# zhizdev/mvdfusion

Hardware: AMD Instinct MI355X
Metric: denoising-steps/sec (higher is better)
Workload: dtype f16x3 (f16 MFMA operands split hi+lo, 3 partial products, fp32 accumulate); 1 GPU; BASELINE.json configs[1]: V=4 views x 256^2 images (32x32 latents), D=1, 50-step DDIM (eta 1), cfg 2.5, SD1.x UNet 320ch + 10 view-aligned transformers + GridAttn, random-init (deterministic fill) weights; views=4, latent=32, depth_samples=1, parallelism=single GPU, CFG pair batched as 2V, hipgraph=True, gemm_tuning=mvdfusion_amd/tuned/gemm_f16.json: 410 problems; 0 problems tuned in this run

## Files before the change

### include/mvd_hip.h

```cpp
#ifndef MVD_HIP_H
#define MVD_HIP_H
#include <stddef.h>
#include <stdint.h>
#ifdef __cplusplus
extern "C" {
#endif

typedef void* mvd_stream_t;

#define MVD_VERSION 100
#define MVD_PREC_X1 1
#define MVD_PREC_X3 3
#define MVD_PREC_X4 4

int mvd_version(void);
const char* mvd_last_error(void);
int mvd_operand_format(void);

size_t mvd_packed_weight_bytes(int N, int K);
int mvd_pack_linear_weight(const float* w, int N, int K, int ldw, int geglu, float scale, void* packed,
                           mvd_stream_t stream);
int mvd_pack_linear_weight_t(const float* wt, int N, int K, int ldw, float scale, void* packed, mvd_stream_t stream);
int mvd_pack_conv3x3_weight(const float* w, int Cout, int Cin, int cin_pad, float scale, void* packed,
                            mvd_stream_t stream);

#define MVD_A_DENSE 0
#define MVD_A_CONV3X3 1

#define MVD_EPI_STORE 0
#define MVD_EPI_GEGLU 1
#define MVD_EPI_QKV 2

#define MVD_ACT_NONE 0
#define MVD_ACT_GELU 1
#define MVD_ACT_SILU 2
#define MVD_ACT_QUICKGELU 3

#define MVD_GEMM_TILES 5
#define MVD_GEMM_LOOPS 8
#define MVD_GEMM_CFG_STRIDE 32
#define MVD_B_PACKED 0
#define MVD_B_PLANES 1

typedef struct mvd_prefetch_item_s {
  const void* ptr;
  unsigned long long bytes;
  int start_after;
  int consumer;
} mvd_prefetch_item;

typedef struct mvd_gemm_desc {
  int M, N, K;
  const void* A;
  int lda;
  int a_mode;
  int B, Hin, Win, Cin, Hout, Wout, stride, upsample;
  int no_pad_tl;
  const void* Wp;
  int b_mode;
  int ldb;
  float acc_scale;
  int prec;
  int epi;
  int act;
  float* out;
  int ldo;
  void* out_sp;
  int ldp;
  int n_store;
  const float* bias;
  const float* bias_b;
  int rows_per_batch;
  int ldbb;
  const float* colscale;
  const float* res;
  int ldr;
  void *q_hi, *q_lo, *k_hi, *k_lo, *vt_hi, *vt_lo;
  int heads, dhead, L, Lpad;
  float qscale;
  int splitk;
  float* workspace;
  size_t workspace_elems;
  int cfg;
  long long* gn_stats;
  int gn_hw, gn_groups;
  float* rs_out;
  int* rs_count;
  int rs_ld;
  const float* ln_stats;
  const int* ln_count;
  const float* ln_colsum;
  int ln_ld, ln_dim;
  float ln_eps;
  void* gna_out_sp;
  const float* gna_gamma;
  const float* gna_beta;
  float gna_eps;
  int gna_flags;
  const float* cat_b;
  int cat_cb;
  void* cat_raw_sp;
  const float* acc_scale_dev;
  const struct mvd_prefetch_item_s* pf_items;
  int pf_n;
  int tap_mode;
  const void* A2;
  int lda2, Cin2;
} mvd_gemm_desc;
#define MVD_TAPS_FULL 0
#define MVD_TAPS_CENTRE_TAIL 2
#define MVD_GNA_SILU 1
#define MVD_GNA_ROUND_F16 2
#define MVD_GNA_OUT_UNUSED 4

int mvd_gemm(const mvd_gemm_desc* d, mvd_stream_t stream);
int mvd_gemm_cfg_supported(const mvd_gemm_desc* d, int cfg);

int mvd_split_planes(const float* x, void* sp, size_t rows, int cols, int ldx, int ldp, mvd_stream_t stream);
int mvd_split_planes_scaled(const float* x, void* sp, size_t rows, int cols, int ldx, int ldp, const float* scale_dev, mvd_stream_t stream);

int mvd_gemv(const float* W, const float* bias, const float* x, float* y, int M, int N, int K, int ldx, int ldy,
             int act_in, int act_out, mvd_stream_t stream);

int mvd_groupnorm_chunks(int HW);
int mvd_groupnorm_nhwc(const float* x, void* y_sp, const float* gamma, const float* beta, int B, int HW, int C,
                       int groups, float eps, int silu, double* ws, size_t ws_elems, mvd_stream_t stream);
int mvd_groupnorm_from_stats(const float* x, void* y_sp, const float* gamma, const float* beta, const long long* stats, int B, int HW,
                             int C, int groups, float eps, int silu, mvd_stream_t stream);
int mvd_softmax_rows(const float* x, void* y_sp, int rows, int cols, int ldx, float scale, float out_scale,
                     mvd_stream_t stream);

int mvd_layernorm(const float* x, void* y_sp, float* y_f32, const float* w, const float* b, int rows, int C, float eps,
                  int w_plus_one, mvd_stream_t stream);
int mvd_layernorm_groups(const float* x, void* y_sp, float* y_f32, const float* w, const float* b, int ldw, int rows, int rows_per_group,
                         int C, float eps, int w_plus_one, mvd_stream_t stream);

size_t mvd_attn_qk_plane_elems(int B, int heads, int L, int dhead);
size_t mvd_attn_vt_plane_elems(int B, int heads, int L, int dhead);
int mvd_attn_lpad(int L);
int mvd_attention(const void* q_hi, const void* q_lo, const void* k_hi, const void* k_lo, const void* vt_hi,
                  const void* vt_lo, void* out_sp, int ldo, int B, int heads, int L, int Lkeys, int dhead, int prec,
                  mvd_stream_t stream);

int mvd_pixel_cross_attn(const float* q, const float* k, const float* v, void* out_sp, int P, int D, int heads,
                         int dhead, mvd_stream_t stream);

int mvd_unet_input(const float* x, const float* input_latents, void* out_sp, int V, int S, int cpad, int cfg,
                   mvd_stream_t stream);
int mvd_unet_input_scenes(const float* x, const float* input_latents, void* out_sp, int nscene, int V, int S, int cpad, int cfg,
                          mvd_stream_t stream);
int mvd_concat_channels(const float* a, int Ca, const float* b, int Cb, float* out, void* out_sp, int rows, long long* gn_stats,
                        int gn_hw, int gn_groups, mvd_stream_t stream);
int mvd_concat_groupnorm_fits(int Ca, int Cb, int hw, int groups);
int mvd_concat_groupnorm(const float* a, int Ca, const float* b, int Cb, float* out, void* raw_sp, void* y_sp, const float* gamma,
                         const float* beta, long long* gn_stats, int B, int hw, int groups, float eps, int silu, mvd_stream_t stream);
int mvd_area_pool(const float* vol, void* out_sp, int B, int S, int D, int C, int factor, int ldp, mvd_stream_t stream);
int mvd_fill_zero(float* p, size_t n, mvd_stream_t stream);

#define MVD_STEP_STRIDE 8
int mvd_timestep_embedding(const float* steps, const int* iter, const float* freqs, float* out, int dim,
                           mvd_stream_t stream);
int mvd_timestep_embedding_scenes(const float* steps, const int* iter, const float* freqs, float* out, int dim, int nscene,
                                  int steps_scene_stride, mvd_stream_t stream);
int mvd_advance_iter(int* iter, mvd_stream_t stream);

#define MVD_CAM_RECORD 20
#define MVD_TOKEN_DIM 723
#define MVD_TOKEN_LD 736
int mvd_zembed(const float* lat, const float* w, const float* b, float* feat, int N, int S, mvd_stream_t stream);
int mvd_gridattn_tokens(const float* x, const float* depth_noise, const float* steps, const int* iter,
                        const float* grid_lin ,
                        const float* feat, const float* in_feat, const float* cams, const float* in_cam,
                        void* tokens_sp, int V, int q0, int Vq, int S, int D, float depth_scale, float depth_shift,
                        mvd_stream_t stream);
int mvd_gridattn_tokens_scenes(const float* x, const float* depth_noise, const float* steps, const int* iter, const float* grid_lin,
                               const float* feat, const float* in_feat, const float* cams, const float* in_cam, void* tokens_sp,
                               int nscene, int V, int q0, int Vq, int S, int D, float depth_scale, float depth_shift,
                               mvd_stream_t stream);
int mvd_gridattn_tokens_scenes_t(const float* x, const float* depth_noise, const float* steps, const int* iter, const float* grid_lin,
                                 const float* feat, const float* in_feat, const float* cams, const float* in_cam, void* tokens_sp,
                                 int nscene, int V, int q0, int Vq, int S, int D, float depth_scale, float depth_shift,
                                 int steps_scene_stride, mvd_stream_t stream);
int mvd_gridattn_fused_slots(void);
size_t mvd_gridattn_fused_stream_bytes(void);
size_t mvd_gridattn_fused_vec_floats(void);
int mvd_gridattn_fused(const float* x, const float* depth_noise, const float* steps, const int* iter, const float* grid_lin,
                       const float* feat, const float* in_feat, const float* cams, const float* in_cam, const void* wstream,
                       const float* vecs, void* pooled_sp, int V, int q0, int Vq, int S, int D, float depth_scale,
                       float depth_shift, int prec ,
                       mvd_stream_t stream);
int mvd_gridattn_fused_scenes(const float* x, const float* depth_noise, const float* steps, const int* iter, const float* grid_lin,
                              const float* feat, const float* in_feat, const float* cams, const float* in_cam, const void* wstream,
                              const float* vecs, void* pooled_sp, int nscene, int V, int q0, int Vq, int S, int D, float depth_scale,
                              float depth_shift, int prec, mvd_stream_t stream);
int mvd_gridattn_fused_scenes_t(const float* x, const float* depth_noise, const float* steps, const int* iter, const float* grid_lin,
                                const float* feat, const float* in_feat, const float* cams, const float* in_cam, const void* wstream,
                                const float* vecs, void* pooled_sp, int nscene, int V, int q0, int Vq, int S, int D, float depth_scale,
                                float depth_shift, int prec, int steps_scene_stride, int vecs_scene_stride, mvd_stream_t stream);
int mvd_gridattn_tokens_window(const float* x, const float* depth_noise, const float* steps, const int* iter, const float* grid_lin,
                               const float* feat, const float* in_feat, const float* cams, const float* in_cam, void* tokens_sp,
                               int nscene, int V, int q0, int Vq, int S, int D, float depth_scale, float depth_shift,
                               int steps_scene_stride, int window, mvd_stream_t stream);
int mvd_gridattn_fused_window(const float* x, const float* depth_noise, const float* steps, const int* iter, const float* grid_lin,
                              const float* feat, const float* in_feat, const float* cams, const float* in_cam, const void* wstream,
                              const float* vecs, void* pooled_sp, int nscene, int V, int q0, int Vq, int S, int D, float depth_scale,
                              float depth_shift, int prec, int steps_scene_stride, int vecs_scene_stride, int window,
                              mvd_stream_t stream);
int mvd_view_mha(const float* qkv, void* out_sp, int Nseq, int V, int heads, int dhead,
                 mvd_stream_t stream);
int mvd_view_pool(const float* x, const float* w, const float* b, void* out_sp, int Nseq, int V, int C,
                  mvd_stream_t stream);

int mvd_cfg_ddim_update(const float* eps_nhwc, int ldc, float* x, float* x0, float* eps_out,
                        const float* ddim_noise, size_t noise_stride ,
                        const float* steps, const int* iter, int V, int S, int cfg, float cfg_scale, int do_update,
                        mvd_stream_t stream);

int mvd_graph_begin(mvd_stream_t stream);
int mvd_graph_end(mvd_stream_t stream, void** graph_exec);
int mvd_graph_launch(void* graph_exec, mvd_stream_t stream);
int mvd_graph_destroy(void* graph_exec);
int mvd_event_create(void** ev);
int mvd_event_record(void* ev, mvd_stream_t stream);
int mvd_event_elapsed_ms(void* start, void* stop, float* ms);
int mvd_event_destroy(void* ev);

int mvd_transpose_planes(const void* x, int src_planes, int rows, int cols, int ldx, void* out_sp, int ldo, mvd_stream_t stream);
int mvd_transpose_planes_scaled(const float* x, int rows, int cols, int ldx, void* out_sp, int ldo, const float* scale_dev,
                                mvd_stream_t stream);
int mvd_im2col3x3_t_planes(const void* x_sp, int B, int H, int W, int Cin, void* out_sp, int ldo, mvd_stream_t stream);
int mvd_pow2_scale(const float* x, size_t n, float* out2, unsigned* scratch2, mvd_stream_t stream);
int mvd_adamw_multi(const void* tensors, int n_tensors, int n_chunks, float lr, float beta1, float beta2, float eps, float weight_decay,
                    float bias_c1, float bias_c2_sqrt, float grad_scale, mvd_stream_t stream);
size_t mvd_col_sum_workspace_doubles(int rows, int cols);
int mvd_col_sum(const float* x, int rows, int cols, int ldx, float* out, double* ws, size_t ws_doubles, mvd_stream_t stream);
int mvd_col_sum_pow2(const float* x, int rows, int cols, int ldx, float* out, double* ws, size_t ws_doubles, float* out2, unsigned* scratch1,
                     mvd_stream_t stream);
int mvd_groupnorm_backward(const float* x, const float* dy, const float* gamma, const float* beta, int B, int HW, int C, int groups,
                           float eps, int silu, float* dx, float* dgamma, float* dbeta, float* ws, size_t ws_floats,
                           mvd_stream_t stream);

int mvd_layernorm_backward(const float* x, const float* dy, const float* w, int rows, int C, float eps, float* dx, float* dyxhat,
                           mvd_stream_t stream);
size_t mvd_col_sum_groups_workspace_doubles(int ngroups, int rows_per_group, int cols);
int mvd_col_sum_groups(const float* x, int ngroups, int rows_per_group, int cols, int ldx, float* out, double* ws, size_t ws_doubles,
                       mvd_stream_t stream);
int mvd_layernorm_backward_groups(const float* x, const float* dy, const float* w, int ldw, int rows, int rows_per_group, int C, float eps,
                                  float* dx, float* dyxhat, float* dw, float* db, double* ws, size_t ws_doubles, mvd_stream_t stream);
int mvd_act_planes(const float* x, void* sp, float* y, size_t rows, int cols, int ldx, int ldp, int ldy, int act, mvd_stream_t stream);
int mvd_act_backward(const float* dy, const float* x, float* dx, size_t n, int act, mvd_stream_t stream);
int mvd_geglu_backward(const float* h, const float* dy, int rows, int half, float* dh, mvd_stream_t stream);
int mvd_attention_backward(const float* q, const float* k, const float* v, const float* dout, int B, int heads, int L, int dhead,
                           float* dq, float* dk, float* dv, float* stats, size_t stats_floats, mvd_stream_t stream);
int mvd_pixel_cross_attn_backward(const float* q, const float* k, const float* v, const float* dout, int P, int D, int heads, int dhead,
                                  float* dq, float* dk, float* dv, mvd_stream_t stream);

int mvd_gridattn_tokens_backward(const float* x, const float* depth_noise, const float* steps, const int* iter, const float* grid_lin,
                                 const float* cams, const float* in_cam, const float* dtok, int ldt, long long* dfeat_acc,
                                 long long* din_feat_acc, float scale, int V, int q0, int Vq, int S, int D, float depth_scale,
                                 float depth_shift, mvd_stream_t stream);
int mvd_gridattn_tokens_backward_scenes(const float* x, const float* depth_noise, const float* steps, const int* iter, const float* grid_lin,
                                        const float* cams, const float* in_cam, const float* dtok, int ldt, long long* dfeat_acc,
                                        long long* din_feat_acc, float scale, int nscene, int V, int q0, int Vq, int S, int D,
                                        float depth_scale, float depth_shift, int steps_scene_stride, mvd_stream_t stream);
int mvd_gridattn_tokens_backward_window(const float* x, const float* depth_noise, const float* steps, const int* iter, const float* grid_lin,
                                        const float* cams, const float* in_cam, const float* dtok, int ldt, long long* dfeat_acc,
                                        long long* din_feat_acc, float scale, int nscene, int V, int q0, int Vq, int S, int D,
                                        float depth_scale, float depth_shift, int steps_scene_stride, int window, mvd_stream_t stream);

#ifdef __cplusplus
}
#endif
#endif
```

### mvdfusion_amd/csrc/gemm.hip

```cpp
#include "gemm_device.hpp"

namespace {

__global__ __launch_bounds__(256) void splitk_reduce_kernel(GemmParams p) {
  const mvd_gemm_desc& d = p.d;
  const size_t MN = (size_t)d.M * d.N;
  if (d.epi == MVD_EPI_GEGLU) {
    const size_t total = (size_t)d.M * (d.N >> 1);
    for (size_t e = (size_t)blockIdx.x * 256 + threadIdx.x; e < total; e += (size_t)gridDim.x * 256) {
      const int m = (int)(e / (d.N >> 1));
      const int col = (int)(e - (size_t)m * (d.N >> 1));
      const int pv = (col >> 4) * 32 + (col & 15);
      float v = 0.f, g = 0.f;
      for (int z = 0; z < p.splits; ++z) {
        v += d.workspace[z * MN + (size_t)m * d.N + pv];
        g += d.workspace[z * MN + (size_t)m * d.N + pv + 16];
      }
      epi_geglu_elem(d, m, pv, v, g);
    }
    return;
  }
  if (d.epi == MVD_EPI_STORE) {
    const size_t MN4 = MN >> 2;
    const float inv = 1.0f / gemm_acc_scale(d);
    (void)inv;
    for (size_t e = (size_t)blockIdx.x * 256 + threadIdx.x; e < MN4; e += (size_t)gridDim.x * 256) {
      float4 v = make_float4(0.f, 0.f, 0.f, 0.f);
      for (int z = 0; z < p.splits; ++z) {
        const float4 t = *(const float4*)(d.workspace + z * MN + e * 4);
        v.x += t.x; v.y += t.y; v.z += t.z; v.w += t.w;
      }
      const int m = (int)((e * 4) / d.N);
      const int n = (int)(e * 4 - (size_t)m * d.N);
      if (n + 3 < d.n_store) {
        epi_store4(d, m, n, v);
      } else {
        epi_store_elem(d, m, n, v.x);
        epi_store_elem(d, m, n + 1, v.y);
        epi_store_elem(d, m, n + 2, v.z);
        epi_store_elem(d, m, n + 3, v.w);
      }
    }
    return;
  }
  for (size_t e = (size_t)blockIdx.x * 256 + threadIdx.x; e < MN; e += (size_t)gridDim.x * 256) {
    float v = 0.f;
    for (int z = 0; z < p.splits; ++z) v += d.workspace[z * MN + e];
    const int m = (int)(e / d.N);
    const int n = (int)(e - (size_t)m * d.N);
    epi_store_elem(d, m, n, v);
  }
}

__global__ __launch_bounds__(256) void splitk_reduce_rows_kernel(GemmParams p) {
  const mvd_gemm_desc& d = p.d;
  const size_t MN = (size_t)d.M * d.N;
  const int lane = threadIdx.x & 63;
  const int m = blockIdx.x * 4 + (threadIdx.x >> 6);
  const int n = blockIdx.y * 256 + lane * 4;
  if (m >= d.M) return;
  float s1 = 0.f, q1 = 0.f;
  if (n < d.N) {
    float4 v = make_float4(0.f, 0.f, 0.f, 0.f);
    const float* w = d.workspace + (size_t)m * d.N + n;
    for (int z = 0; z < p.splits; ++z) {
      const float4 t = *(const float4*)(w + z * MN);
      v.x += t.x; v.y += t.y; v.z += t.z; v.w += t.w;
    }
    const float4 f = epi_store4(d, m, n, v);
    s1 = (f.x + f.y) + (f.z + f.w);
    q1 = (f.x * f.x + f.y * f.y) + (f.z * f.z + f.w * f.w);
  }
  s1 = wave_sum(s1);
  q1 = wave_sum(q1);
  if (lane == 0) *((float2*)d.rs_out + (size_t)m * d.rs_ld + blockIdx.y) = make_float2(s1, q1);
  if (blockIdx.x == 0 && blockIdx.y == 0 && threadIdx.x == 0) d.rs_count[0] = gridDim.y;
}

template <int RPT>
__global__ __launch_bounds__(256) void splitk_reduce_stats_kernel(GemmParams p) {
  __shared__ float cs[2][4][256];
  const mvd_gemm_desc& d = p.d;
  const size_t MN = (size_t)d.M * d.N;
  const int m0 = blockIdx.x * (4 * RPT), n0 = blockIdx.y * 256;
  const int c4 = threadIdx.x & 63, rg = threadIdx.x >> 6;
  const int n = n0 + c4 * 4;
  float4 s = make_float4(0.f, 0.f, 0.f, 0.f), q = make_float4(0.f, 0.f, 0.f, 0.f);
  if (n < d.N) {
    float4 v[RPT];
#pragma unroll
    for (int r = 0; r < RPT; ++r) v[r] = make_float4(0.f, 0.f, 0.f, 0.f);
    const float* w = d.workspace + (size_t)(m0 + rg * RPT) * d.N + n;
#pragma unroll 2
    for (int z = 0; z < p.splits; ++z) {
#pragma unroll
      for (int r = 0; r < RPT; ++r) {
        const float4 t = *(const float4*)(w + z * MN + (size_t)r * d.N);
        v[r].x += t.x; v[r].y += t.y; v[r].z += t.z; v[r].w += t.w;
      }
    }
#pragma unroll
    for (int r = 0; r < RPT; ++r) v[r] = epi_value4(d, m0 + rg * RPT + r, n, v[r]);
#pragma unroll
    for (int r = 0; r < RPT; ++r) {
      const float4 f = v[r];
      epi_put4(d, m0 + rg * RPT + r, n, f);
      s.x += f.x; s.y += f.y; s.z += f.z; s.w += f.w;
      q.x += f.x * f.x; q.y += f.y * f.y; q.z += f.z * f.z; q.w += f.w * f.w;
    }
  }
  *(float4*)&cs[0][rg][c4 * 4] = s;
  *(float4*)&cs[1][rg][c4 * 4] = q;
  __syncthreads();
  const int c = threadIdx.x, nn = n0 + c;
  const float cs_ = cs[0][0][c] + cs[0][1][c] + cs[0][2][c] + cs[0][3][c];
  const float cq_ = cs[1][0][c] + cs[1][1][c] + cs[1][2][c] + cs[1][3][c];
  __syncthreads();
  cs[0][0][c] = cs_;
  cs[1][0][c] = cq_;
  __syncthreads();
  if (nn >= d.N) return;
  const int cg = d.N / d.gn_groups;
  const int g = nn / cg, pos = nn - g * cg;
  if (c != 0 && pos != 0) return;
  int len = cg - pos;
  if (len > 256 - c) len = 256 - c;
  float ss = 0.f, qq = 0.f;
  for (int j = 0; j < len; ++j) {
    ss += cs[0][0][c + j];
    qq += cs[1][0][c + j];
  }
  gn_stats_add(d.gn_stats, m0 / d.gn_hw, g, d.gn_groups, ss, qq);
}

#define MVD_GNK_THREADS 1024
__global__ __launch_bounds__(MVD_GNK_THREADS) void splitk_gn_kernel(GemmParams p) {
  constexpr int NT = MVD_GNK_THREADS, NWV = NT / 64, U = 3, ZC = 4;
  extern __shared__ float s_val[];
  __shared__ double s_red[2][NWV];
  __shared__ float s_coef[2][128];
  const mvd_gemm_desc& d = p.d;
  const int G = d.gn_groups, HW = d.gn_hw;
  const int CT = d.N + (d.cat_b ? d.cat_cb : 0);
  const int cg = CT / G, cg2 = cg >> 1;
  int g, b;
  {
    const int bid = blockIdx.x;
    if ((G & 7) == 0) {
      const int gpx = G >> 3, x = bid & 7, r = bid >> 3;
      g = x * gpx + r % gpx;
      b = r / gpx;
    } else {
      g = bid % G;
      b = bid / G;
    }
  }
  const int tid = threadIdx.x, lane = tid & 63, wave = tid >> 6;
  const int c0 = g * cg, m0 = b * HW;
  const size_t MN = (size_t)d.M * d.N;
  const int total = HW * cg2;
  const bool put_out = d.out != nullptr && !(d.gna_flags & MVD_GNA_OUT_UNUSED);
  const int dq = NT / cg2, dj = NT - dq * cg2;
  const int rs = tid / cg2, js = tid - rs * cg2;
  const int r0 = tid < total ? rs : 0, j0 = tid < total ? js : 0;
  const float* const zero2 = (const float*)g_zero_page;
  const bool has_bias = d.bias != nullptr, has_bb = d.bias_b != nullptr, has_res = d.res != nullptr;
  const float ascale = gemm_acc_scale(d);
  float s = 0.f, q = 0.f;
  {
    int r = rs, j = js;
    for (int e0 = tid; e0 < total; e0 += NT * U) {
      int rr[U], jj[U];
      bool ok[U];
#pragma unroll
      for (int u = 0; u < U; ++u) {
        ok[u] = e0 + u * NT < total;
        rr[u] = ok[u] ? r : r0;
        jj[u] = ok[u] ? j : j0;
        r += dq;
        j += dj;
        if (j >= cg2) {
          j -= cg2;
          ++r;
        }
      }
      float2 acc[U], tb[U], tbb[U], tr[U];
      float2 t[ZC][U];
      const int nz0 = p.splits < ZC ? p.splits : ZC;
      bool own[U];
      float2 tc[U];
#pragma unroll
      for (int u = 0; u < U; ++u) {
        const int m = m0 + rr[u], nn = c0 + 2 * jj[u];
        own[u] = nn < d.N;
        const int n = own[u] ? nn : 0;
        tb[u] = *(const float2*)(has_bias ? d.bias + n : zero2);
        tbb[u] = *(const float2*)(has_bb ? d.bias_b + (size_t)(m / d.rows_per_batch) * d.ldbb + n : zero2);
        tr[u] = *(const float2*)(has_res ? d.res + (size_t)m * d.ldr + n : zero2);
        tc[u] = *(const float2*)(own[u] ? zero2 : d.cat_b + (size_t)m * d.cat_cb + (nn - d.N));
#pragma unroll
        for (int z = 0; z < ZC; ++z) {
          const float* w = d.workspace + (size_t)(z < nz0 ? z : 0) * MN + (size_t)m * d.N + n;
          t[z][u] = *(const float2*)w;
        }
      }
#pragma unroll
      for (int u = 0; u < U; ++u) {
        acc[u] = make_float2(0.f, 0.f);
#pragma unroll
        for (int z = 0; z < ZC; ++z)
          if (z < nz0) {
            acc[u].x += t[z][u].x;
            acc[u].y += t[z][u].y;
          }
      }
      for (int zb = ZC; zb < p.splits; zb += ZC) {
        const int nz = p.splits - zb < ZC ? p.splits - zb : ZC;
#pragma unroll
        for (int u = 0; u < U; ++u) {
          const int m = m0 + rr[u], n = own[u] ? c0 + 2 * jj[u] : 0;
#pragma unroll
          for (int z = 0; z < ZC; ++z) t[z][u] = *(const float2*)(d.workspace + (size_t)(zb + (z < nz ? z : 0)) * MN + (size_t)m * d.N + n);
        }
#pragma unroll
        for (int u = 0; u < U; ++u)
#pragma unroll
          for (int z = 0; z < ZC; ++z)
            if (z < nz) {
              acc[u].x += t[z][u].x;
              acc[u].y += t[z][u].y;
            }
      }
#pragma unroll
      for (int u = 0; u < U; ++u) {
        float2 v = acc[u];
        v.x = v.x * ascale + tb[u].x + tbb[u].x + tr[u].x;
        v.y = v.y * ascale + tb[u].y + tbb[u].y + tr[u].y;
        if (!own[u]) v = tc[u];
        if (ok[u]) {
          const int m = m0 + rr[u], n = c0 + 2 * jj[u];
          if (put_out && own[u]) *(float2*)(d.out + (size_t)m * d.ldo + n) = v;
          if (d.cat_raw_sp) {
            uint32_t hh, ll;
            split_op16x2(v.x, v.y, hh, ll);
            u16* pp = (u16*)d.cat_raw_sp + sp_index((size_t)m, CT, n);
            *(uint32_t*)pp = hh;
            *(uint32_t*)(pp + 32) = ll;
          }
          *(float2*)(s_val + 2 * (e0 + u * NT)) = v;
          s += v.x + v.y;
          q += v.x * v.x + v.y * v.y;
        }
      }
    }
  }
  unsigned pf_sink = 0;
  if (d.pf_items != nullptr) {
    const __attribute__((address_space(4))) mvd_prefetch_item* tab = (const __attribute__((address_space(4))) mvd_prefetch_item*)d.pf_items;
    const int gw = blockIdx.x * NWV + wave, GW = gridDim.x * NWV;
    for (int it = 0; it < d.pf_n; ++it) {
      const unsigned char* base = (const unsigned char*)tab[it].ptr;
      const long lines = (long)((tab[it].bytes + 127) >> 7);
      for (long l = (long)gw * 64 + lane; l < lines; l += (long)GW * 64) {
        const unsigned char* a = base + (l << 7);
        asm volatile("global_load_dword %0, %1, off" : "+v"(pf_sink) : "v"(a) : "memory");
      }
    }
  }
  {
    const double sd = wave_sum_d((double)s), qd = wave_sum_d((double)q);
    if (lane == 0) {
      s_red[0][wave] = sd;
      s_red[1][wave] = qd;
    }
  }
  __syncthreads();
  double S1 = 0.0, S2 = 0.0;
#pragma unroll
  for (int w = 0; w < NWV; ++w) {
    S1 += s_red[0][w];
    S2 += s_red[1][w];
  }
  const double cnt = (double)HW * cg;
  const double mean = S1 / cnt;
  double var = S2 / cnt - mean * mean;
  if (var < 0.0) var = 0.0;
  const float rstd = (float)(1.0 / sqrt(var + (double)d.gna_eps));
  if (tid < cg) {
    const float a = rstd * d.gna_gamma[c0 + tid];
    s_coef[0][tid] = a;
    s_coef[1][tid] = d.gna_beta[c0 + tid] - (float)mean * a;
  }
  if (tid == 0 && d.gn_stats) gn_stats_add(d.gn_stats, b, g, G, (float)S1, (float)S2);
  __syncthreads();
  u16* const ysp = (u16*)d.gna_out_sp;
  const int fl = d.gna_flags;
  {
    int r = rs, j = js;
    for (int e = tid; e < total; e += NT) {
      float2 v = *(const float2*)(s_val + 2 * e);
      v.x = v.x * s_coef[0][2 * j] + s_coef[1][2 * j];
      v.y = v.y * s_coef[0][2 * j + 1] + s_coef[1][2 * j + 1];
      if (fl & MVD_GNA_ROUND_F16) {
        v.x = (float)(_Float16)v.x;
        v.y = (float)(_Float16)v.y;
      }
      if (fl & MVD_GNA_SILU) {
        v.x = silu_f(v.x);
        v.y = silu_f(v.y);
      }
      uint32_t hh, ll;
      split_op16x2(v.x, v.y, hh, ll);
      u16* pp = ysp + sp_index((size_t)(m0 + r), CT, c0 + 2 * j);
      *(uint32_t*)pp = hh;
      *(uint32_t*)(pp + 32) = ll;
      r += dq;
      j += dj;
      if (j >= cg2) {
        j -= cg2;
        ++r;
      }
    }
  }
  asm volatile("" ::"v"(pf_sink));
}

struct TileInfo {
  int bm, bn, waves;
  int cores_plain, cores_pipe;
};
static const TileInfo kTiles[MVD_GEMM_TILES] = {{64, 64, 4, 5, 3}, {128, 128, 8, 2, 1}, {128, 80, 4, 2, 2}, {64, 80, 4, 4, 3},
                                                {128, 160, 8, 1, 1}};

static int choose_splits(long tiles, int nk, const TileInfo& ti, int loop, size_t mn) {
  const double area = (double)ti.bm * ti.bn / (128.0 * 128.0);
  const double t_mfma = 0.75 * area;
  const double t_lat = loop == 0 ? 1.0 : (loop == 1 ? 0.4 : (loop == 2 ? 0.2 : (loop == 5 ? 0.05 : 0.1)));
  const double t_epi = 0.27 + 1.73 * area;
  const int coresident = loop == 0 ? ti.cores_plain : (loop == 1 ? ti.cores_pipe : (loop == 4 && ti.waves == 4 ? 2 : 1));
  const double red_fixed = 6.0, red_per_split = (double)mn * 8.0 / 3.0e12 / 0.7e-6;
  int best = 1;
  double best_t = 1e30;
  const int smax = nk / 8 < 1 ? 1 : (nk / 8 > 32 ? 32 : nk / 8);
  for (int sp = 1; sp <= smax; ++sp) {
    const int iters = (nk + sp - 1) / sp;
    if ((long)iters * (sp - 1) >= nk) continue;
    const long per_cu = (tiles * sp + 255) / 256;
    const long rounds = (per_cu + coresident - 1) / coresident;
    const double busy = (double)per_cu * (iters * t_mfma + t_epi);
    const double lat = (double)rounds * (iters * t_lat + t_epi);
    double t = busy > lat ? busy : lat;
    if (sp > 1) t += red_fixed + sp * red_per_split;
    if (t < best_t * 0.97) {
      best_t = t;
      best = sp;
    }
  }
  return best;
}

static int patch_shares(const mvd_gemm_desc& d, const TileInfo& ti) {
  if (d.a_mode != MVD_A_CONV3X3 || d.b_mode != MVD_B_PACKED || d.stride != 1 || d.upsample || d.no_pad_tl) return 0;
  if (d.tap_mode != MVD_TAPS_FULL) return 0;
  if (d.Hin != d.Hout || d.Win != d.Wout || ti.bm != 128) return 0;
  const int W = d.Wout, HW = d.Hout * d.Wout;
  if (ti.bm % W != 0 || (HW >= ti.bm ? HW % ti.bm != 0 : ti.bm % HW != 0)) return 0;
  const int nseg = HW >= ti.bm ? 1 : ti.bm / HW, Rb = HW >= ti.bm ? ti.bm / W : d.Hout;
  const int P = nseg * (Rb + 2) * (W + 2);
  if (P > MVD_PATCH_SLOTS_MAX) return 0;
  const int PG = (P + 7) / 8, cap = (11 - conv_patch_ring(ti.bn, ti.waves)) * ti.waves;
  return PG <= cap ? 1 : (PG <= 2 * cap ? 2 : 0);
}

static bool cfg_supported(const mvd_gemm_desc& d, int cfg) {
  if (cfg == 0) return true;
  if (cfg < 0 || cfg > MVD_GEMM_CFG_STRIDE * MVD_GEMM_TILES) return false;
  const int tile = (cfg - 1) / MVD_GEMM_CFG_STRIDE, loop = ((cfg - 1) % MVD_GEMM_CFG_STRIDE) >> 1;
  if (loop >= MVD_GEMM_LOOPS) return false;
  if (tile >= 2 && d.epi != MVD_EPI_STORE) return false;
  const int waves = kTiles[tile].waves;
  if ((loop == 2 || loop == 3) && waves != 8) return false;
  if (loop == 3 || loop >= 8) return false;
  if (loop == 5 && waves != 4) return false;
  if (loop == 6) return (tile == 1 || tile == 2 || tile == 4) && patch_shares(d, kTiles[tile]) > 0;
  if (loop == 7) return tile == 1 || ((tile == 2 || tile == 4) && d.epi == MVD_EPI_STORE);
  return true;
}

}

extern "C" int mvd_gemm_cfg_supported(const mvd_gemm_desc* dp, int cfg) { return dp && cfg_supported(*dp, cfg) ? 1 : 0; }

extern "C" int mvd_gemm(const mvd_gemm_desc* dp, mvd_stream_t stream) {
  MVD_CHECK_ARG(dp != nullptr, "mvd_gemm: null descriptor");
  GemmParams p;
  p.d = *dp;
  mvd_gemm_desc& d = p.d;
  MVD_CHECK_ARG(d.M > 0 && d.N > 0 && d.K > 0, "mvd_gemm: bad sizes M=%d N=%d K=%d", d.M, d.N, d.K);
  MVD_CHECK_ARG(d.K % 32 == 0, "mvd_gemm: K=%d must be a multiple of 32 (pad the packed weight)", d.K);
  MVD_CHECK_ARG(d.N % 16 == 0, "mvd_gemm: N=%d must be a multiple of 16 (pad the packed weight)", d.N);
  MVD_CHECK_ARG(d.prec == MVD_PREC_X1 || d.prec == MVD_PREC_X3 || d.prec == MVD_PREC_X4, "mvd_gemm: bad prec %d", d.prec);
  MVD_CHECK_ARG(d.A && d.Wp, "mvd_gemm: null operand");
  MVD_CHECK_ARG(((uintptr_t)d.A & 127) == 0 && ((uintptr_t)d.Wp & 127) == 0, "mvd_gemm: operands must be 128-byte aligned");
  if (d.a_mode == MVD_A_CONV3X3) {
    MVD_CHECK_ARG(d.tap_mode == MVD_TAPS_FULL || d.tap_mode == MVD_TAPS_CENTRE_TAIL, "mvd_gemm: tap_mode %d is not served", d.tap_mode);
    const bool tail = d.tap_mode == MVD_TAPS_CENTRE_TAIL;
    if (tail) {
      MVD_CHECK_ARG(d.A2 != nullptr && ((uintptr_t)d.A2 & 127) == 0 && d.Cin2 > 0 && d.Cin2 % 32 == 0 && d.lda2 >= d.Cin2 && d.lda2 % 32 == 0,
                    "mvd_gemm: the centre-tap tail needs A2 (128-byte aligned), Cin2 %% 32 == 0 and lda2 >= Cin2, a multiple of 32 (Cin2=%d lda2=%d)",
                    d.Cin2, d.lda2);
      MVD_CHECK_ARG(d.stride == 1 && !d.upsample && !d.no_pad_tl && d.Hin == d.Hout && d.Win == d.Wout && d.b_mode == MVD_B_PACKED,
                    "mvd_gemm: the centre-tap tail serves stride-1 padded convolutions with Hin == Hout, Win == Wout and a packed weight");
      MVD_CHECK_ARG((long long)d.M * 2 * d.lda2 < (1ll << 31), "mvd_gemm: A2 is addressed with 32-bit offsets (M=%d lda2=%d)", d.M, d.lda2);
    }
    MVD_CHECK_ARG(d.Cin % 32 == 0 && d.K == 9 * d.Cin + (tail ? d.Cin2 : 0),
                  "mvd_gemm: conv needs Cin %% 32 == 0 and K == 9*Cin (+ Cin2 with a centre-tap tail) (Cin=%d Cin2=%d K=%d)", d.Cin,
                  tail ? d.Cin2 : 0, d.K);
    MVD_CHECK_ARG(d.M == d.B * d.Hout * d.Wout, "mvd_gemm: conv M mismatch");
    MVD_CHECK_ARG(d.stride == 1 || d.stride == 2, "mvd_gemm: conv stride must be 1 or 2");
    if (d.upsample) MVD_CHECK_ARG(d.stride == 1 && d.Hout == 2 * d.Hin && d.Wout == 2 * d.Win, "mvd_gemm: upsample geometry");
  } else {
    MVD_CHECK_ARG(d.a_mode == MVD_A_DENSE, "mvd_gemm: bad a_mode");
    MVD_CHECK_ARG(d.tap_mode == MVD_TAPS_FULL, "mvd_gemm: tap_mode %d needs a_mode == MVD_A_CONV3X3", d.tap_mode);
    MVD_CHECK_ARG(d.lda >= d.K && d.lda % 32 == 0, "mvd_gemm: lda=%d must be >= K=%d and a multiple of 32", d.lda, d.K);
  }
  if (d.out_sp) MVD_CHECK_ARG(d.ldp > 0 && d.ldp % 32 == 0 && ((uintptr_t)d.out_sp & 127) == 0,
                              "mvd_gemm: split-plane output needs ldp %% 32 == 0 and 128-byte alignment");
  if (d.out) MVD_CHECK_ARG(d.ldo % 4 == 0 && ((uintptr_t)d.out & 15) == 0, "mvd_gemm: out must be 16-byte aligned with ldo %% 4 == 0");
  if (d.res) MVD_CHECK_ARG(d.ldr % 4 == 0 && ((uintptr_t)d.res & 15) == 0, "mvd_gemm: res must be 16-byte aligned with ldr %% 4 == 0");
  MVD_CHECK_ARG(((uintptr_t)d.bias & 15) == 0 && ((uintptr_t)d.bias_b & 15) == 0 && ((uintptr_t)d.colscale & 15) == 0,
                "mvd_gemm: bias / bias_b / colscale must be 16-byte aligned");
  if (d.epi == MVD_EPI_STORE) {
    MVD_CHECK_ARG(d.out != nullptr || d.out_sp != nullptr, "mvd_gemm: no output");
    if (d.n_store <= 0 || d.n_store > d.N) d.n_store = d.N;
    if (d.bias_b) {
      MVD_CHECK_ARG(d.rows_per_batch > 0, "mvd_gemm: bias_b needs rows_per_batch");
      if (d.ldbb == 0) d.ldbb = d.N;
      MVD_CHECK_ARG(d.ldbb % 4 == 0, "mvd_gemm: ldbb %% 4 != 0");
    }
  } else if (d.epi == MVD_EPI_GEGLU) {
    MVD_CHECK_ARG((d.out != nullptr || d.out_sp != nullptr) && d.N % 32 == 0, "mvd_gemm: GEGLU needs an output and N %% 32 == 0");
    d.bias_b = nullptr;
  } else if (d.epi == MVD_EPI_QKV) {
    MVD_CHECK_ARG(d.q_hi && d.q_lo && d.k_hi && d.k_lo && d.vt_hi && d.vt_lo, "mvd_gemm: QKV planes missing");
    MVD_CHECK_ARG(d.heads > 0 && d.dhead > 0 && d.N == 3 * d.heads * d.dhead, "mvd_gemm: QKV needs N == 3*heads*dhead");
    MVD_CHECK_ARG(d.L > 0 && d.M % d.L == 0 && d.Lpad >= d.L, "mvd_gemm: QKV needs M %% L == 0");
    MVD_CHECK_ARG(d.dhead % 4 == 0 && d.L % 4 == 0, "mvd_gemm: QKV needs dhead %% 4 == 0 and L %% 4 == 0");
  } else {
    MVD_CHECK_ARG(false, "mvd_gemm: bad epilogue %d", d.epi);
  }
  if (d.rs_out)
    MVD_CHECK_ARG(d.epi == MVD_EPI_STORE && d.n_store == d.N && !d.gn_stats && d.rs_count && d.rs_ld >= cdiv(d.N, 32) && ((uintptr_t)d.rs_out & 7) == 0,
                  "mvd_gemm: rs_out needs MVD_EPI_STORE, n_store == N, no gn_stats, rs_count and rs_ld >= N / 32 (N=%d rs_ld=%d)", d.N, d.rs_ld);
  if (d.ln_stats) {
    MVD_CHECK_ARG((d.epi == MVD_EPI_QKV || d.epi == MVD_EPI_GEGLU) && d.ln_count && d.ln_colsum && d.ln_dim > 0 && d.ln_ld > 0 &&
                      ((uintptr_t)d.ln_stats & 7) == 0 && ((uintptr_t)d.ln_colsum & 15) == 0,
                  "mvd_gemm: ln_stats (LayerNorm fold) serves the QKV / GEGLU epilogues and needs ln_count, ln_colsum, ln_dim, ln_ld");
    d.splitk = 1;
  }
  if (d.gn_stats)
    MVD_CHECK_ARG(d.epi == MVD_EPI_STORE && d.n_store == d.N && d.M % 16 == 0 && d.gn_hw > 0 && d.gn_hw % 16 == 0 && d.gn_groups > 0 &&
                      d.N % d.gn_groups == 0,
                  "mvd_gemm: gn_stats needs MVD_EPI_STORE, n_store == N, M %% 16 == 0, gn_hw %% 16 == 0, N %% gn_groups == 0 (N=%d M=%d hw=%d)",
                  d.N, d.M, d.gn_hw);
  if (d.gna_out_sp)
    MVD_CHECK_ARG(d.gn_stats && d.out && d.ldo == d.N && d.gna_gamma && d.gna_beta && d.N % 32 == 0 && d.M % d.gn_hw == 0 &&
                      ((uintptr_t)d.gna_out_sp & 127) == 0,
                  "mvd_gemm: gna_out_sp (GroupNorm apply behind the GEMM) needs gn_stats, out with ldo == N, gamma / beta, N %% 32 == 0, M %% gn_hw == 0");
  if (d.cat_b)
    MVD_CHECK_ARG(d.gna_out_sp && d.cat_cb > 0 && d.cat_cb % 2 == 0 && (d.N + d.cat_cb) % 32 == 0 && (d.N + d.cat_cb) % d.gn_groups == 0 &&
                      ((uintptr_t)d.cat_b & 7) == 0 && ((uintptr_t)d.cat_raw_sp & 127) == 0 &&
                      mvd_concat_groupnorm_fits(d.N, d.cat_cb, d.gn_hw, d.gn_groups),
                  "mvd_gemm: cat_b (GroupNorm over [out | cat_b]) needs gna_out_sp, an even cat_cb, (N + cat_cb) %% 32 == 0 and a shape "
                  "mvd_concat_groupnorm_fits() accepts (N=%d cat_cb=%d hw=%d)", d.N, d.cat_cb, d.gn_hw);
  long long* const gna_stats = d.gn_stats;
  if (d.cat_b) d.gn_stats = nullptr;
  if (d.b_mode == MVD_B_PLANES)
    MVD_CHECK_ARG(d.ldb >= d.K && d.ldb % 32 == 0, "mvd_gemm: B planes need ldb=%d >= K=%d, a multiple of 32", d.ldb, d.K);
  else
    MVD_CHECK_ARG(d.b_mode == MVD_B_PACKED, "mvd_gemm: bad b_mode %d", d.b_mode);
  if (d.acc_scale == 0.f) d.acc_scale = 1.f;
  p.nk = d.K / 32;
  p.nt16 = d.N / 16;
  int tile, loop = 0, order = -1;
  MVD_CHECK_ARG(d.cfg >= 0 && d.cfg <= MVD_GEMM_CFG_STRIDE * MVD_GEMM_TILES, "mvd_gemm: bad cfg %d", d.cfg);
  if (d.cfg >= 1) {
    tile = (d.cfg - 1) / MVD_GEMM_CFG_STRIDE;
    loop = ((d.cfg - 1) % MVD_GEMM_CFG_STRIDE) >> 1;
    order = (d.cfg - 1) & 1;
    MVD_CHECK_ARG(cfg_supported(d, d.cfg), "mvd_gemm: cfg %d (tile %d, loop %d) does not serve this problem (include/mvd_hip.h: cfg)", d.cfg, tile,
                  loop);
  } else {
    const long tiles128 = (long)cdiv(d.M, 128) * cdiv(d.N, 128);
    tile = (tiles128 >= 128 && (d.N >= 512 || d.K >= 2048)) ? 1 : 0;
  }
  const TileInfo& ti = kTiles[tile];
  p.tiles_n = cdiv(d.N, ti.bn);
  p.tiles_m = cdiv(d.M, ti.bm);
  if (order < 0) {
    const double W = (double)d.N * d.K * 4.0;
    const double A = (double)d.M * d.K * 4.0 / (d.a_mode == MVD_A_CONV3X3 ? 9.0 : 1.0);
    const double rep_m = p.tiles_m < 8 ? p.tiles_m : 8, rep_n = p.tiles_n < 8 ? p.tiles_n : 8;
    order = (W + A * rep_n) < (W * rep_m + A) ? 1 : 0;
  }
  p.m_fastest = order;
  int splits = d.splitk;
  const long tiles = (long)p.tiles_m * p.tiles_n;
  if (splits == 0) splits = choose_splits(tiles, p.nk, ti, loop, (size_t)d.M * d.N);
  if (splits < 1) splits = 1;
  if (splits > p.nk) splits = p.nk;
  if (splits > 1) {
    if (d.workspace == nullptr) splits = 1;
    else {
      const size_t cap = d.workspace_elems / ((size_t)d.M * d.N);
      if ((size_t)splits > cap) splits = cap < 1 ? 1 : (int)cap;
    }
  }
  p.kt_per_split = cdiv(p.nk, splits);
  if (loop == 6) p.kt_per_split = 9 * cdiv(p.nk / 9, splits);
  p.splits = cdiv(p.nk, p.kt_per_split);
  hipStream_t s = (hipStream_t)stream;
  bool launched;
  if (loop == 6) launched = mvd_gemm_launch_patch(tile, p, s, patch_shares(d, ti));
  else if (loop == 7) launched = mvd_gemm_launch_ws(tile, p, s);
  else if (tile == 0) launched = mvd_gemm_launch_plain_t0(loop, p, s);
  else if (tile == 1) launched = mvd_gemm_launch_plain_t1(loop, p, s);
  else if (tile == 2) launched = mvd_gemm_launch_plain_t2(loop, p, s);
  else if (tile == 3) launched = mvd_gemm_launch_plain_t3(loop, p, s);
  else launched = mvd_gemm_launch_plain_t4(loop, p, s);
  MVD_CHECK_ARG(launched, "mvd_gemm: no kernel for tile %d loop %d", tile, loop);
  MVD_CHECK_LAUNCH("mvd_gemm");
  const int gna_ct = d.N + (d.cat_b ? d.cat_cb : 0);
  const int gna_cg = d.gna_out_sp ? gna_ct / d.gn_groups : 0;
  const size_t gna_lds = (size_t)d.gn_hw * gna_cg * 4;
  const bool gna_fused = d.gna_out_sp && p.splits > 1 && !d.rs_out && !d.out_sp && !d.colscale && d.act == MVD_ACT_NONE && (gna_cg & 1) == 0 &&
                         gna_cg <= 128 && gna_lds <= 128 * 1024 && d.ldo % 2 == 0 && (!d.res || d.ldr % 2 == 0) && (!d.bias_b || d.ldbb % 2 == 0) &&
                         d.N % 2 == 0;
  if (gna_fused) {
    {
      static unsigned long long raised = 0;
      const hipError_t e = mvd_raise_dynamic_lds((const void*)splitk_gn_kernel, 128 * 1024, &raised);
      MVD_CHECK_ARG(e == hipSuccess, "mvd_gemm: hipFuncSetAttribute(MaxDynamicSharedMemorySize): %s", hipGetErrorString(e));
    }
    p.d.gn_stats = gna_stats;
    if (loop == 7) p.d.pf_items = nullptr;
    hipLaunchKernelGGL(splitk_gn_kernel, dim3((d.M / d.gn_hw) * d.gn_groups), dim3(MVD_GNK_THREADS), gna_lds, s, p);
    MVD_CHECK_LAUNCH("mvd_gemm/splitk_gn");
    return 0;
  }
  if (p.splits > 1) {
    if (d.rs_out) {
      hipLaunchKernelGGL(splitk_reduce_rows_kernel, dim3(cdiv(d.M, 4), cdiv(d.N, 256)), dim3(256), 0, s, p);
    } else if (d.gn_stats) {
      const int spans = (d.N + 255) / 256;
      if ((d.M / 16) * spans >= 1024)
        hipLaunchKernelGGL(splitk_reduce_stats_kernel<4>, dim3(d.M / 16, spans), dim3(256), 0, s, p);
      else
        hipLaunchKernelGGL(splitk_reduce_stats_kernel<2>, dim3(d.M / 8, spans), dim3(256), 0, s, p);
    } else {
      const size_t total = (size_t)d.M * d.N;
      int blocks = (int)((total + 255) / 256);
      if (blocks > 2048) blocks = 2048;
      hipLaunchKernelGGL(splitk_reduce_kernel, dim3(blocks), dim3(256), 0, s, p);
    }
    MVD_CHECK_LAUNCH("mvd_gemm/splitk_reduce");
  }
  if (d.gna_out_sp && d.cat_b)
    return mvd_concat_groupnorm(d.out, d.N, d.cat_b, d.cat_cb, nullptr, d.cat_raw_sp, d.gna_out_sp, d.gna_gamma, d.gna_beta, gna_stats,
                                d.M / d.gn_hw, d.gn_hw, d.gn_groups, d.gna_eps, d.gna_flags & (MVD_GNA_SILU | MVD_GNA_ROUND_F16), stream);
  if (d.gna_out_sp)
    return mvd_groupnorm_from_stats(d.out, d.gna_out_sp, d.gna_gamma, d.gna_beta, d.gn_stats, d.M / d.gn_hw, d.gn_hw, d.N, d.gn_groups,
                                    d.gna_eps, d.gna_flags & (MVD_GNA_SILU | MVD_GNA_ROUND_F16), stream);
  return 0;
}

namespace {
__global__ __launch_bounds__(256) void pack_kernel(const float* __restrict__ w, u16* __restrict__ out, int N, int K,
                                                   int Np, int Kp, int ldw, int geglu, int conv_cin, int trans,
                                                   float scale) {
  const int nt16 = Np >> 4;
  const size_t total = (size_t)(Kp >> 5) * nt16 * 64;
  for (size_t e = (size_t)blockIdx.x * 256 + threadIdx.x; e < total; e += (size_t)gridDim.x * 256) {
    const size_t mt = e >> 6;
    const int l = (int)(e & 63);
    const int kt = (int)(mt / nt16), nt = (int)(mt - (size_t)kt * nt16);
    const int n = nt * 16 + (l & 15);
    const int k = kt * 32 + (l >> 4) * 8;
    int src_n = n;
    if (geglu) {
      const int blk = n >> 5, within = n & 31;
      src_n = within < 16 ? blk * 16 + within : (N >> 1) + blk * 16 + (within - 16);
    }
    float v[8];
#pragma unroll
    for (int j = 0; j < 8; ++j) v[j] = 0.f;
    if (src_n < N) {
      if (conv_cin > 0) {
        const int cb = kt / 9, tap = kt - cb * 9;
        const int ci0 = cb * 32 + (k & 31);
#pragma unroll
        for (int j = 0; j < 8; ++j)
          if (ci0 + j < conv_cin) v[j] = w[((size_t)src_n * conv_cin + ci0 + j) * 9 + tap];
      } else if (trans) {
#pragma unroll
        for (int j = 0; j < 8; ++j)
          if (k + j < K) v[j] = w[(size_t)(k + j) * ldw + src_n];
      } else {
        const float* src = w + (size_t)src_n * ldw + k;
        if (k + 7 < K && (ldw & 3) == 0 && ((uintptr_t)w & 15) == 0) {
          const float4 a = *(const float4*)src, b = *(const float4*)(src + 4);
          v[0] = a.x; v[1] = a.y; v[2] = a.z; v[3] = a.w; v[4] = b.x; v[5] = b.y; v[6] = b.z; v[7] = b.w;
        } else {
#pragma unroll
          for (int j = 0; j < 8; ++j)
            if (k + j < K) v[j] = src[j];
        }
      }
    }
    union { uint4 q; u16 h[8]; } H, Lo;
#pragma unroll
    for (int j = 0; j < 8; ++j) split_op16(v[j] * scale, H.h[j], Lo.h[j]);
    u16* o = out + mt * 1024 + l * 8;
    *(uint4*)o = H.q;
    *(uint4*)(o + 512) = Lo.q;
  }
}

__global__ __launch_bounds__(256) void split_planes_kernel(const float* __restrict__ x, u16* __restrict__ sp, size_t rows, int cols,
                                                           int ldx, int ldp, const float* __restrict__ scale) {
  const float sc = scale != nullptr ? *scale : 1.f;
  const int c4 = ldp >> 2;
  const size_t total = rows * c4;
  for (size_t e = (size_t)blockIdx.x * 256 + threadIdx.x; e < total; e += (size_t)gridDim.x * 256) {
    const size_t r = e / c4;
    const int c = (int)(e - r * c4) * 4;
    float v[4];
#pragma unroll
    for (int j = 0; j < 4; ++j) v[j] = (c + j) < cols ? x[r * ldx + c + j] * sc : 0.f;
    store_sp4(sp, r, ldp, c, v[0], v[1], v[2], v[3]);
  }
}
}

extern "C" size_t mvd_packed_weight_bytes(int N, int K) {
  const size_t Np = (size_t)((N + 15) & ~15), Kp = (size_t)((K + 31) & ~31);
  return Np * Kp * 4;
}

extern "C" int mvd_operand_format(void) { return MVD_OPERAND_FORMAT; }

extern "C" int mvd_pack_linear_weight(const float* w, int N, int K, int ldw, int geglu, float scale, void* packed,
                                      mvd_stream_t stream) {
  MVD_CHECK_ARG(w && packed && N > 0 && K > 0 && ldw >= K, "mvd_pack_linear_weight: bad arguments");
  if (geglu) MVD_CHECK_ARG(N % 32 == 0, "mvd_pack_linear_weight: geglu needs N %% 32 == 0");
  const int Np = (N + 15) & ~15, Kp = (K + 31) & ~31;
  const size_t total = (size_t)Np * Kp / 8;
  int blocks = (int)((total + 255) / 256);
  if (blocks > 4096) blocks = 4096;
  hipLaunchKernelGGL(pack_kernel, dim3(blocks), dim3(256), 0, (hipStream_t)stream, w, (u16*)packed, N, K, Np, Kp, ldw,
                     geglu, 0, 0, scale);
  MVD_CHECK_LAUNCH("mvd_pack_linear_weight");
  return 0;
}

extern "C" int mvd_pack_linear_weight_t(const float* wt, int N, int K, int ldw, float scale, void* packed, mvd_stream_t stream) {
  MVD_CHECK_ARG(wt && packed && N > 0 && K > 0 && ldw >= N, "mvd_pack_linear_weight_t: bad arguments");
  const int Np = (N + 15) & ~15, Kp = (K + 31) & ~31;
  const size_t total = (size_t)Np * Kp / 8;
  int blocks = (int)((total + 255) / 256);
  if (blocks > 4096) blocks = 4096;
  hipLaunchKernelGGL(pack_kernel, dim3(blocks), dim3(256), 0, (hipStream_t)stream, wt, (u16*)packed, N, K, Np, Kp, ldw, 0, 0, 1, scale);
  MVD_CHECK_LAUNCH("mvd_pack_linear_weight_t");
  return 0;
}

extern "C" int mvd_pack_conv3x3_weight(const float* w, int Cout, int Cin, int cin_pad, float scale, void* packed,
                                       mvd_stream_t stream) {
  MVD_CHECK_ARG(w && packed && Cout > 0 && Cin > 0 && cin_pad >= Cin && cin_pad % 32 == 0,
                "mvd_pack_conv3x3_weight: bad arguments (cin_pad must be a multiple of 32)");
  const int Np = (Cout + 15) & ~15, Kp = 9 * cin_pad;
  const size_t total = (size_t)Np * Kp / 8;
  int blocks = (int)((total + 255) / 256);
  if (blocks > 4096) blocks = 4096;
  hipLaunchKernelGGL(pack_kernel, dim3(blocks), dim3(256), 0, (hipStream_t)stream, w, (u16*)packed, Cout, Kp, Np, Kp, 0,
                     0, Cin, 0, scale);
  MVD_CHECK_LAUNCH("mvd_pack_conv3x3_weight");
  return 0;
}

extern "C" int mvd_split_planes_scaled(const float* x, void* sp, size_t rows, int cols, int ldx, int ldp, const float* scale_dev,
                                       mvd_stream_t stream) {
  MVD_CHECK_ARG(x && sp && rows > 0 && cols > 0 && ldx >= cols && ldp >= cols && ldp % 32 == 0,
                "mvd_split_planes: bad arguments (ldp must be a multiple of 32)");
  const size_t total = rows * (size_t)(ldp / 4);
  int blocks = (int)((total + 255) / 256);
  if (blocks > 4096) blocks = 4096;
  hipLaunchKernelGGL(split_planes_kernel, dim3(blocks), dim3(256), 0, (hipStream_t)stream, x, (u16*)sp, rows, cols, ldx, ldp, scale_dev);
  MVD_CHECK_LAUNCH("mvd_split_planes");
  return 0;
}

extern "C" int mvd_split_planes(const float* x, void* sp, size_t rows, int cols, int ldx, int ldp, mvd_stream_t stream) {
  return mvd_split_planes_scaled(x, sp, rows, cols, ldx, ldp, nullptr, stream);
}
```

### mvdfusion_amd/csrc/gemm_common.hpp

```cpp
#pragma once
#include "common.hpp"
#include "../../include/mvd_hip.h"

struct GemmParams {
  mvd_gemm_desc d;
  int nk;
  int nt16;
  int kt_per_split;
  int splits;
  int tiles_m, tiles_n;
  int m_fastest;
};

__device__ __forceinline__ float gemm_acc_scale(const mvd_gemm_desc& d) {
  return d.acc_scale_dev != nullptr ? d.acc_scale * *d.acc_scale_dev : d.acc_scale;
}

bool mvd_gemm_launch_plain_t0(int loop, GemmParams& p, hipStream_t s);
bool mvd_gemm_launch_plain_t1(int loop, GemmParams& p, hipStream_t s);
bool mvd_gemm_launch_plain_t2(int loop, GemmParams& p, hipStream_t s);
bool mvd_gemm_launch_plain_t3(int loop, GemmParams& p, hipStream_t s);
bool mvd_gemm_launch_plain_t4(int loop, GemmParams& p, hipStream_t s);
bool mvd_gemm_launch_ws(int tile, GemmParams& p, hipStream_t s);
bool mvd_gemm_launch_patch(int tile, GemmParams& p, hipStream_t s, int patch_shares);
```

### mvdfusion_amd/csrc/gemm_device.hpp

```cpp
#pragma once
#include <stdlib.h>
#include <type_traits>

#include "gemm_common.hpp"

namespace {

__device__ __attribute__((aligned(16))) unsigned int g_zero_page[4];

__device__ __forceinline__ float apply_act(float v, int act) {
  if (act == MVD_ACT_GELU) return gelu_erf(v);
  if (act == MVD_ACT_SILU) return silu_f(v);
  if (act == MVD_ACT_QUICKGELU) return v / (1.0f + expf(-1.702f * v));
  return v;
}

__device__ __forceinline__ void store_out(const mvd_gemm_desc& d, int m, int n, float v) {
  if (d.out) d.out[(size_t)m * d.ldo + n] = v;
  if (d.out_sp) store_sp1((u16*)d.out_sp, (size_t)m, d.ldp, n, v);
}

__device__ __forceinline__ float epi_store_elem(const mvd_gemm_desc& d, int m, int n, float v) {
  if (d.epi == MVD_EPI_STORE && n >= d.n_store) return 0.f;
  v *= gemm_acc_scale(d);
  if (d.bias) v += d.bias[n];
  if (d.bias_b) v += d.bias_b[(size_t)(m / d.rows_per_batch) * d.ldbb + n];
  if (d.epi == MVD_EPI_QKV) {
    const int C = d.heads * d.dhead;
    const int which = n / C;
    const int cc = n - which * C;
    const int head = cc / d.dhead;
    const int dd = cc - head * d.dhead;
    const int b = m / d.L;
    const int tok = m - b * d.L;
    if (which == 0) v *= d.qscale;
    if (which < 2) {
      const int dq = mvd_attn_dpad(d.dhead);
      const size_t idx = ((size_t)(b * d.heads + head) * d.Lpad + tok) * dq + dd;
      store_planes1((u16*)(which == 0 ? d.q_hi : d.k_hi), (u16*)(which == 0 ? d.q_lo : d.k_lo), idx, v);
    } else {
      const int dv = (d.dhead + 15) & ~15;
      const size_t idx = ((size_t)(b * d.heads + head) * dv + dd) * d.Lpad + tok;
      store_planes1((u16*)d.vt_hi, (u16*)d.vt_lo, idx, v);
    }
    return v;
  }
  v = apply_act(v, d.act);
  if (d.colscale) v *= d.colscale[n];
  if (d.res) v += d.res[(size_t)m * d.ldr + n];
  store_out(d, m, n, v);
  return v;
}

__device__ __forceinline__ void epi_geglu_elem(const mvd_gemm_desc& d, int m, int p_value, float v, float g) {
  const int col = (p_value >> 5) * 16 + (p_value & 15);
  const int half = d.N >> 1;
  v *= gemm_acc_scale(d);
  g *= gemm_acc_scale(d);
  if (d.bias) {
    v += d.bias[col];
    g += d.bias[half + col];
  }
  store_out(d, m, col, v * gelu_erf(g));
}

__device__ __forceinline__ float4 epi_value4(const mvd_gemm_desc& d, int m, int n, float4 v) {
  v.x *= gemm_acc_scale(d); v.y *= gemm_acc_scale(d); v.z *= gemm_acc_scale(d); v.w *= gemm_acc_scale(d);
  if (d.bias) {
    const float4 b = *(const float4*)(d.bias + n);
    v.x += b.x; v.y += b.y; v.z += b.z; v.w += b.w;
  }
  if (d.bias_b) {
    const float4 b = *(const float4*)(d.bias_b + (size_t)(m / d.rows_per_batch) * d.ldbb + n);
    v.x += b.x; v.y += b.y; v.z += b.z; v.w += b.w;
  }
  if (d.act) {
    v.x = apply_act(v.x, d.act); v.y = apply_act(v.y, d.act); v.z = apply_act(v.z, d.act); v.w = apply_act(v.w, d.act);
  }
  if (d.colscale) {
    const float4 g = *(const float4*)(d.colscale + n);
    v.x *= g.x; v.y *= g.y; v.z *= g.z; v.w *= g.w;
  }
  if (d.res) {
    const float4 r = *(const float4*)(d.res + (size_t)m * d.ldr + n);
    v.x += r.x; v.y += r.y; v.z += r.z; v.w += r.w;
  }
  return v;
}
__device__ __forceinline__ void epi_put4(const mvd_gemm_desc& d, int m, int n, const float4& v) {
  if (d.out) *(float4*)(d.out + (size_t)m * d.ldo + n) = v;
  if (d.out_sp) store_sp4((u16*)d.out_sp, (size_t)m, d.ldp, n, v.x, v.y, v.z, v.w);
}
__device__ __forceinline__ float4 epi_store4(const mvd_gemm_desc& d, int m, int n, float4 v) {
  v = epi_value4(d, m, n, v);
  epi_put4(d, m, n, v);
  return v;
}

__device__ __forceinline__ int conv_tail_start(const mvd_gemm_desc& d) {
  return d.tap_mode == MVD_TAPS_CENTRE_TAIL ? 9 * (d.Cin >> 5) : 0x7fffffff;
}

#define MVD_PATCH_SLOTS_MAX 288
__host__ __device__ constexpr int conv_patch_ring(int bn, int waves) {
  const int bstage = ((bn / 8 + waves - 1) / waves) * waves;
  const int fit = (160 - 2 * (MVD_PATCH_SLOTS_MAX / 8 + 1) - 2) / bstage;
  return fit > 4 ? 4 : fit;
}

__device__ __forceinline__ float2 ln_row_stats(const mvd_gemm_desc& d, int m) {
  const int cnt = d.ln_count[0];
  const float2* p = (const float2*)d.ln_stats + (size_t)m * d.ln_ld;
  double s = 0.0, q = 0.0;
  for (int i = 0; i < cnt; i += 4) {
    float2 v[4];
#pragma unroll
    for (int j = 0; j < 4; ++j) v[j] = p[min(i + j, cnt - 1)];
#pragma unroll
    for (int j = 0; j < 4; ++j) {
      if (i + j < cnt) {
        s += (double)v[j].x;
        q += (double)v[j].y;
      }
    }
  }
  const double mean = s / (double)d.ln_dim;
  double var = q / (double)d.ln_dim - mean * mean;
  if (var < 0.0) var = 0.0;
  return make_float2((float)mean, (float)(1.0 / sqrt(var + (double)d.ln_eps)));
}

#ifdef MVD_STAMP
#define MVD_STAMP_AT(d, wave, slot)                                                                                       \
  do {                                                                                                                    \
    if ((blockIdx.x == 0 || blockIdx.x == 100) && (wave) < 4 && (threadIdx.x & 63) == 0)                                  \
      ((long long*)(d).workspace)[(blockIdx.x == 100 ? 64 : 0) + (wave) * 16 + (slot)] = (long long)__builtin_readcyclecounter(); \
  } while (0)
#else
#define MVD_STAMP_AT(d, wave, slot) do {} while (0)
#endif

template <int BM, int BN, int WM, int WN>
__device__ __forceinline__ void tile_epilogue(const GemmParams& p, f32x4 (&acc)[BM / WM / 16][BN / WN / 16], unsigned char* smem, int m0,
                                              int n0, int lane, int wave, const float* s_rows = nullptr) {
  constexpr int WTM = BM / WM, WTN = BN / WN;
  constexpr int TM = WTM / 16, TN = WTN / 16;
  constexpr int LDW = WTN + 4;
  constexpr int C4 = WTN / 4;
  const mvd_gemm_desc& d = p.d;
  const int wm = wave / WN, wn = wave % WN;
  float* sC = (float*)smem + wave * (WTM * LDW);
  MVD_STAMP_AT(d, wave, 4);
  {
    const int crow = (lane >> 4) * 4, ccol = lane & 15;
#pragma unroll
    for (int i = 0; i < TM; ++i)
#pragma unroll
      for (int j = 0; j < TN; ++j)
#pragma unroll
        for (int r = 0; r < 4; ++r) sC[(i * 16 + crow + r) * LDW + j * 16 + ccol] = acc[i][j][r];
  }
  const int wm0 = m0 + wm * WTM, wn0 = n0 + wn * WTN;
#ifdef MVD_STAMP
  asm volatile("s_waitcnt lgkmcnt(0)" ::: "memory");
#endif
  MVD_STAMP_AT(d, wave, 5);
  if (wn0 >= d.N) return;
  const bool lnf = s_rows != nullptr;
  const float* sR = s_rows + (wave / WN) * WTM * 2;
  if (p.splits > 1) {
    float* ws = d.workspace + (size_t)blockIdx.z * d.M * d.N;
#pragma unroll 2
    for (int ps = 0; ps < (WTM * C4 + 63) / 64; ++ps) {
      const int idx = ps * 64 + lane;
      const int row = idx / C4, col = (idx - row * C4) * 4;
      const int m = wm0 + row, n = wn0 + col;
      if (idx < WTM * C4 && m < d.M && n < d.N) *(float4*)(ws + (size_t)m * d.N + n) = *(const float4*)(sC + row * LDW + col);
    }
    return;
  }
  if constexpr (WTN % 32 == 0) {
  if (d.epi == MVD_EPI_GEGLU || d.epi == MVD_EPI_QKV) {
  const int wn0_tile = wn0;
  float* const sC_tile = sC;
#pragma unroll 1
  for (int jb = 0; jb < WTN / 32; ++jb) {
  const int wn0 = wn0_tile + jb * 32;
  float* const sC = sC_tile + jb * 32;
  if (wn0 >= d.N) break;
  if (d.epi == MVD_EPI_GEGLU) {
    const int ocol0 = (wn0 >> 5) * 16;
    const int half = d.N >> 1;
    const int q = (lane & 3) * 4, col = ocol0 + q;
    float4 sv = make_float4(0.f, 0.f, 0.f, 0.f), sg = sv, bv = sv, bg = sv;
    if (lnf) {
      sv = *(const float4*)(d.ln_colsum + col);
      sg = *(const float4*)(d.ln_colsum + half + col);
    }
    if (d.bias) {
      bv = *(const float4*)(d.bias + col);
      bg = *(const float4*)(d.bias + half + col);
    }
    constexpr int NCH = WTM / 16;
    float4 gv[NCH];
    const float scale = gemm_acc_scale(d);
    auto geglu_values = [&](auto lnf_c) {
      constexpr bool LNF = decltype(lnf_c)::value;
#pragma unroll
      for (int ps = 0; ps < NCH; ++ps) {
        const int row = ps * 16 + (lane >> 2);
        float4 v = *(const float4*)(sC + row * LDW + q);
        float4 g = *(const float4*)(sC + row * LDW + 16 + q);
        v.x *= scale; v.y *= scale; v.z *= scale; v.w *= scale;
        g.x *= scale; g.y *= scale; g.z *= scale; g.w *= scale;
        if (LNF) {
          const float mean = sR[row * 2], rstd = sR[row * 2 + 1];
          v.x = (v.x - mean * sv.x) * rstd; v.y = (v.y - mean * sv.y) * rstd; v.z = (v.z - mean * sv.z) * rstd; v.w = (v.w - mean * sv.w) * rstd;
          g.x = (g.x - mean * sg.x) * rstd; g.y = (g.y - mean * sg.y) * rstd; g.z = (g.z - mean * sg.z) * rstd; g.w = (g.w - mean * sg.w) * rstd;
        }
        v.x += bv.x; v.y += bv.y; v.z += bv.z; v.w += bv.w;
        g.x += bg.x; g.y += bg.y; g.z += bg.z; g.w += bg.w;
        gelu_erf4(g.x, g.y, g.z, g.w);
        v.x *= g.x; v.y *= g.y; v.z *= g.z; v.w *= g.w;
        gv[ps] = v;
      }
    };
    if (lnf) geglu_values(std::integral_constant<bool, true>{});
    else geglu_values(std::integral_constant<bool, false>{});
#pragma unroll
    for (int ps = 0; ps < NCH; ++ps) {
      const int m = wm0 + ps * 16 + (lane >> 2);
      if (m < d.M) {
        if (d.out) *(float4*)(d.out + (size_t)m * d.ldo + col) = gv[ps];
        if (d.out_sp) store_sp4((u16*)d.out_sp, (size_t)m, d.ldp, col, gv[ps].x, gv[ps].y, gv[ps].z, gv[ps].w);
      }
    }
    continue;
  }
  {
    const int C = d.heads * d.dhead;
    const int which = wn0 / C;
    if (which < 2) {
      const int dq = mvd_attn_dpad(d.dhead);
      u16* ph = (u16*)(which == 0 ? d.q_hi : d.k_hi);
      u16* pl = (u16*)(which == 0 ? d.q_lo : d.k_lo);
      const int col = (lane & 7) * 4, n = wn0 + col;
      const int cc = n - which * C;
      const int head = cc / d.dhead, dd = cc - head * d.dhead;
      const float qs = which == 0 ? d.qscale : 1.0f;
      float4 bb = make_float4(0.f, 0.f, 0.f, 0.f), cs = bb;
      if (d.bias) bb = *(const float4*)(d.bias + n);
      if (lnf) cs = *(const float4*)(d.ln_colsum + n);
      constexpr int NCQ = WTM / 8;
      float4 qv[NCQ];
      const float scale = gemm_acc_scale(d);
      auto qk_values = [&](auto lnf_c) {
        constexpr bool LNF = decltype(lnf_c)::value;
#pragma unroll
        for (int ps = 0; ps < NCQ; ++ps) {
          const int row = ps * 8 + (lane >> 3);
          float4 v = *(const float4*)(sC + row * LDW + col);
          v.x *= scale; v.y *= scale; v.z *= scale; v.w *= scale;
          if (LNF) {
            const float mean = sR[row * 2], rstd = sR[row * 2 + 1];
            v.x = (v.x - mean * cs.x) * rstd; v.y = (v.y - mean * cs.y) * rstd; v.z = (v.z - mean * cs.z) * rstd; v.w = (v.w - mean * cs.w) * rstd;
          }
          qv[ps] = make_float4((v.x + bb.x) * qs, (v.y + bb.y) * qs, (v.z + bb.z) * qs, (v.w + bb.w) * qs);
        }
      };
      if (lnf) qk_values(std::integral_constant<bool, true>{});
      else qk_values(std::integral_constant<bool, false>{});
#pragma unroll
      for (int ps = 0; ps < NCQ; ++ps) {
        const int m = wm0 + ps * 8 + (lane >> 3);
        if (m < d.M) {
          const int b = m / d.L, tok = m - b * d.L;
          const size_t idx = ((size_t)(b * d.heads + head) * d.Lpad + tok) * dq + dd;
          store_planes4(ph, pl, idx, qv[ps].x, qv[ps].y, qv[ps].z, qv[ps].w);
        }
      }
    } else {
      const int dv = (d.dhead + 15) & ~15;
      const int col = lane & 31, rsel = lane >> 5;
      const int cc = wn0 + col - 2 * C;
      const int head = cc / d.dhead, dd = cc - head * d.dhead;
      const float bv = d.bias ? d.bias[wn0 + col] : 0.f;
      const float csv = lnf ? d.ln_colsum[wn0 + col] : 0.f;
      constexpr int NCV = WTM / 8;
      float4 vv[NCV];
      const float scale = gemm_acc_scale(d);
      auto vt_values = [&](auto lnf_c) {
        constexpr bool LNF = decltype(lnf_c)::value;
#pragma unroll
        for (int ps = 0; ps < NCV; ++ps) {
          const int row = (ps * 2 + rsel) * 4;
          float t4[4];
#pragma unroll
          for (int i = 0; i < 4; ++i) {
            t4[i] = sC[(row + i) * LDW + col] * scale;
            if (LNF) t4[i] = (t4[i] - sR[(row + i) * 2] * csv) * sR[(row + i) * 2 + 1];
            t4[i] += bv;
          }
          vv[ps] = make_float4(t4[0], t4[1], t4[2], t4[3]);
        }
      };
      if (lnf) vt_values(std::integral_constant<bool, true>{});
      else vt_values(std::integral_constant<bool, false>{});
#pragma unroll
      for (int ps = 0; ps < NCV; ++ps) {
        const int m = wm0 + (ps * 2 + rsel) * 4;
        if (m < d.M) {
          const int b = m / d.L, tok = m - b * d.L;
          const size_t idx = ((size_t)(b * d.heads + head) * dv + dd) * d.Lpad + tok;
          store_planes4((u16*)d.vt_hi, (u16*)d.vt_lo, idx, vv[ps].x, vv[ps].y, vv[ps].z, vv[ps].w);
        }
      }
    }
  }
  }
  MVD_STAMP_AT(d, wave, 9);
  MVD_STAMP_AT(d, wave, 6);
  MVD_STAMP_AT(d, wave, 7);
  return;
  }
  }
  constexpr int RPC = 64 / C4;
  constexpr int NPS = (WTM + RPC - 1) / RPC;
  const int lrow = lane / C4, lcol = (lane - lrow * C4) * 4;
  const int n = wn0 + lcol;
  const int mrow0 = wm0 + lrow;
  const bool lane_ok = lane < RPC * C4 && n + 3 < d.n_store;
  float* const sL = sC + lrow * LDW + lcol;
  const int rows_ok = min(WTM - lrow, d.M - mrow0);
  auto pass1 = [&](auto act_c, auto res_c, auto bb_c) {
    constexpr int ACT = decltype(act_c)::value;
    constexpr bool HAS_RES = decltype(res_c)::value, HAS_BB = decltype(bb_c)::value;
    constexpr int GRP = NPS <= 11 ? NPS : (NPS + 1) / 2, NGRP = (NPS + GRP - 1) / GRP;
    const float scale = gemm_acc_scale(d);
    const bool has_bias = d.bias != nullptr, has_cs = d.colscale != nullptr;
    float4 b = make_float4(0.f, 0.f, 0.f, 0.f), cs = make_float4(1.f, 1.f, 1.f, 1.f);
    if (has_bias && lane_ok) b = *(const float4*)(d.bias + n);
    if (has_cs && lane_ok) cs = *(const float4*)(d.colscale + n);
    const float* const zero = (const float*)g_zero_page;
    const bool use_res = HAS_RES && d.res != nullptr, use_bb = HAS_BB && d.bias_b != nullptr;
    const bool lane_any = lane_ok && rows_ok > 0;
    const float* const rbase = use_res && lane_any ? d.res + (size_t)mrow0 * d.ldr + n : zero;
    const size_t rstep = use_res && lane_any ? (size_t)RPC * d.ldr : 0;
    const float* const bbase = use_bb && lane_any ? d.bias_b + n : zero;
    const int rpb = use_bb ? d.rows_per_batch : 1, ldbb = use_bb && lane_any ? d.ldbb : 0;
#pragma unroll 1
    for (int g = 0; g < NGRP; ++g) {
      float4 qr[GRP], qb[GRP], qv[GRP];
#pragma unroll
      for (int j = 0; j < GRP; ++j) {
        const int ps = g * GRP + j;
        const bool ok = lane_ok && ps * RPC < rows_ok;
        const int pc = ok ? ps : 0;
        if (HAS_RES) qr[j] = *(const float4*)(rbase + (size_t)pc * rstep);
        if (HAS_BB) qb[j] = *(const float4*)(bbase + (size_t)((mrow0 + pc * RPC) / rpb) * ldbb);
        qv[j] = *(const float4*)(sL + pc * (RPC * LDW));
      }
#pragma unroll
      for (int j = 0; j < GRP; ++j) {
        const int ps = g * GRP + j;
        float4 v = qv[j];
        v.x *= scale; v.y *= scale; v.z *= scale; v.w *= scale;
        if (has_bias) {
          v.x += b.x; v.y += b.y; v.z += b.z; v.w += b.w;
        }
        if (HAS_BB) {
          v.x += qb[j].x; v.y += qb[j].y; v.z += qb[j].z; v.w += qb[j].w;
        }
        if (ACT == MVD_ACT_GELU) {
          gelu_erf4(v.x, v.y, v.z, v.w);
        } else if (ACT != MVD_ACT_NONE) {
          v.x = apply_act(v.x, ACT); v.y = apply_act(v.y, ACT); v.z = apply_act(v.z, ACT); v.w = apply_act(v.w, ACT);
        }
        if (has_cs) {
          v.x *= cs.x; v.y *= cs.y; v.z *= cs.z; v.w *= cs.w;
        }
        if (HAS_RES) {
          v.x += qr[j].x; v.y += qr[j].y; v.z += qr[j].z; v.w += qr[j].w;
        }
        if (lane_ok && ps * RPC < rows_ok) *(float4*)(sL + ps * (RPC * LDW)) = v;
      }
    }
  };
  {
    using std::integral_constant;
    const integral_constant<bool, true> yes{};
    const integral_constant<bool, false> no{};
    if (d.act == MVD_ACT_NONE) {
      if (d.res) {
        if (d.bias_b) pass1(integral_constant<int, MVD_ACT_NONE>{}, yes, yes);
        else pass1(integral_constant<int, MVD_ACT_NONE>{}, yes, no);
      } else {
        if (d.bias_b) pass1(integral_constant<int, MVD_ACT_NONE>{}, no, yes);
        else pass1(integral_constant<int, MVD_ACT_NONE>{}, no, no);
      }
    } else if (d.act == MVD_ACT_SILU) pass1(integral_constant<int, MVD_ACT_SILU>{}, yes, yes);
    else if (d.act == MVD_ACT_GELU) pass1(integral_constant<int, MVD_ACT_GELU>{}, yes, yes);
    else pass1(integral_constant<int, MVD_ACT_QUICKGELU>{}, yes, yes);
  }
  if (d.n_store & 3 || d.n_store < d.N) {
    if (lane < RPC * C4 && n < d.N && n + 3 >= d.n_store) {
#pragma unroll 1
      for (int ps = 0; ps * RPC < rows_ok; ++ps)
#pragma unroll 1
        for (int e = 0; e < 4; ++e) epi_store_elem(d, mrow0 + ps * RPC, n + e, sL[ps * (RPC * LDW) + e]);
    }
  }
  MVD_STAMP_AT(d, wave, 9);
  if (lane_ok) {
    float* po = d.out ? d.out + (size_t)mrow0 * d.ldo + n : nullptr;
    u16* psp = d.out_sp ? (u16*)d.out_sp + sp_index((size_t)mrow0, d.ldp, n) : nullptr;
    const size_t ostep = (size_t)RPC * d.ldo, sstep = (size_t)RPC * 2 * d.ldp;
#pragma unroll 1
    for (int p0 = 0; p0 * RPC < rows_ok; p0 += 4) {
      float4 f[4];
#pragma unroll
      for (int j = 0; j < 4; ++j) f[j] = *(const float4*)(sL + ((p0 + j) * RPC < rows_ok ? p0 + j : 0) * (RPC * LDW));
#pragma unroll
      for (int j = 0; j < 4; ++j) {
        if ((p0 + j) * RPC >= rows_ok) break;
        if (po) {
          *(float4*)po = f[j];
          po += ostep;
        }
        if (psp) {
          uint32_t h0, l0, h1, l1;
          split_op16x2(f[j].x, f[j].y, h0, l0);
          split_op16x2(f[j].z, f[j].w, h1, l1);
          *(uint2*)psp = make_uint2(h0, h1);
          *(uint2*)(psp + 32) = make_uint2(l0, l1);
          psp += sstep;
        }
      }
    }
  }
  MVD_STAMP_AT(d, wave, 6);
#ifdef MVD_STAMP
  asm volatile("s_waitcnt vmcnt(0)" ::: "memory");
#endif
  MVD_STAMP_AT(d, wave, 7);
  if (d.rs_out) {
    __builtin_amdgcn_fence(__ATOMIC_RELEASE, "wavefront");
    __builtin_amdgcn_wave_barrier();
    const int ncol = min(WTN, d.n_store - wn0);
    for (int r = lane; r < WTM && wm0 + r < d.M; r += 64) {
      float s1 = 0.f, q1 = 0.f;
      for (int c = 0; c + 3 < ncol; c += 4) {
        const float4 v = *(const float4*)(sC + r * LDW + c);
        s1 += (v.x + v.y) + (v.z + v.w);
        q1 += (v.x * v.x + v.y * v.y) + (v.z * v.z + v.w * v.w);
      }
      *((float2*)d.rs_out + (size_t)(wm0 + r) * d.rs_ld + wn0 / WTN) = make_float2(s1, q1);
    }
    if (m0 == 0 && n0 == 0 && wave == 0 && lane == 0) d.rs_count[0] = (d.n_store + WTN - 1) / WTN;
  }
  if (d.gn_stats) {
    const int cg = d.n_store / d.gn_groups;
    const int jmax = cg < 64 ? cg : 64;
    __builtin_amdgcn_fence(__ATOMIC_RELEASE, "wavefront");
    __builtin_amdgcn_wave_barrier();
#pragma unroll 1
    for (int c0 = 0; c0 < WTN; c0 += 64) {
      const int col = c0 + lane, n = wn0 + col;
      const bool okc = col < WTN && n < d.n_store;
      const int gidx = okc ? n / cg : 0, pos = okc ? n - gidx * cg : 0;
      const bool leader = okc && (pos == 0 || lane == 0);
      int len = 0;
      if (leader) {
        len = cg - pos;
        if (len > 64 - lane) len = 64 - lane;
        if (len > WTN - col) len = WTN - col;
        if (len > d.n_store - n) len = d.n_store - n;
      }
      const bool whole = d.gn_hw % WTM == 0;
      float s1 = 0.f, q1 = 0.f;
#pragma unroll 1
      for (int sl = 0; sl < WTM / 16; ++sl) {
        const int ms = wm0 + sl * 16;
        if (ms >= d.M) break;
        if (!whole) s1 = q1 = 0.f;
        if (okc) {
#pragma unroll
          for (int r = 0; r < 16; ++r) {
            const float v = sC[(sl * 16 + r) * LDW + col];
            s1 += v;
            q1 += v * v;
          }
        }
        if (whole && sl + 1 < WTM / 16 && ms + 16 < d.M) continue;
        float ss = s1, qq = q1;
        for (int j = 1; j < jmax; ++j) {
          const float ts = __shfl_down(s1, j, 64), tq = __shfl_down(q1, j, 64);
          if (j < len) {
            ss += ts;
            qq += tq;
          }
        }
        if (leader) gn_stats_add(d.gn_stats, ms / d.gn_hw, gidx, d.gn_groups, ss, qq);
      }
    }
  }
}

__device__ __forceinline__ void wait_lgkm_and_barrier() { asm volatile("s_waitcnt lgkmcnt(0)\n\ts_barrier" ::: "memory"); }

template <int N>
__device__ __forceinline__ void wait_vm_and_barrier() {
  asm volatile("s_waitcnt vmcnt(%0) lgkmcnt(0)\n\ts_barrier" ::"i"(N) : "memory");
}

template <int G, int SLOTS, int NM, int LPS>
__device__ __forceinline__ void sched_pattern() {
  if constexpr (G < SLOTS) {
    constexpr int mf = NM * (G + 1) / SLOTS - NM * G / SLOTS;
    if constexpr (mf > 0) __builtin_amdgcn_sched_group_barrier(0x008, mf, 0);
    if constexpr (G < LPS)
      __builtin_amdgcn_sched_group_barrier(0x020, 1, 0);
    else
      __builtin_amdgcn_sched_group_barrier(0x100, 1, 0);
    sched_pattern<G + 1, SLOTS, NM, LPS>();
  }
}

template <int J, int N, class F>
__device__ __forceinline__ void unroll_steps(F&& f) {
  if constexpr (J < N) {
    f(std::integral_constant<int, J>{});
    unroll_steps<J + 1, N>(f);
  }
}

template <int G, int NR, int NM>
__device__ __forceinline__ void sched_reads_early() {
  if constexpr (G < NR) {
    __builtin_amdgcn_sched_group_barrier(0x008, 1, 0);
    __builtin_amdgcn_sched_group_barrier(0x100, 1, 0);
    sched_reads_early<G + 1, NR, NM>();
  } else if constexpr (NM > NR) {
    __builtin_amdgcn_sched_group_barrier(0x008, NM - NR, 0);
  }
}

}
```

### mvdfusion_amd/csrc/gemm_plain.hpp

```cpp
#pragma once
#include "gemm_device.hpp"

namespace {

template <int BM, int BN, int WM, int WN, int NS, int AMODE, int STAGES>
__global__ __launch_bounds__(WM * WN * 64, (BM == 128 && BN == 128 && STAGES == 2 && AMODE == MVD_A_DENSE) ? 4 : ((BM == 64 && BN == 80 && STAGES == 3) ? 3 : 1))
void gemm_kernel(GemmParams p) {
  constexpr int NW = WM * WN;
  constexpr int WTM = BM / WM, WTN = BN / WN;
  constexpr int TM = WTM / 16, TN = WTN / 16;
  constexpr int A_GRAN = BM / 8, B_GRAN = BN / 8;
  constexpr int AI = A_GRAN / NW, BI = (B_GRAN + NW - 1) / NW;
  constexpr int B_GRAN_P = BI * NW;
  constexpr int STAGE = (A_GRAN + B_GRAN_P) * 1024;
  constexpr int LPS = AI + BI;
  constexpr int LDW = WTN + 4;
  constexpr int EPI_BYTES = NW * WTM * LDW * 4;
  constexpr bool RING = STAGES == 6 || STAGES == 7;
  constexpr bool PIPE = STAGES == 3 || RING;
  constexpr bool STAG = STAGES == 4;
  constexpr int TAB_BYTES = AMODE != MVD_A_DENSE ? BM * 9 * 4 : 0;
  constexpr int LNR_BYTES = AMODE == MVD_A_DENSE ? BM * 8 : 0;
  constexpr int RING_FIT = (160 * 1024 - TAB_BYTES - LNR_BYTES) / STAGE;
  constexpr int RING_WANT = STAGES == 6 ? 4 : 8;
  constexpr int NBUF = STAG ? STAGES - 1 : (RING ? (RING_WANT < RING_FIT ? RING_WANT : RING_FIT) : 2);
  constexpr int LEAD = NBUF - 1;
  constexpr int SMEM = NBUF * STAGE > EPI_BYTES ? NBUF * STAGE : EPI_BYTES;
  static_assert(NBUF >= 2 && SMEM + TAB_BYTES + LNR_BYTES <= 160 * 1024, "LDS budget");
  static_assert(!STAG || NW == 8, "the staggered loop pairs the two wavefronts of each SIMD: 8-wave tiles only");
  static_assert(A_GRAN % NW == 0, "A granules must divide evenly over the waves");
  static_assert(WTM % 16 == 0 && WTN % 16 == 0 && B_GRAN % 2 == 0, "wave tiles are made of 16x16 MFMA tiles");

  __shared__ __attribute__((aligned(1024))) unsigned char smem[SMEM + TAB_BYTES + LNR_BYTES];

  const mvd_gemm_desc& d = p.d;
  const int tid = threadIdx.x;
  const int lane = tid & 63;
  const int wave = __builtin_amdgcn_readfirstlane(tid >> 6);
  const int wm = wave / WN, wn = wave % WN;
  MVD_STAMP_AT(d, wave, 0);
  int tile;
  {
    const int nb = p.tiles_n * p.tiles_m, bid = blockIdx.x;
    const int q = nb >> 3, r = nb & 7, xcd = bid & 7, idx = bid >> 3;
    tile = (xcd < r ? xcd * (q + 1) : r * (q + 1) + (xcd - r) * q) + idx;
  }
  const int m0 = (p.m_fastest ? tile % p.tiles_m : tile / p.tiles_n) * BM;
  const int n0 = (p.m_fastest ? tile / p.tiles_m : tile % p.tiles_n) * BN;
  const int kt0 = blockIdx.z * p.kt_per_split;
  const int kt1 = min(p.nk, kt0 + p.kt_per_split);
  const int nkt = kt1 - kt0;
  float* s_rows = (float*)(smem + SMEM + TAB_BYTES);
  auto ln_gather_rows = [&]() {
    if (AMODE == MVD_A_DENSE && d.ln_stats != nullptr && tid < BM) {
      const float2 st = m0 + tid < d.M ? ln_row_stats(d, m0 + tid) : make_float2(0.f, 0.f);
      s_rows[tid * 2] = st.x;
      s_rows[tid * 2 + 1] = st.y;
    }
  };

  const int gr = lane >> 3;
  const u16* zero = (const u16*)g_zero_page;

  const u16* a_src[AI];
  bool a_ok[AI];
  int a_tab[AI], a_chunk[AI];
  int a_tail[AI];
#pragma unroll
  for (int i = 0; i < AI; ++i) {
    const int gi = wave + i * NW;
    const int R = (gi & 1) * 8 + gr;
    const int gc = (lane & 7) ^ ((R >> 1) & 7);
    const int m = m0 + gi * 8 + gr;
    a_ok[i] = m < d.M;
    a_src[i] = (const u16*)d.A + (size_t)(a_ok[i] ? m : 0) * 2 * d.lda + gc * 8;
    a_tab[i] = (gi * 8 + gr) * 9;
    a_chunk[i] = gc * 8;
    a_tail[i] = a_ok[i] ? m * 2 * d.lda2 : -1;
  }
  int* s_tab = (int*)(smem + SMEM);
  if (AMODE != MVD_A_DENSE) {
    const int hw = d.Hout * d.Wout;
    for (int e = tid; e < BM * 9; e += NW * 64) {
      const int row = e / 9, tap = e - row * 9;
      const int m = m0 + row;
      int off = -1;
      if (m < d.M) {
        const int b = m / hw;
        const int rem = m - b * hw;
        const int oy = rem / d.Wout, ox = rem - oy * d.Wout;
        const int ky = tap / 3, kx = tap - ky * 3;
        int iy, ix;
        bool ok;
        if (d.upsample) {
          const int uy = oy + ky - 1, ux = ox + kx - 1;
          ok = uy >= 0 && uy < d.Hout && ux >= 0 && ux < d.Wout;
          iy = uy >> 1;
          ix = ux >> 1;
        } else {
          iy = oy * d.stride + ky - (d.no_pad_tl ? 0 : 1);
          ix = ox * d.stride + kx - (d.no_pad_tl ? 0 : 1);
          ok = iy >= 0 && iy < d.Hin && ix >= 0 && ix < d.Win;
        }
        if (ok) off = ((b * d.Hin + iy) * d.Win + ix) * 2 * d.Cin;
      }
      s_tab[e] = off;
    }
    __syncthreads();
  }
  const u16* b_src[BI];
#pragma unroll
  for (int i = 0; i < BI; ++i) {
    const int gi = wave + i * NW;
    const int nt = (n0 >> 4) + (gi >> 1);
    if (d.b_mode == MVD_B_PLANES) {
      const int R = (gi & 1) * 8 + gr;
      const int gc = (lane & 7) ^ ((R >> 1) & 7);
      const int n = n0 + gi * 8 + gr;
      b_src[i] = (gi < B_GRAN && n < d.N) ? (const u16*)d.Wp + (size_t)n * 2 * d.ldb + gc * 8 : nullptr;
    } else {
      b_src[i] = (gi < B_GRAN && nt < p.nt16) ? (const u16*)d.Wp + (size_t)nt * 1024 + (gi & 1) * 512 + lane * 8 : nullptr;
    }
  }
  const size_t b_kstride = d.b_mode == MVD_B_PLANES ? (size_t)64 : (size_t)p.nt16 * 1024;

  const u16* a_cur[AI];
  int a_step[AI];
  int a_off[AI];
  int c_tap = 0, c_cb = 0;
  int c_kt = kt0;
  const int c_main = conv_tail_start(d);
  if (AMODE == MVD_A_DENSE) {
#pragma unroll
    for (int i = 0; i < AI; ++i) {
      a_cur[i] = a_ok[i] ? a_src[i] + (size_t)kt0 * 64 : zero;
      a_step[i] = a_ok[i] ? 64 : 0;
    }
  } else {
    c_cb = kt0 / 9;
    c_tap = kt0 - c_cb * 9;
#pragma unroll
    for (int i = 0; i < AI; ++i) a_off[i] = s_tab[a_tab[i] + c_tap];
  }
  const u16* b_cur[BI];
  size_t b_step[BI];
#pragma unroll
  for (int i = 0; i < BI; ++i) {
    b_cur[i] = b_src[i] ? b_src[i] + (size_t)kt0 * b_kstride : zero;
    b_step[i] = b_src[i] ? b_kstride : 0;
  }

  auto stage = [&](int buf) {
    unsigned char* sbase = smem + buf * STAGE;
#pragma unroll
    for (int i = 0; i < AI; ++i) {
      const u16* src;
      if (AMODE == MVD_A_DENSE) {
        src = a_cur[i];
        a_cur[i] += a_step[i];
      } else {
        const bool tail = c_kt >= c_main;
        const u16* const base = (const u16*)(tail ? d.A2 : d.A);
        const int off = tail ? a_tail[i] : a_off[i];
        src = off >= 0 ? base + (unsigned)(off + (tail ? c_kt - c_main : c_cb) * 64 + a_chunk[i]) : zero;
      }
      __builtin_amdgcn_global_load_lds((const __attribute__((address_space(1))) void*)src,
                                       (__attribute__((address_space(3))) void*)(sbase + (wave + i * NW) * 1024), 16, 0, 0);
    }
#pragma unroll
    for (int i = 0; i < BI; ++i) {
      __builtin_amdgcn_global_load_lds(
          (const __attribute__((address_space(1))) void*)b_cur[i],
          (__attribute__((address_space(3))) void*)(sbase + (A_GRAN + wave + i * NW) * 1024), 16, 0, 0);
      b_cur[i] += b_step[i];
    }
  };
  auto advance_tap = [&]() {
    if (AMODE != MVD_A_DENSE) {
      ++c_kt;
      if (++c_tap == 9) {
        c_tap = 0;
        ++c_cb;
      }
#pragma unroll
      for (int i = 0; i < AI; ++i) a_off[i] = s_tab[a_tab[i] + c_tap];
    }
  };

  f32x4 acc[TM][TN];
#pragma unroll
  for (int i = 0; i < TM; ++i)
#pragma unroll
    for (int j = 0; j < TN; ++j) acc[i][j] = (f32x4){0.f, 0.f, 0.f, 0.f};

  const int frow = lane & 15;
  const int fsw = (frow >> 1) & 7;
  const int fbase = (frow >> 3) * 1024 + (frow & 7) * 128;
  const int foff_hi = fbase + (((lane >> 4)) ^ fsw) * 16;
  const int foff_lo = fbase + ((4 + (lane >> 4)) ^ fsw) * 16;

  auto mfma_tile = [&](const op16x8 (&ah)[TM], const op16x8 (&al)[TM], const op16x8 (&bh)[TN], const op16x8 (&bl)[TN]) {
    if (NS == 4) {
#pragma unroll
      for (int i = 0; i < TM; ++i)
#pragma unroll
        for (int j = 0; j < TN; ++j) acc[i][j] = MVD_MFMA_16x16x32(al[i], bl[j], acc[i][j], 0, 0, 0);
    }
    if (NS >= 3) {
#pragma unroll
      for (int i = 0; i < TM; ++i)
#pragma unroll
        for (int j = 0; j < TN; ++j) acc[i][j] = MVD_MFMA_16x16x32(al[i], bh[j], acc[i][j], 0, 0, 0);
#pragma unroll
      for (int i = 0; i < TM; ++i)
#pragma unroll
        for (int j = 0; j < TN; ++j) acc[i][j] = MVD_MFMA_16x16x32(ah[i], bl[j], acc[i][j], 0, 0, 0);
    }
#pragma unroll
    for (int i = 0; i < TM; ++i)
#pragma unroll
      for (int j = 0; j < TN; ++j) acc[i][j] = MVD_MFMA_16x16x32(ah[i], bh[j], acc[i][j], 0, 0, 0);
  };
  const int boff_hi = d.b_mode == MVD_B_PLANES ? foff_hi : lane * 16;
  const int boff_lo = d.b_mode == MVD_B_PLANES ? foff_lo : 1024 + lane * 16;
  auto read_frags = [&](int buf, op16x8 (&ah)[TM], op16x8 (&al)[TM], op16x8 (&bh)[TN], op16x8 (&bl)[TN]) {
    const unsigned char* sA = smem + buf * STAGE;
    const unsigned char* sB = sA + A_GRAN * 1024;
#pragma unroll
    for (int i = 0; i < TM; ++i) {
      ah[i] = *(const op16x8*)(sA + (wm * TM + i) * 2048 + foff_hi);
      if (NS >= 3) al[i] = *(const op16x8*)(sA + (wm * TM + i) * 2048 + foff_lo);
    }
#pragma unroll
    for (int j = 0; j < TN; ++j) {
      bh[j] = *(const op16x8*)(sB + (wn * TN + j) * 2048 + boff_hi);
      if (NS >= 3) bl[j] = *(const op16x8*)(sB + (wn * TN + j) * 2048 + boff_lo);
    }
  };

  if (STAG) {
    const int grp = wave >> 2;
    op16x8 ah[TM], al[TM], bh[TN], bl[TN];
#pragma unroll
    for (int q = 0; q < LEAD; ++q) {
      if (q < nkt) {
        stage(q);
        advance_tap();
      }
    }
    ln_gather_rows();
    MVD_STAMP_AT(d, wave, 1);
    if (nkt >= LEAD) wait_vm_and_barrier<(LEAD - 1) * LPS>();
    else wait_vm_and_barrier<0>();
    MVD_STAMP_AT(d, wave, 2);
    for (int ph = 0; ph <= 2 * nkt; ++ph) {
      const int u = ph - grp;
      if (u >= 0 && u < 2 * nkt) {
        const int t = u >> 1;
        if ((u & 1) == 0) {
          const bool more = t + LEAD < nkt;
          if (more) {
            stage((t + LEAD) % NBUF);
            advance_tap();
          }
          read_frags(t % NBUF, ah, al, bh, bl);
          if (more) wait_vm_and_barrier<(LEAD - 1) * LPS>();
          else wait_vm_and_barrier<0>();
          continue;
        }
        mfma_tile(ah, al, bh, bl);
      }
      asm volatile("s_barrier" ::: "memory");
    }
    __syncthreads();
  } else if (PIPE) {
    op16x8 fah[2][TM], fal[2][TM], fbh[2][TN], fbl[2][TN];
#pragma unroll
    for (int q = 0; q < NBUF; ++q) {
      if (q < nkt) {
        stage(q);
        advance_tap();
      }
    }
    ln_gather_rows();
    MVD_STAMP_AT(d, wave, 1);
    if (nkt >= NBUF) wait_vm_and_barrier<(NBUF - 1) * LPS>();
    else wait_vm_and_barrier<0>();
    MVD_STAMP_AT(d, wave, 2);
    read_frags(0, fah[0], fal[0], fbh[0], fbl[0]);
    int bs = 0, br = NBUF > 1 ? 1 : 0;
    auto step = [&](auto parity, auto steady, int it) {
      constexpr int P = decltype(parity)::value;
      constexpr bool FULL = decltype(steady)::value;
      if (FULL) wait_vm_and_barrier<(NBUF - 2) * LPS>();
      else wait_vm_and_barrier<0>();
      if (FULL || it + NBUF < nkt) stage(bs);
      if (FULL || it + 1 < nkt) read_frags(br, fah[P ^ 1], fal[P ^ 1], fbh[P ^ 1], fbl[P ^ 1]);
      mfma_tile(fah[P], fal[P], fbh[P], fbl[P]);
      if (FULL) {
        constexpr int NM = TM * TN * NS, NR = (TM + TN) * (NS >= 3 ? 2 : 1);
        sched_pattern<0, LPS + NR, NM, LPS>();
      }
      if (FULL || it + NBUF < nkt) advance_tap();
      bs = bs + 1 == NBUF ? 0 : bs + 1;
      br = br + 1 == NBUF ? 0 : br + 1;
    };
    using std::integral_constant;
    int it = 0;
    for (; it + NBUF + 1 < nkt; it += 2) {
      step(integral_constant<int, 0>{}, integral_constant<bool, true>{}, it);
      step(integral_constant<int, 1>{}, integral_constant<bool, true>{}, it + 1);
    }
    unroll_steps<0, NBUF + 1>([&](auto j) {
      constexpr int J = decltype(j)::value;
      if (it + J < nkt) step(integral_constant<int, J & 1>{}, integral_constant<bool, false>{}, it + J);
    });
    __syncthreads();
  } else {
    stage(0);
    advance_tap();
    ln_gather_rows();
    MVD_STAMP_AT(d, wave, 1);
    wait_vm_and_barrier<0>();
    MVD_STAMP_AT(d, wave, 2);
    int buf = 0;
    for (int it = 0; it < nkt; ++it) {
      if (it + 1 < nkt) {
        stage(buf ^ 1);
        advance_tap();
      }
      op16x8 ah[TM], al[TM], bh[TN], bl[TN];
      read_frags(buf, ah, al, bh, bl);
      mfma_tile(ah, al, bh, bl);
      wait_vm_and_barrier<0>();
      buf ^= 1;
    }
  }

  MVD_STAMP_AT(d, wave, 3);
  tile_epilogue<BM, BN, WM, WN>(p, acc, smem, m0, n0, lane, wave, AMODE == MVD_A_DENSE && d.ln_stats != nullptr ? s_rows : nullptr);
  MVD_STAMP_AT(d, wave, 8);
}

template <int BM, int BN, int WM, int WN, int STAGES>
void launch_cfg(GemmParams& p, hipStream_t s) {
  dim3 grid(p.tiles_n * p.tiles_m, 1, p.splits), block(WM * WN * 64);
  const bool conv = p.d.a_mode == MVD_A_CONV3X3;
  const int ns = p.d.prec;
  if (!conv && ns == 4) hipLaunchKernelGGL((gemm_kernel<BM, BN, WM, WN, 4, MVD_A_DENSE, STAGES>), grid, block, 0, s, p);
  if (!conv && ns == 3) hipLaunchKernelGGL((gemm_kernel<BM, BN, WM, WN, 3, MVD_A_DENSE, STAGES>), grid, block, 0, s, p);
  if (!conv && ns == 1) hipLaunchKernelGGL((gemm_kernel<BM, BN, WM, WN, 1, MVD_A_DENSE, STAGES>), grid, block, 0, s, p);
  if (conv && ns == 4) hipLaunchKernelGGL((gemm_kernel<BM, BN, WM, WN, 4, MVD_A_CONV3X3, STAGES>), grid, block, 0, s, p);
  if (conv && ns == 3) hipLaunchKernelGGL((gemm_kernel<BM, BN, WM, WN, 3, MVD_A_CONV3X3, STAGES>), grid, block, 0, s, p);
  if (conv && ns == 1) hipLaunchKernelGGL((gemm_kernel<BM, BN, WM, WN, 1, MVD_A_CONV3X3, STAGES>), grid, block, 0, s, p);
}

}
```

### mvdfusion_amd/csrc/gemm_ws.hip

```cpp
#include "gemm_device.hpp"

namespace {

template <int BM, int BN, int CM, int CN, int NS, int AMODE>
__global__ __launch_bounds__(512) void gemm_ws_kernel(GemmParams p) {
  constexpr int NC = CM * CN, NL = 4;
  static_assert(NC == 4, "four consumer wavefronts (one per SIMD) + four loader wavefronts");
  constexpr int WTM = BM / CM, WTN = BN / CN;
  constexpr int TM = WTM / 16, TN = WTN / 16;
  constexpr int A_GRAN = BM / 8, B_GRAN = BN / 8;
  constexpr int AI = A_GRAN / NL, BI = (B_GRAN + NL - 1) / NL;
  constexpr int B_GRAN_P = BI * NL;
  constexpr int STAGE = (A_GRAN + B_GRAN_P) * 1024;
  constexpr int LPS = AI + BI;
  constexpr int LDW = WTN + 4;
  constexpr int EPI_BYTES = NC * WTM * LDW * 4;
  constexpr int TAB_BYTES = AMODE != MVD_A_DENSE ? BM * 9 * 4 : 0;
  constexpr int LNR_BYTES = AMODE == MVD_A_DENSE ? BM * 8 : 0;
  constexpr int FIT = (160 * 1024 - TAB_BYTES - LNR_BYTES) / STAGE;
  constexpr int NBUF = FIT < 8 ? FIT : 8;
  constexpr int SMEM = NBUF * STAGE > EPI_BYTES ? NBUF * STAGE : EPI_BYTES;
  static_assert(NBUF >= 3 && SMEM + TAB_BYTES + LNR_BYTES <= 160 * 1024, "LDS budget");
  static_assert(A_GRAN % NL == 0 && WTM % 16 == 0 && WTN % 16 == 0 && B_GRAN % 2 == 0, "tile geometry");
  __shared__ __attribute__((aligned(1024))) unsigned char smem[SMEM + TAB_BYTES + LNR_BYTES];

  const mvd_gemm_desc& d = p.d;
  const int tid = threadIdx.x;
  const int lane = tid & 63;
  const int wave = __builtin_amdgcn_readfirstlane(tid >> 6);
  MVD_STAMP_AT(d, wave, 0);
  int tile;
  {
    const int nb = p.tiles_n * p.tiles_m, bid = blockIdx.x;
    const int q = nb >> 3, r = nb & 7, xcd = bid & 7, idx = bid >> 3;
    tile = (xcd < r ? xcd * (q + 1) : r * (q + 1) + (xcd - r) * q) + idx;
  }
  const int m0 = (p.m_fastest ? tile % p.tiles_m : tile / p.tiles_n) * BM;
  const int n0 = (p.m_fastest ? tile / p.tiles_m : tile % p.tiles_n) * BN;
  const int kt0 = blockIdx.z * p.kt_per_split;
  const int nkt = min(p.nk, kt0 + p.kt_per_split) - kt0;
  float* s_rows = (float*)(smem + SMEM + TAB_BYTES);
  int* s_tab = (int*)(smem + SMEM);
  if (AMODE != MVD_A_DENSE) {
    const int hw = d.Hout * d.Wout;
    for (int e = tid; e < BM * 9; e += 512) {
      const int row = e / 9, tap = e - row * 9;
      const int m = m0 + row;
      int off = -1;
      if (m < d.M) {
        const int b = m / hw;
        const int rem = m - b * hw;
        const int oy = rem / d.Wout, ox = rem - oy * d.Wout;
        const int ky = tap / 3, kx = tap - ky * 3;
        int iy, ix;
        bool ok;
        if (d.upsample) {
          const int uy = oy + ky - 1, ux = ox + kx - 1;
          ok = uy >= 0 && uy < d.Hout && ux >= 0 && ux < d.Wout;
          iy = uy >> 1;
          ix = ux >> 1;
        } else {
          iy = oy * d.stride + ky - (d.no_pad_tl ? 0 : 1);
          ix = ox * d.stride + kx - (d.no_pad_tl ? 0 : 1);
          ok = iy >= 0 && iy < d.Hin && ix >= 0 && ix < d.Win;
        }
        if (ok) off = ((b * d.Hin + iy) * d.Win + ix) * 2 * d.Cin;
      }
      s_tab[e] = off;
    }
    __syncthreads();
  }

  if (wave >= NC) {
    const int lw = wave - NC;
    const int gr = lane >> 3;
    const u16* zero = (const u16*)g_zero_page;
    const u16* a_cur[AI];
    int a_step[AI], a_tab[AI], a_chunk[AI], a_off[AI], a_tail[AI];
    int c_tap = 0, c_cb = 0, c_kt = kt0;
    const int c_main = conv_tail_start(d);
#pragma unroll
    for (int i = 0; i < AI; ++i) {
      const int gi = lw + i * NL;
      const int R = (gi & 1) * 8 + gr;
      const int gc = (lane & 7) ^ ((R >> 1) & 7);
      const int m = m0 + gi * 8 + gr;
      const bool ok = m < d.M;
      a_cur[i] = ok ? (const u16*)d.A + (size_t)m * 2 * d.lda + gc * 8 + (size_t)kt0 * 64 : zero;
      a_step[i] = ok ? 64 : 0;
      a_tab[i] = (gi * 8 + gr) * 9;
      a_chunk[i] = gc * 8;
      a_tail[i] = ok ? m * 2 * d.lda2 : -1;
    }
    if (AMODE != MVD_A_DENSE) {
      c_cb = kt0 / 9;
      c_tap = kt0 - c_cb * 9;
#pragma unroll
      for (int i = 0; i < AI; ++i) a_off[i] = s_tab[a_tab[i] + c_tap];
    }
    const u16* b_cur[BI];
    size_t b_step[BI];
    {
      const size_t b_kstride = d.b_mode == MVD_B_PLANES ? (size_t)64 : (size_t)p.nt16 * 1024;
#pragma unroll
      for (int i = 0; i < BI; ++i) {
        const int gi = lw + i * NL;
        const int nt = (n0 >> 4) + (gi >> 1);
        const u16* src;
        if (d.b_mode == MVD_B_PLANES) {
          const int R = (gi & 1) * 8 + gr;
          const int gc = (lane & 7) ^ ((R >> 1) & 7);
          const int n = n0 + gi * 8 + gr;
          src = (gi < B_GRAN && n < d.N) ? (const u16*)d.Wp + (size_t)n * 2 * d.ldb + gc * 8 : nullptr;
        } else {
          src = (gi < B_GRAN && nt < p.nt16) ? (const u16*)d.Wp + (size_t)nt * 1024 + (gi & 1) * 512 + lane * 8 : nullptr;
        }
        b_cur[i] = src ? src + (size_t)kt0 * b_kstride : zero;
        b_step[i] = src ? b_kstride : 0;
      }
    }
    auto stage = [&](int buf) {
      unsigned char* sbase = smem + buf * STAGE;
#pragma unroll
      for (int i = 0; i < AI; ++i) {
        const u16* src;
        if (AMODE == MVD_A_DENSE) {
          src = a_cur[i];
          a_cur[i] += a_step[i];
        } else {
          const bool tail = c_kt >= c_main;
          const u16* const base = (const u16*)(tail ? d.A2 : d.A);
          const int off = tail ? a_tail[i] : a_off[i];
          src = off >= 0 ? base + (unsigned)(off + (tail ? c_kt - c_main : c_cb) * 64 + a_chunk[i]) : zero;
        }
        __builtin_amdgcn_global_load_lds((const __attribute__((address_space(1))) void*)src,
                                         (__attribute__((address_space(3))) void*)(sbase + (lw + i * NL) * 1024), 16, 0, 0);
      }
#pragma unroll
      for (int i = 0; i < BI; ++i) {
        __builtin_amdgcn_global_load_lds((const __attribute__((address_space(1))) void*)b_cur[i],
                                         (__attribute__((address_space(3))) void*)(sbase + (A_GRAN + lw + i * NL) * 1024), 16, 0, 0);
        b_cur[i] += b_step[i];
      }
      if (AMODE != MVD_A_DENSE) {
        ++c_kt;
        if (++c_tap == 9) {
          c_tap = 0;
          ++c_cb;
        }
#pragma unroll
        for (int i = 0; i < AI; ++i) a_off[i] = s_tab[a_tab[i] + c_tap];
      }
    };
#pragma unroll
    for (int q = 0; q < NBUF; ++q)
      if (q < nkt) stage(q);
    if (nkt >= NBUF) wait_vm_and_barrier<(NBUF - 2) * LPS>();
    else wait_vm_and_barrier<0>();
    int bs = 0;
    for (int it = 0; it < nkt; ++it) {
      asm volatile("s_barrier" ::: "memory");
      if (it + NBUF < nkt) {
        stage(bs);
        asm volatile("s_waitcnt vmcnt(%0)" ::"i"((NBUF - 2) * LPS) : "memory");
      } else {
        asm volatile("s_waitcnt vmcnt(0)" ::: "memory");
      }
      bs = bs + 1 == NBUF ? 0 : bs + 1;
    }
    __syncthreads();
    return;
  }

#if defined(MVD_WS_VARIANT) && (MVD_WS_VARIANT & 2)
  __builtin_amdgcn_s_setprio(3);
#endif
  const int cm = wave / CN, cn = wave % CN;
  if (AMODE == MVD_A_DENSE && d.ln_stats != nullptr && tid < BM) {
    const float2 st = m0 + tid < d.M ? ln_row_stats(d, m0 + tid) : make_float2(0.f, 0.f);
    s_rows[tid * 2] = st.x;
    s_rows[tid * 2 + 1] = st.y;
  }
  f32x4 acc[TM][TN];
#pragma unroll
  for (int i = 0; i < TM; ++i)
#pragma unroll
    for (int j = 0; j < TN; ++j) acc[i][j] = (f32x4){0.f, 0.f, 0.f, 0.f};
  const int frow = lane & 15;
  const int fsw = (frow >> 1) & 7;
  const int fbase = (frow >> 3) * 1024 + (frow & 7) * 128;
  const int foff_hi = fbase + (((lane >> 4)) ^ fsw) * 16;
  const int foff_lo = fbase + ((4 + (lane >> 4)) ^ fsw) * 16;
  const int boff_hi = d.b_mode == MVD_B_PLANES ? foff_hi : lane * 16;
  const int boff_lo = d.b_mode == MVD_B_PLANES ? foff_lo : 1024 + lane * 16;
  auto read_frags = [&](int buf, op16x8 (&ah)[TM], op16x8 (&al)[TM], op16x8 (&bh)[TN], op16x8 (&bl)[TN]) {
    const unsigned char* sA = smem + buf * STAGE;
    const unsigned char* sB = sA + A_GRAN * 1024;
#pragma unroll
    for (int i = 0; i < TM; ++i) {
      ah[i] = *(const op16x8*)(sA + (cm * TM + i) * 2048 + foff_hi);
      if (NS >= 3) al[i] = *(const op16x8*)(sA + (cm * TM + i) * 2048 + foff_lo);
    }
#pragma unroll
    for (int j = 0; j < TN; ++j) {
      bh[j] = *(const op16x8*)(sB + (cn * TN + j) * 2048 + boff_hi);
      if (NS >= 3) bl[j] = *(const op16x8*)(sB + (cn * TN + j) * 2048 + boff_lo);
    }
  };
  auto mfma_tile = [&](const op16x8 (&ah)[TM], const op16x8 (&al)[TM], const op16x8 (&bh)[TN], const op16x8 (&bl)[TN]) {
    if (NS == 4) {
#pragma unroll
      for (int i = 0; i < TM; ++i)
#pragma unroll
        for (int j = 0; j < TN; ++j) acc[i][j] = MVD_MFMA_16x16x32(al[i], bl[j], acc[i][j], 0, 0, 0);
    }
    if (NS >= 3) {
#pragma unroll
      for (int i = 0; i < TM; ++i)
#pragma unroll
        for (int j = 0; j < TN; ++j) acc[i][j] = MVD_MFMA_16x16x32(al[i], bh[j], acc[i][j], 0, 0, 0);
#pragma unroll
      for (int i = 0; i < TM; ++i)
#pragma unroll
        for (int j = 0; j < TN; ++j) acc[i][j] = MVD_MFMA_16x16x32(ah[i], bl[j], acc[i][j], 0, 0, 0);
    }
#pragma unroll
    for (int i = 0; i < TM; ++i)
#pragma unroll
      for (int j = 0; j < TN; ++j) acc[i][j] = MVD_MFMA_16x16x32(ah[i], bh[j], acc[i][j], 0, 0, 0);
  };
  op16x8 fah[2][TM], fal[2][TM], fbh[2][TN], fbl[2][TN];
  unsigned pf_sink = 0;
  if (d.pf_items != nullptr) {
    const int gw = (blockIdx.z * gridDim.x + blockIdx.x) * NC + wave, GW = gridDim.x * gridDim.z * NC;
    const __attribute__((address_space(4))) mvd_prefetch_item* tab = (const __attribute__((address_space(4))) mvd_prefetch_item*)d.pf_items;
    for (int it = 0; it < d.pf_n; ++it) {
      const unsigned char* base = (const unsigned char*)tab[it].ptr;
      const long lines = (long)((tab[it].bytes + 127) >> 7);
      for (long l = (long)gw * 64 + lane; l < lines; l += (long)GW * 64) {
        const unsigned char* a = base + (l << 7);
        asm volatile("global_load_dword %0, %1, off" : "+v"(pf_sink) : "v"(a) : "memory");
      }
    }
  }
  MVD_STAMP_AT(d, wave, 1);
  wait_lgkm_and_barrier();
  MVD_STAMP_AT(d, wave, 2);
  read_frags(0, fah[0], fal[0], fbh[0], fbl[0]);
  int br = 1 % NBUF;
  auto step = [&](auto parity, int it) {
    constexpr int Pq = decltype(parity)::value;
    wait_lgkm_and_barrier();
    if (it + 1 < nkt) read_frags(br, fah[Pq ^ 1], fal[Pq ^ 1], fbh[Pq ^ 1], fbl[Pq ^ 1]);
    mfma_tile(fah[Pq], fal[Pq], fbh[Pq], fbl[Pq]);
    {
      constexpr int NM = TM * TN * NS, NR = (TM + TN) * (NS >= 3 ? 2 : 1);
      sched_reads_early<0, NR, NM>();
    }
#if !defined(MVD_WS_VARIANT) || !(MVD_WS_VARIANT & 1)
    __builtin_amdgcn_sched_barrier(0);
#endif
    br = br + 1 == NBUF ? 0 : br + 1;
  };
  using std::integral_constant;
  int it = 0;
  for (; it + 2 < nkt; it += 2) {
    step(integral_constant<int, 0>{}, it);
    step(integral_constant<int, 1>{}, it + 1);
  }
  if (it < nkt) step(integral_constant<int, 0>{}, it);
  if (it + 1 < nkt) step(integral_constant<int, 1>{}, it + 1);
  MVD_STAMP_AT(d, wave, 3);
  asm volatile("s_waitcnt vmcnt(0)" ::"v"(pf_sink) : "memory");
  __syncthreads();
  tile_epilogue<BM, BN, CM, CN>(p, acc, smem, m0, n0, lane, wave, AMODE == MVD_A_DENSE && d.ln_stats != nullptr ? s_rows : nullptr);
  MVD_STAMP_AT(d, wave, 8);
}

template <int BM, int BN, int CM, int CN>
void launch_ws(GemmParams& p, hipStream_t s) {
  dim3 grid(p.tiles_n * p.tiles_m, 1, p.splits), block(512);
  const bool conv = p.d.a_mode == MVD_A_CONV3X3;
  const int ns = p.d.prec;
  if (!conv && ns == 4) hipLaunchKernelGGL((gemm_ws_kernel<BM, BN, CM, CN, 4, MVD_A_DENSE>), grid, block, 0, s, p);
  if (!conv && ns == 3) hipLaunchKernelGGL((gemm_ws_kernel<BM, BN, CM, CN, 3, MVD_A_DENSE>), grid, block, 0, s, p);
  if (!conv && ns == 1) hipLaunchKernelGGL((gemm_ws_kernel<BM, BN, CM, CN, 1, MVD_A_DENSE>), grid, block, 0, s, p);
  if (conv && ns == 4) hipLaunchKernelGGL((gemm_ws_kernel<BM, BN, CM, CN, 4, MVD_A_CONV3X3>), grid, block, 0, s, p);
  if (conv && ns == 3) hipLaunchKernelGGL((gemm_ws_kernel<BM, BN, CM, CN, 3, MVD_A_CONV3X3>), grid, block, 0, s, p);
  if (conv && ns == 1) hipLaunchKernelGGL((gemm_ws_kernel<BM, BN, CM, CN, 1, MVD_A_CONV3X3>), grid, block, 0, s, p);
}

}

bool mvd_gemm_launch_ws(int tile, GemmParams& p, hipStream_t s) {
  switch (tile) {
    case 1: launch_ws<128, 128, 2, 2>(p, s); return true;
    case 2: launch_ws<128, 80, 4, 1>(p, s); return true;
    case 4: launch_ws<128, 160, 2, 2>(p, s); return true;
  }
  return false;
}
```

### mvdfusion_amd/hip.py

```python
import ctypes as C
import os

import torch

_HERE = os.path.dirname(os.path.abspath(__file__))
LIB_PATHS = {"f16": os.path.join(_HERE, "csrc", "libmvd_hip.so"), "bf16": os.path.join(_HERE, "csrc", "libmvd_hip_bf16.so")}
if os.environ.get("MVD_HIP_LIB"):
    LIB_PATHS["f16"] = os.environ["MVD_HIP_LIB"]
LIB_PATH = LIB_PATHS["f16"]
OPERAND_FORMAT = os.environ.get("MVD_OPERAND_FORMAT", "f16")

PREC_X1, PREC_X3, PREC_X4 = 1, 3, 4
PREC_KINDS = ("conv", "skip", "proj", "qkv", "attn", "out", "geglu", "ffproj", "xattn", "ga")


def parse_precision(name):
    base, _, over = name.partition(":")
    names = {"f16": ("f16", PREC_X1), "bf16": ("bf16", PREC_X1), "f16x3": ("f16", PREC_X3), "f16x4": ("f16", PREC_X4),
             "bf16x3": ("bf16", PREC_X3), "bf16x4": ("bf16", PREC_X4)}
    if base not in names:
        raise ValueError(f"precision '{name}': base must be one of {sorted(names)}")
    fmt, default = names[base]
    policy = {}
    for item in filter(None, over.split(",")):
        k, _, v = item.partition("=")
        k = k.strip()
        if k not in PREC_KINDS or int(v) not in (PREC_X1, PREC_X3, PREC_X4):
            raise ValueError(f"precision policy '{name}': '{item}' is not <kind>=<1|3|4> with kind in {PREC_KINDS}")
        policy[k] = int(v)
    return fmt, default, policy
A_DENSE, A_CONV3X3 = 0, 1
TAPS_FULL, TAPS_CENTRE_TAIL = 0, 2
EPI_STORE, EPI_GEGLU, EPI_QKV = 0, 1, 2
ACT_NONE, ACT_GELU, ACT_SILU, ACT_QUICKGELU = 0, 1, 2, 3
STEP_STRIDE = 8
CAM_RECORD = 20
TOKEN_DIM, TOKEN_LD = 723, 736

_vp, _i, _f, _sz = C.c_void_p, C.c_int, C.c_float, C.c_size_t
c_void_p = C.c_void_p


class GemmDesc(C.Structure):
    _fields_ = [
        ("M", _i), ("N", _i), ("K", _i),
        ("A", _vp), ("lda", _i), ("a_mode", _i),
        ("B", _i), ("Hin", _i), ("Win", _i), ("Cin", _i), ("Hout", _i), ("Wout", _i), ("stride", _i), ("upsample", _i), ("no_pad_tl", _i),
        ("Wp", _vp), ("b_mode", _i), ("ldb", _i), ("acc_scale", _f), ("prec", _i),
        ("epi", _i), ("act", _i), ("out", _vp), ("ldo", _i), ("out_sp", _vp), ("ldp", _i),
        ("n_store", _i),
        ("bias", _vp), ("bias_b", _vp), ("rows_per_batch", _i), ("ldbb", _i), ("colscale", _vp), ("res", _vp), ("ldr", _i),
        ("q_hi", _vp), ("q_lo", _vp), ("k_hi", _vp), ("k_lo", _vp), ("vt_hi", _vp), ("vt_lo", _vp),
        ("heads", _i), ("dhead", _i), ("L", _i), ("Lpad", _i), ("qscale", _f),
        ("splitk", _i), ("workspace", _vp), ("workspace_elems", _sz), ("cfg", _i),
        ("gn_stats", _vp), ("gn_hw", _i), ("gn_groups", _i),
        ("rs_out", _vp), ("rs_count", _vp), ("rs_ld", _i),
        ("ln_stats", _vp), ("ln_count", _vp), ("ln_colsum", _vp), ("ln_ld", _i), ("ln_dim", _i), ("ln_eps", _f),
        ("gna_out_sp", _vp), ("gna_gamma", _vp), ("gna_beta", _vp), ("gna_eps", _f), ("gna_flags", _i),
        ("cat_b", _vp), ("cat_cb", _i), ("cat_raw_sp", _vp),
        ("acc_scale_dev", _vp), ("pf_items", _vp), ("pf_n", _i),
        ("tap_mode", _i), ("A2", _vp), ("lda2", _i), ("Cin2", _i),
    ]


class PrefetchItem(C.Structure):
    _fields_ = [("ptr", _vp), ("bytes", C.c_ulonglong), ("start_after", _i), ("consumer", _i)]


SIGNATURES = {
    "mvd_version": (_i, []),
    "mvd_last_error": (C.c_char_p, []),
    "mvd_packed_weight_bytes": (_sz, [_i, _i]),
    "mvd_operand_format": (_i, []),
    "mvd_pack_linear_weight": (_i, [_vp, _i, _i, _i, _i, _f, _vp, _vp]),
    "mvd_pack_linear_weight_t": (_i, [_vp, _i, _i, _i, _f, _vp, _vp]),
    "mvd_pack_conv3x3_weight": (_i, [_vp, _i, _i, _i, _f, _vp, _vp]),
    "mvd_gemm": (_i, [C.POINTER(GemmDesc), _vp]),
    "mvd_gemm_cfg_supported": (_i, [C.POINTER(GemmDesc), _i]),
    "mvd_split_planes": (_i, [_vp, _vp, _sz, _i, _i, _i, _vp]),
    "mvd_gemv": (_i, [_vp, _vp, _vp, _vp, _i, _i, _i, _i, _i, _i, _i, _vp]),
    "mvd_groupnorm_chunks": (_i, [_i]),
    "mvd_groupnorm_nhwc": (_i, [_vp, _vp, _vp, _vp, _i, _i, _i, _i, _f, _i, _vp, _sz, _vp]),
    "mvd_layernorm": (_i, [_vp, _vp, _vp, _vp, _vp, _i, _i, _f, _i, _vp]),
    "mvd_layernorm_groups": (_i, [_vp, _vp, _vp, _vp, _vp, _i, _i, _i, _i, _f, _i, _vp]),
    "mvd_softmax_rows": (_i, [_vp, _vp, _i, _i, _i, _f, _f, _vp]),
    "mvd_attn_qk_plane_elems": (_sz, [_i, _i, _i, _i]),
    "mvd_attn_vt_plane_elems": (_sz, [_i, _i, _i, _i]),
    "mvd_attn_lpad": (_i, [_i]),
    "mvd_attention": (_i, [_vp] * 7 + [_i, _i, _i, _i, _i, _i, _i, _vp]),
    "mvd_pixel_cross_attn": (_i, [_vp, _vp, _vp, _vp, _i, _i, _i, _i, _vp]),
    "mvd_unet_input": (_i, [_vp, _vp, _vp, _i, _i, _i, _i, _vp]),
    "mvd_unet_input_scenes": (_i, [_vp, _vp, _vp, _i, _i, _i, _i, _i, _vp]),
    "mvd_concat_channels": (_i, [_vp, _i, _vp, _i, _vp, _vp, _i, _vp, _i, _i, _vp]),
    "mvd_concat_groupnorm_fits": (_i, [_i, _i, _i, _i]),
    "mvd_concat_groupnorm": (_i, [_vp, _i, _vp, _i, _vp, _vp, _vp, _vp, _vp, _vp, _i, _i, _i, _f, _i, _vp]),
    "mvd_transpose_planes": (_i, [_vp, _i, _i, _i, _i, _vp, _i, _vp]),
    "mvd_im2col3x3_t_planes": (_i, [_vp, _i, _i, _i, _i, _vp, _i, _vp]),
    "mvd_col_sum_workspace_doubles": (_sz, [_i, _i]),
    "mvd_col_sum": (_i, [_vp, _i, _i, _i, _vp, _vp, _sz, _vp]),
    "mvd_col_sum_groups_workspace_doubles": (_sz, [_i, _i, _i]),
    "mvd_col_sum_groups": (_i, [_vp, _i, _i, _i, _i, _vp, _vp, _sz, _vp]),
    "mvd_col_sum_pow2": (_i, [_vp, _i, _i, _i, _vp, _vp, _sz, _vp, _vp, _vp]),
    "mvd_gridattn_tokens_backward": (_i, [_vp, _vp, _vp, _vp, _vp, _vp, _vp, _vp, _i, _vp, _vp, _f, _i, _i, _i, _i, _i, _f, _f, _vp]),
    "mvd_gridattn_tokens_backward_scenes": (_i, [_vp, _vp, _vp, _vp, _vp, _vp, _vp, _vp, _i, _vp, _vp, _f, _i, _i, _i, _i, _i, _i, _f, _f, _i,
                                                 _vp]),
    "mvd_gridattn_tokens_backward_window": (_i, [_vp, _vp, _vp, _vp, _vp, _vp, _vp, _vp, _i, _vp, _vp, _f, _i, _i, _i, _i, _i, _i, _f, _f, _i,
                                                 _i, _vp]),
    "mvd_layernorm_backward": (_i, [_vp, _vp, _vp, _i, _i, _f, _vp, _vp, _vp]),
    "mvd_layernorm_backward_groups": (_i, [_vp, _vp, _vp, _i, _i, _i, _i, _f, _vp, _vp, _vp, _vp, _vp, _sz, _vp]),
    "mvd_geglu_backward": (_i, [_vp, _vp, _i, _i, _vp, _vp]),
    "mvd_act_planes": (_i, [_vp, _vp, _vp, _sz, _i, _i, _i, _i, _i, _vp]),
    "mvd_act_backward": (_i, [_vp, _vp, _vp, _sz, _i, _vp]),
    "mvd_attention_backward": (_i, [_vp, _vp, _vp, _vp, _i, _i, _i, _i, _vp, _vp, _vp, _vp, _sz, _vp]),
    "mvd_pixel_cross_attn_backward": (_i, [_vp, _vp, _vp, _vp, _i, _i, _i, _i, _vp, _vp, _vp, _vp]),
    "mvd_groupnorm_backward": (_i, [_vp, _vp, _vp, _vp, _i, _i, _i, _i, _f, _i, _vp, _vp, _vp, _vp, _sz, _vp]),
    "mvd_groupnorm_from_stats": (_i, [_vp, _vp, _vp, _vp, _vp, _i, _i, _i, _i, _f, _i, _vp]),
    "mvd_area_pool": (_i, [_vp, _vp, _i, _i, _i, _i, _i, _i, _vp]),
    "mvd_fill_zero": (_i, [_vp, _sz, _vp]),
    "mvd_pow2_scale": (_i, [_vp, _sz, _vp, _vp, _vp]),
    "mvd_split_planes_scaled": (_i, [_vp, _vp, _sz, _i, _i, _i, _vp, _vp]),
    "mvd_transpose_planes_scaled": (_i, [_vp, _i, _i, _i, _vp, _i, _vp, _vp]),
    "mvd_adamw_multi": (_i, [_vp, _i, _i, _f, _f, _f, _f, _f, _f, _f, _f, _vp]),
    "mvd_timestep_embedding": (_i, [_vp, _vp, _vp, _vp, _i, _vp]),
    "mvd_timestep_embedding_scenes": (_i, [_vp, _vp, _vp, _vp, _i, _i, _i, _vp]),
    "mvd_advance_iter": (_i, [_vp, _vp]),
    "mvd_zembed": (_i, [_vp, _vp, _vp, _vp, _i, _i, _vp]),
    "mvd_gridattn_tokens": (_i, [_vp] * 10 + [_i, _i, _i, _i, _i, _f, _f, _vp]),
    "mvd_gridattn_tokens_scenes": (_i, [_vp] * 10 + [_i, _i, _i, _i, _i, _i, _f, _f, _vp]),
    "mvd_gridattn_tokens_scenes_t": (_i, [_vp] * 10 + [_i, _i, _i, _i, _i, _i, _f, _f, _i, _vp]),
    "mvd_gridattn_fused_slots": (_i, []),
    "mvd_gridattn_fused_stream_bytes": (_sz, []),
    "mvd_gridattn_fused_vec_floats": (_sz, []),
    "mvd_gridattn_fused": (_i, [_vp] * 12 + [_i, _i, _i, _i, _i, _f, _f, _i, _vp]),
    "mvd_gridattn_fused_scenes": (_i, [_vp] * 12 + [_i, _i, _i, _i, _i, _i, _f, _f, _i, _vp]),
    "mvd_gridattn_fused_scenes_t": (_i, [_vp] * 12 + [_i, _i, _i, _i, _i, _i, _f, _f, _i, _i, _i, _vp]),
    "mvd_gridattn_tokens_window": (_i, [_vp] * 10 + [_i, _i, _i, _i, _i, _i, _f, _f, _i, _i, _vp]),
    "mvd_gridattn_fused_window": (_i, [_vp] * 12 + [_i, _i, _i, _i, _i, _i, _f, _f, _i, _i, _i, _i, _vp]),
    "mvd_view_mha": (_i, [_vp, _vp, _i, _i, _i, _i, _vp]),
    "mvd_view_pool": (_i, [_vp, _vp, _vp, _vp, _i, _i, _i, _vp]),
    "mvd_cfg_ddim_update": (_i, [_vp, _i, _vp, _vp, _vp, _vp, _sz, _vp, _vp, _i, _i, _i, _f, _i, _vp]),
    "mvd_graph_begin": (_i, [_vp]),
    "mvd_graph_end": (_i, [_vp, C.POINTER(_vp)]),
    "mvd_graph_launch": (_i, [_vp, _vp]),
    "mvd_graph_destroy": (_i, [_vp]),
    "mvd_event_create": (_i, [C.POINTER(_vp)]),
    "mvd_event_record": (_i, [_vp, _vp]),
    "mvd_event_elapsed_ms": (_i, [_vp, _vp, C.POINTER(_f)]),
    "mvd_event_destroy": (_i, [_vp]),
}

_lib = None


def lib():
    global _lib
    if _lib is None:
        path = LIB_PATHS[OPERAND_FORMAT]
        if not os.path.exists(path):
            raise RuntimeError(
                f"{path} not found: build it with `python -m mvdfusion_amd.csrc.build` "
                "(or `python -c 'import __graft_entry__ as g; g.build()'`). mvdfusion_amd has no CPU fallback.")
        l = C.CDLL(path)
        for name, (res, args) in SIGNATURES.items():
            fn = getattr(l, name)
            fn.restype, fn.argtypes = res, args
        assert l.mvd_operand_format() == {"f16": 0xf16, "bf16": 0xbf16}[OPERAND_FORMAT]
        _lib = l
        load_default_tuned()
    return _lib


def set_operand_format(fmt):
    global OPERAND_FORMAT
    assert fmt in LIB_PATHS
    if _lib is not None and fmt != OPERAND_FORMAT:
        raise RuntimeError(f"operand format already fixed to {OPERAND_FORMAT} for this process")
    OPERAND_FORMAT = fmt


def check(rc):
    if rc != 0:
        raise RuntimeError(f"mvd_hip error {rc}: {lib().mvd_last_error().decode()}")


try:
    _raw_stream = torch._C._cuda_getCurrentRawStream
    _cur_device = torch._C._cuda_getDevice
except AttributeError:
    _raw_stream = None


def stream():
    if _raw_stream is not None:
        return C.c_void_p(_raw_stream(_cur_device()))
    return C.c_void_p(torch.cuda.current_stream().cuda_stream)


def ptr(t):
    if t is None:
        return None
    return C.c_void_p(t.data_ptr())


def _req(t, dtype=torch.float32):
    assert t.is_cuda and t.dtype == dtype and t.is_contiguous(), (t.device, t.dtype, t.shape, t.stride())
    return t


class PackedWeight:

    __slots__ = ("data", "N", "K", "n_real", "bias", "geglu", "conv_cin", "acc_scale", "tail_cin")

    def __init__(self, data, N, K, n_real, bias, geglu=False, conv_cin=0, acc_scale=1.0, tail_cin=0):
        self.data, self.N, self.K, self.n_real, self.bias, self.geglu, self.conv_cin = data, N, K, n_real, bias, geglu, conv_cin
        self.acc_scale = acc_scale
        self.tail_cin = tail_cin


class RowStats:

    __slots__ = ("slots", "count", "ld")

    def __init__(self, rows, n_max, device):
        self.ld = (n_max + 31) // 32
        self.slots = torch.zeros(rows, self.ld, 2, dtype=torch.float32, device=device)
        self.count = torch.zeros(1, dtype=torch.int32, device=device)


class LnFold:

    __slots__ = ("w", "colsum", "dim", "eps")

    def __init__(self, weight, bias, norm, geglu=False):
        Wd = weight.detach().double()
        g, b = norm.weight.detach().double(), norm.bias.detach().double()
        Wf = Wd * g[None, :]
        bf = Wd @ b + (bias.detach().double() if bias is not None else 0.0)
        self.w = pack_linear(Wf.float().contiguous(), bf.float().contiguous(), geglu=geglu)
        Np = self.w.N if not geglu else Wd.shape[0]
        cs = torch.zeros(max(Np, Wd.shape[0]), dtype=torch.float32, device=weight.device)
        cs[:Wd.shape[0]] = Wf.sum(dim=1).float()
        self.colsum, self.dim, self.eps = cs, int(Wd.shape[1]), float(norm.eps)


class PlanesOperand:

    __slots__ = ("data", "N", "K", "n_real", "bias", "geglu", "conv_cin", "acc_scale", "ld")

    def __init__(self, planes, N=None, K=None, bias=None, acc_scale=1.0, ld=None):
        assert planes.dtype == torch.int16 and planes.dim() == 2
        self.data, self.ld = planes, int(ld if ld is not None else planes.shape[-1] // 2)
        self.N = int(N if N is not None else planes.shape[0])
        self.K = int(K if K is not None else self.ld)
        assert self.N % 16 == 0 and self.K % 32 == 0 and self.K <= self.ld, (self.N, self.K, self.ld)
        self.n_real, self.bias, self.geglu, self.conv_cin, self.acc_scale = self.N, bias, False, 0, acc_scale


_PARAM_MAX = {}


def register_param_maxima(params):
    import weakref
    ps = [p for p in params if p.dtype == torch.float32 and p.numel() > 0]
    _PARAM_MAX.clear()
    if not ps:
        return 0
    with torch.no_grad():
        try:
            norms = torch._foreach_norm([p.detach().reshape(-1) for p in ps], float("inf"))
        except Exception:
            norms = [torch.linalg.vector_norm(p.detach().reshape(-1), ord=float("inf")) for p in ps]
        vals = torch.stack([n.reshape(()) for n in norms]).tolist()
    for p, v in zip(ps, vals):
        _PARAM_MAX[p.data_ptr()] = (weakref.ref(p), p.numel(), float(v), p._version)
    return len(ps)


def forget_param_maxima():
    _PARAM_MAX.clear()


def _known_max(t):
    ent = _PARAM_MAX.get(t.data_ptr())
    if ent is None:
        return None
    ref, numel, mx, version = ent
    p = ref()
    if p is None or p.data_ptr() != t.data_ptr() or numel != t.numel() or p._version != version:
        return None
    return mx


def _pack_scale(w, like=None):
    import math
    mx = None
    srcs = [w] if like is None else (list(like) if isinstance(like, (list, tuple)) else [like])
    known = [_known_max(s.detach()) for s in srcs]
    if all(k is not None for k in known):
        mx = max(known)
    if mx is None:
        mx = float(torch.linalg.vector_norm(w.detach().reshape(-1), ord=float("inf")))
    if not (mx > 0.0) or not math.isfinite(mx):
        return 1.0
    return 2.0 ** (10 - math.floor(math.log2(mx)))


def pack_linear(weight, bias=None, geglu=False, like=None):
    w = weight.detach().reshape(weight.shape[0], -1).contiguous().float()
    N, K = w.shape
    Np, Kp = (N + 15) // 16 * 16, (K + 31) // 32 * 32
    data = torch.empty(lib().mvd_packed_weight_bytes(N, K), dtype=torch.uint8, device=w.device)
    scale = _pack_scale(w, like if like is not None else weight)
    check(lib().mvd_pack_linear_weight(ptr(w), N, K, K, int(geglu), scale, ptr(data), stream()))
    b = None
    if bias is not None:
        b = torch.zeros(Np, dtype=torch.float32, device=w.device)
        b[:N] = bias.detach().float()
    return PackedWeight(data, Np, Kp, N, b, geglu, acc_scale=1.0 / scale)


def pack_linear_t(weight, like=None):
    w = weight.detach()
    assert w.dim() == 2 and w.dtype == torch.float32 and w.is_contiguous()
    K, N = w.shape
    Np, Kp = (N + 15) // 16 * 16, (K + 31) // 32 * 32
    data = torch.empty(lib().mvd_packed_weight_bytes(N, K), dtype=torch.uint8, device=w.device)
    scale = _pack_scale(w, like if like is not None else weight)
    check(lib().mvd_pack_linear_weight_t(ptr(w), N, K, N, scale, ptr(data), stream()))
    return PackedWeight(data, Np, Kp, N, None, False, acc_scale=1.0 / scale)


def pack_linear_cat(weights):
    return pack_linear(torch.cat([w.detach().float() for w in weights], dim=0), like=list(weights))


def pack_conv3x3(weight, bias=None, like=None):
    w = weight.detach().contiguous().float()
    Cout, Cin = w.shape[0], w.shape[1]
    cin_pad = (Cin + 31) // 32 * 32
    Np = (Cout + 15) // 16 * 16
    data = torch.empty(Np * 9 * cin_pad * 4, dtype=torch.uint8, device=w.device)
    scale = _pack_scale(w, like if like is not None else weight)
    check(lib().mvd_pack_conv3x3_weight(ptr(w), Cout, Cin, cin_pad, scale, ptr(data), stream()))
    b = None
    if bias is not None:
        b = torch.zeros(Np, dtype=torch.float32, device=w.device)
        b[:Cout] = bias.detach().float()
    return PackedWeight(data, Np, 9 * cin_pad, Cout, b, conv_cin=cin_pad, acc_scale=1.0 / scale)


def tap_schedule(cin, cin2=0):
    assert cin % 32 == 0 and cin2 % 32 == 0
    return [(0, cb, tap) for cb in range(cin // 32) for tap in range(9)] + [(1, cb, 4) for cb in range(cin2 // 32)]


def compose_conv_tail_bias(bias, tail_bias):
    if bias is None and tail_bias is None:
        return None
    terms = [t.detach().double() for t in (bias, tail_bias) if t is not None]
    return sum(terms[1:], terms[0]).float()


def pack_conv3x3_tail(weight, bias, tail_weight, tail_bias):
    w = weight.detach().contiguous().float()
    wt = tail_weight.detach().reshape(tail_weight.shape[0], -1).contiguous().float()
    Cout, Cin, Cin2 = w.shape[0], w.shape[1], wt.shape[1]
    assert wt.shape[0] == Cout
    cin_pad, cin2_pad, Np = (Cin + 31) // 32 * 32, (Cin2 + 31) // 32 * 32, (Cout + 15) // 16 * 16
    n_main = Np * 9 * cin_pad * 4
    data = torch.empty(n_main + Np * cin2_pad * 4, dtype=torch.uint8, device=w.device)
    scale = min(_pack_scale(w, weight), _pack_scale(wt, tail_weight))
    check(lib().mvd_pack_conv3x3_weight(ptr(w), Cout, Cin, cin_pad, scale, ptr(data), stream()))
    check(lib().mvd_pack_linear_weight(ptr(wt), Cout, Cin2, Cin2, 0, scale, ptr(data[n_main:]), stream()))
    bsum = compose_conv_tail_bias(bias, tail_bias)
    b = None
    if bsum is not None:
        b = torch.zeros(Np, dtype=torch.float32, device=w.device)
        b[:Cout] = bsum
    return PackedWeight(data, Np, 9 * cin_pad + cin2_pad, Cout, b, conv_cin=cin_pad, acc_scale=1.0 / scale, tail_cin=cin2_pad)


_CACHE_ATTRS = ("_p", "_pg", "_temb", "_xattn", "_head", "_pq", "_q", "_fused", "_lnf")


def params_signature(module):
    slots = module.__dict__.get("_mvd_sig_slots")
    if slots is None:
        ps, bs, seen = [], [], set()
        for m in module.modules():
            for n, p in m._parameters.items():
                if p is not None and id(p) not in seen:
                    seen.add(id(p))
                    ps.append((m._parameters, n))
            for n, b in m._buffers.items():
                if b is not None and id(b) not in seen:
                    seen.add(id(b))
                    bs.append((m._buffers, n))
        slots = module.__dict__["_mvd_sig_slots"] = (ps, bs)
    ps, bs = slots
    sig = []
    for d_, n in ps:
        p = d_.get(n)
        sig.append((p.data_ptr(), p._version) if p is not None else None)
    for d_, n in bs:
        b = d_.get(n)
        sig.append(b.data_ptr() if b is not None else None)
    return hash(tuple(sig))


def drop_packed_caches(module):
    module.__dict__.pop("_mvd_sig_slots", None)
    for m in module.modules():
        for name in _CACHE_ATTRS:
            if name in m.__dict__:
                cur = m.__dict__[name]
                if isinstance(cur, dict):
                    m.__dict__[name] = {}
                elif cur is not None:
                    m.__dict__[name] = None


def check_finite(t, what):
    if not bool(torch.isfinite(t).all()):
        raise FloatingPointError(
            f"{what}: non-finite values. mvd_hip splits GEMM operands into fp16 hi + lo (range +-65504); an activation or "
            "weight outside that range overflowed. Use precision='bf16x3' (bf16 operands, fp32 range) for such weights.")
    return t


def planes_like(rows, cols, device):
    assert cols % 32 == 0, cols
    return torch.empty(rows, 2 * cols, dtype=torch.int16, device=device)


def sp_cols(p):
    return p.shape[-1] // 2


def split_planes(x, out=None, ldp=None, scale=None):
    rows, cols = x.numel() // x.shape[-1], x.shape[-1]
    ldp = (cols + 31) // 32 * 32 if ldp is None else ldp
    if out is None:
        out = planes_like(rows, ldp, x.device)
    if scale is None:
        check(lib().mvd_split_planes(ptr(x), ptr(out), rows, cols, cols, ldp, stream()))
    else:
        check(lib().mvd_split_planes_scaled(ptr(x), ptr(out), rows, cols, cols, ldp, ptr(scale), stream()))
    return out


def gemm(A, W, out=None, *, prec=PREC_X4, M=None, lda=None, bias=True, act=ACT_NONE, res=None, colscale=None,
         bias_b=None, rows_per_batch=0, epi=EPI_STORE, conv=None, qkv=None, workspace=None, splitk=0, ldo=None,
         out_planes=None, out_planes_col=0, cfg=None, gn_stats=None, gn_hw=0, gn_groups=32, row_stats=None, ln=None, gn_apply=None, cat=None,
         acc_scale_dev=None, a2=None):
    assert A.dtype == torch.int16, "A must be in split-planes format (see hip.split_planes)"
    d = GemmDesc()
    d.N, d.K = W.N, W.K
    d.A = A.data_ptr()
    d.Wp = W.data.data_ptr()
    if isinstance(W, PlanesOperand):
        d.b_mode, d.ldb = 1, W.ld
    d.acc_scale = W.acc_scale
    if acc_scale_dev is not None:
        d.acc_scale_dev = acc_scale_dev.data_ptr()
    d.prec = prec
    if conv is not None:
        d.a_mode = A_CONV3X3
        for k in ("B", "Hin", "Win", "Cin", "Hout", "Wout", "stride", "upsample"):
            setattr(d, k, int(conv[k]))
        d.no_pad_tl = int(conv.get("no_pad_tl", 0))
        d.M = conv["B"] * conv["Hout"] * conv["Wout"]
        tail_cin = getattr(W, "tail_cin", 0)
        assert (a2 is not None) == bool(tail_cin), "a weight of pack_conv3x3_tail needs a2=, and only such a weight takes it"
        if a2 is not None:
            assert a2.dtype == torch.int16 and a2.numel() // a2.shape[-1] == d.M and a2.shape[-1] // 2 >= tail_cin
            d.tap_mode, d.A2, d.lda2, d.Cin2 = TAPS_CENTRE_TAIL, a2.data_ptr(), int(a2.shape[-1] // 2), int(tail_cin)
        assert conv["Cin"] * 9 + tail_cin == W.K, (conv["Cin"], tail_cin, W.K)
    else:
        d.a_mode = A_DENSE
        d.M = int(M if M is not None else A.numel() // A.shape[-1])
        d.lda = int(lda if lda is not None else A.shape[-1] // 2)
        assert a2 is None, "a2= (centre-tap tail) belongs to a convolution"
        assert d.lda >= W.K, f"A has {d.lda} columns, packed K is {W.K} (pad A)"
    d.epi, d.act = epi, act
    if out is not None:
        d.out = out.data_ptr()
        d.ldo = int(ldo if ldo is not None else out.shape[-1])
    if out_planes is not None:
        assert out_planes_col % 32 == 0 and out_planes.dtype == torch.int16
        d.out_sp = out_planes.data_ptr() + 4 * int(out_planes_col)
        d.ldp = int(out_planes.shape[-1] // 2)
    d.n_store = W.n_real
    if bias and W.bias is not None:
        d.bias = W.bias.data_ptr()
    if bias_b is not None:
        d.bias_b = bias_b.data_ptr()
        d.rows_per_batch = int(rows_per_batch)
        d.ldbb = bias_b.stride(0) if bias_b.dim() == 2 else 0
    if colscale is not None:
        d.colscale = colscale.data_ptr()
    if res is not None:
        d.res = res.data_ptr()
        d.ldr = int(res.shape[-1])
    if qkv is not None:
        qh, ql, kh, kl, vh, vl = qkv["planes"]
        d.q_hi, d.q_lo, d.k_hi, d.k_lo, d.vt_hi, d.vt_lo = (t.data_ptr() for t in (qh, ql, kh, kl, vh, vl))
        d.heads, d.dhead, d.L = qkv["heads"], qkv["dhead"], qkv["L"]
        d.Lpad = lib().mvd_attn_lpad(qkv["L"])
        d.qscale = float(qkv["dhead"]) ** -0.5 * 1.4426950408889634
    if gn_stats is not None:
        d.gn_stats, d.gn_hw, d.gn_groups = gn_stats.data_ptr(), int(gn_hw), int(gn_groups)
    if gn_apply is not None:
        gamma, beta, eps, flags, planes = gn_apply
        ct = d.N + (cat[0].shape[-1] if cat is not None else 0)
        assert gn_stats is not None and out is not None and planes.dtype == torch.int16 and planes.shape[-1] == 2 * ct
        if cat is not None:
            skip, raw = cat
            assert skip.dtype == torch.float32 and skip.is_contiguous() and skip.shape[0] == d.M and (raw is None or raw.shape[-1] == 2 * ct)
            d.cat_b, d.cat_cb, d.cat_raw_sp = skip.data_ptr(), int(skip.shape[-1]), (raw.data_ptr() if raw is not None else None)
        d.gna_gamma, d.gna_beta, d.gna_eps, d.gna_flags, d.gna_out_sp = gamma.data_ptr(), beta.data_ptr(), float(eps), int(flags), planes.data_ptr()
    if row_stats is not None:
        assert row_stats.slots.shape[0] >= d.M and row_stats.ld >= (d.N + 31) // 32
        d.rs_out, d.rs_count, d.rs_ld = row_stats.slots.data_ptr(), row_stats.count.data_ptr(), row_stats.ld
    if ln is not None:
        rs, fold = ln
        d.ln_stats, d.ln_count, d.ln_ld = rs.slots.data_ptr(), rs.count.data_ptr(), rs.ld
        d.ln_colsum, d.ln_dim, d.ln_eps = fold.colsum.data_ptr(), fold.dim, fold.eps
        splitk = 1
    d.splitk = splitk
    if workspace is not None:
        d.workspace = workspace.data_ptr()
        d.workspace_elems = workspace.numel()
    key = (d.M, d.N, d.K, d.a_mode, d.Cin, d.stride, d.upsample, d.no_pad_tl, d.epi, d.prec, res is not None, out is not None,
           out_planes is not None, splitk, d.b_mode, row_stats is not None, ln is not None, gn_apply is not None, cat[0].shape[-1] if cat is not None else 0,
           d.tap_mode, d.Cin2)
    if cfg is None:
        tuned = _TUNED.get(key)
        if tuned is None and AUTOTUNE and 2.0 * d.M * d.N * d.K >= AUTOTUNE_MIN_FLOPS:
            tuned = _autotune(d, A if A.is_contiguous() else None, W_data=W.data if not isinstance(W, PlanesOperand) else None)
            _TUNED[key] = tuned
            global TUNED_IN_RUN
            TUNED_IN_RUN += 1
        if tuned is not None:
            cfg, d.splitk = tuned
    d.cfg = cfg or 0
    global LAST_CFG
    LAST_CFG = d.cfg
    if GEMM_SEQUENCE is not None:
        GEMM_SEQUENCE.note(d, W)
    check(lib().mvd_gemm(C.byref(d), stream()))
    return out


GEMM_SEQUENCE = None
SELF_PREFETCH_MIN = int(os.environ.get("MVD_SELF_PREFETCH_MIN", "0"))


class WeightPrefetcher:

    def __init__(self, device, window=24 << 20, max_items=24, gn_hosts=0, self_min=None):
        self.device = device
        self.window, self.max_items = int(window), int(max_items)
        self.self_min = int(SELF_PREFETCH_MIN if self_min is None else self_min)
        self.gn_hosts = bool(gn_hosts)
        self.seq, self.recording, self.table, self.n, self.launch_idx, self.shares = [], False, None, 0, 0, {}

    class _Following:
        def __init__(self, pf, record):
            self.pf, self.record = pf, record

        def __enter__(self):
            global GEMM_SEQUENCE
            self.prev, GEMM_SEQUENCE = GEMM_SEQUENCE, self.pf
            self.pf.recording = self.record
            self.pf.launch_idx = 0
            if self.record:
                self.pf.seq = []
            return self.pf

        def __exit__(self, *exc):
            global GEMM_SEQUENCE
            GEMM_SEQUENCE = self.prev
            if self.record and exc[0] is None:
                self.pf._build()
            self.pf.recording = False
            return False

    def following(self, record=False):
        return WeightPrefetcher._Following(self, record)

    def note(self, d, W):
        j = self.launch_idx
        self.launch_idx += 1
        is_ws = bool(d.cfg) and _cfg_parts(d.cfg)[1] == WS_LOOP
        host = 1 if is_ws else (2 if (d.gna_out_sp and d.splitk != 1 and self.gn_hosts) else 0)
        if self.recording:
            packed = not isinstance(W, PlanesOperand)
            self.seq.append((W.data.data_ptr(), W.data.numel() * W.data.element_size(), host) if packed else (0, 0, host))
            return
        if host and j in self.shares:
            first, n = self.shares[j]
            d.pf_items, d.pf_n = self.table.data_ptr() + first * C.sizeof(PrefetchItem), n

    def _build(self):
        items = []
        self.shares = {}
        hosts = [j for j, e in enumerate(self.seq) if e[2]]
        sure = [j for j, e in enumerate(self.seq) if e[2] == 1]
        for j in hosts:
            nxt = [k for k in sure if k > j]
            end = nxt[0] if nxt else len(self.seq) - 1
            first, acc, seen = len(items), 0, set()
            if self.self_min > 0 and self.seq[j][2] == 1 and self.seq[j][1] >= self.self_min:
                items.append((self.seq[j][0], self.seq[j][1], j, j))
                seen.add(self.seq[j][0])
            for k in range(j + 1, end + 1):
                ptr_, nbytes, _ = self.seq[k]
                if not nbytes or ptr_ in seen or acc + nbytes > self.window or len(items) - first >= self.max_items:
                    continue
                seen.add(ptr_)
                acc += nbytes
                items.append((ptr_, nbytes, j, k))
            if len(items) > first:
                self.shares[j] = (first, len(items) - first)
        self.n = len(items)
        arr = (PrefetchItem * max(self.n, 1))()
        for i, (ptr_, nbytes, sa, cons) in enumerate(items):
            arr[i].ptr, arr[i].bytes, arr[i].start_after, arr[i].consumer = ptr_, nbytes, sa, cons
        self.table = torch.frombuffer(bytearray(bytes(arr)), dtype=torch.uint8).clone().to(self.device)
        self.items = items


CFG_STRIDE = 32
GNA_SILU, GNA_ROUND_F16, GNA_OUT_UNUSED = 1, 2, 4
TUNE_CACHE_VERSION = 12
GEMM_TILES = ((64, 64, 2, 2), (128, 128, 2, 4), (128, 80, 4, 1), (64, 80, 4, 1), (128, 160, 4, 2))
GEMM_LOOPS = (2, 3, 4, None, 6, 7, "patch", "ws")
REMOVED_LOOPS = tuple(i for i, l in enumerate(GEMM_LOOPS) if l is None)
PATCH_LOOP = 6
WS_LOOP = 7


def _cfg_parts(cfg):
    return (cfg - 1) // CFG_STRIDE, ((cfg - 1) % CFG_STRIDE) >> 1, (cfg - 1) & 1


def make_cfg(tile, loop, order=0):
    return 1 + CFG_STRIDE * tile + 2 * loop + order


def _cfg_valid(cfg, epi, b_mode=0):
    tile, loop, _ = _cfg_parts(cfg)
    if loop >= len(GEMM_LOOPS):
        return False
    bm, bn, wm, wn = GEMM_TILES[tile]
    waves = wm * wn
    return loop not in REMOVED_LOOPS and (loop != 2 or waves == 8) and (loop != 5 or waves == 4) and \
        (loop != PATCH_LOOP or tile in (1, 2, 4)) and (tile < 2 or epi == EPI_STORE) and \
        (loop != WS_LOOP or tile == 1 or (tile in (2, 4) and epi == EPI_STORE))


_ALL_CONFIGS = tuple(c for c in range(1, CFG_STRIDE * len(GEMM_TILES) + 1) if _cfg_valid(c, EPI_STORE))
GEMM_CONFIGS = tuple(c for c in _ALL_CONFIGS if _cfg_parts(c)[1] != PATCH_LOOP)
PATCH_CONFIGS = tuple(c for c in _ALL_CONFIGS if _cfg_parts(c)[1] == PATCH_LOOP)
GEMM_CONFIGS_CONV = GEMM_CONFIGS + PATCH_CONFIGS


def gemm_configs(epi=EPI_STORE, b_mode=0, conv=False):
    return tuple(c for c in (GEMM_CONFIGS_CONV if conv else GEMM_CONFIGS) if _cfg_valid(c, epi, b_mode))


def cfg_supported(d, cfg):
    return bool(lib().mvd_gemm_cfg_supported(C.byref(d), cfg))


def kernel_symbol(cfg, prec, conv):
    if not cfg:
        return f"gemm_kernel<auto, {prec}, {1 if conv else 0}>"
    tile, loop, _ = _cfg_parts(cfg)
    bm, bn, wm, wn = GEMM_TILES[tile]
    if loop == PATCH_LOOP:
        return f"conv_patch_kernel<{bm}, {bn}, {wm}, {wn}, {prec}>"
    if loop == WS_LOOP:
        cm, cn = {1: (2, 2), 2: (4, 1), 4: (2, 2)}[tile]
        return f"gemm_ws_kernel<{bm}, {bn}, {cm}, {cn}, {prec}, {1 if conv else 0}>"
    return f"gemm_kernel<{bm}, {bn}, {wm}, {wn}, {prec}, {1 if conv else 0}, {GEMM_LOOPS[loop]}>"


def gemm_fingerprint():
    import glob
    import hashlib
    h = hashlib.sha256()
    root = os.path.dirname(_HERE)
    pats = ("mvdfusion_amd/csrc/gemm*.hip", "mvdfusion_amd/csrc/gemm*.hpp", "mvdfusion_amd/csrc/common.hpp")
    for f in sorted(f for pat in pats for f in glob.glob(os.path.join(root, pat))):
        h.update(os.path.relpath(f, root).encode())
        h.update(open(f, "rb").read())
    return h.hexdigest()[:16]


def default_tuned_path(fmt=None):
    return os.path.join(_HERE, "tuned", f"gemm_{fmt or OPERAND_FORMAT}.json")


TUNED_IN_RUN = 0
TUNED_SOURCE = None


def load_default_tuned():
    global TUNED_SOURCE
    env = os.environ.get("MVD_TUNE_CACHE", "")
    if env == "0":
        TUNED_SOURCE = "none (MVD_TUNE_CACHE=0): tuned in this run"
        return 0
    path = env or default_tuned_path()
    if not os.path.exists(path):
        TUNED_SOURCE = f"none ({os.path.relpath(path, os.path.dirname(_HERE))} missing): tuned in this run"
        return 0
    n = load_tuned(path, require_fingerprint=os.environ.get("MVD_TUNE_CACHE_ANY") != "1")
    rel = os.path.relpath(path, os.path.dirname(_HERE))
    TUNED_SOURCE = f"{rel}: {n} problems" if n else f"none ({rel} was tuned on other GEMM sources or another cfg encoding): tuned in this run"
    return n


def save_tuned(path, merge=False):
    import json
    entries = {}
    if merge and os.path.exists(path):
        doc = json.load(open(path))
        if _tuned_doc_ok(doc) and doc.get("gemm_fingerprint") == gemm_fingerprint():
            entries = {tuple(k): tuple(v) for k, v in doc["entries"]}
    entries.update(_TUNED)
    os.makedirs(os.path.dirname(os.path.abspath(path)), exist_ok=True)
    with open(path, "w") as f:
        json.dump({"version": TUNE_CACHE_VERSION, "cfg_stride": CFG_STRIDE, "operand_format": OPERAND_FORMAT,
                   "gemm_fingerprint": gemm_fingerprint(),
                   "entries": sorted([list(k), list(v)] for k, v in entries.items())}, f, indent=0)


def _tuned_doc_ok(doc):
    return isinstance(doc, dict) and doc.get("version") == TUNE_CACHE_VERSION and doc.get("cfg_stride") == CFG_STRIDE and \
        doc.get("operand_format") == OPERAND_FORMAT


def load_tuned(path, require_fingerprint=False):
    import json
    doc = json.load(open(path))
    if not _tuned_doc_ok(doc) or (require_fingerprint and doc.get("gemm_fingerprint") != gemm_fingerprint()):
        return 0
    n = 0
    for k, v in doc["entries"]:
        cfg = int(v[0])
        if cfg != 0 and not (1 <= cfg <= CFG_STRIDE * len(GEMM_TILES) and _cfg_parts(cfg)[1] < len(GEMM_LOOPS) and
                             _cfg_parts(cfg)[1] not in REMOVED_LOOPS):
            continue
        _TUNED[tuple(k)] = tuple(v)
        n += 1
    return n


LAST_CFG = 0
AUTOTUNE = False
AUTOTUNE_MIN_FLOPS = 0.0
_TUNED = {}


_TRASH = None
TUNE_SPLITS = os.environ.get("MVD_TUNE_SPLITS") == "1"
TUNE_COLD = True


def _flush_caches():
    global _TRASH
    if _TRASH is None:
        _TRASH = torch.zeros(160 * 1024 * 1024, dtype=torch.float32, device="cuda")
    _TRASH.add_(1.0)


def release_tuning_buffers():
    global _TRASH
    _TRASH = None


_TUNE_STATS = {}


def _autotune(d, A=None, reps=4, trials=int(os.environ.get("MVD_TUNE_TRIALS", "3")), W_data=None):
    best, best_ms = (0, d.splitk), float("inf")
    e0, e1 = Event(), Event()
    stats_ptr, d.gn_stats = d.gn_stats, None
    if d.gna_out_sp:
        n = (d.M // d.gn_hw) * d.gn_groups * 2
        n = (n, str(A.device) if A is not None else "cuda")
        scratch = _TUNE_STATS.get(n)
        if scratch is None:
            scratch = _TUNE_STATS[n] = torch.zeros(n[0], dtype=torch.int64, device=A.device if A is not None else "cuda")
        d.gn_stats = scratch.data_ptr()
    skip = set()
    skip |= {int(t) for t in os.environ.get("MVD_TUNE_EXCLUDE_LOOPS", "").split(",") if t}
    fixed_split = d.splitk
    cands = [(c, sk) for c in gemm_configs(d.epi, d.b_mode, conv=d.a_mode == A_CONV3X3) if cfg_supported(d, c) and _cfg_parts(c)[1] not in skip
             for sk in ((0, 1) if d.splitk == 0 else (d.splitk,))]
    timed, second_pass = [], False
    wp0 = d.Wp
    rot = [wp0]
    if TUNE_COLD and A is not None and d.b_mode == 0:
        if W_data is not None and W_data.data_ptr() == wp0:
            rot += [W_data.clone(), W_data.clone()]
    ptrs = [wp0] + [t.data_ptr() for t in rot[1:]]
    for cfg, sk in cands:
        d.cfg, d.splitk = cfg, sk
        check(lib().mvd_gemm(C.byref(d), stream()))
        ms = float("inf")
        if TUNE_COLD and A is not None:
            for _ in range(trials + 1):
                _flush_caches()
                A.view(-1)[:A.numel() // 2 * 2].view(torch.int32).sum()
                e0.record()
                for wp in ptrs:
                    d.Wp = wp
                    check(lib().mvd_gemm(C.byref(d), stream()))
                e1.record()
                ms = min(ms, e0.elapsed_ms(e1) / len(ptrs))
            d.Wp = wp0
        else:
            for _ in range(trials):
                e0.record()
                for _ in range(reps):
                    check(lib().mvd_gemm(C.byref(d), stream()))
                e1.record()
                ms = min(ms, e0.elapsed_ms(e1))
        if sk != 1:
            ms += 0.0015
        timed.append((ms, cfg, sk))
        if ms < best_ms * 0.99:
            best, best_ms = (cfg, sk), ms
        if len(timed) == len(cands) and TUNE_SPLITS and fixed_split == 0 and not second_pass:
            second_pass = True
            nk = d.K // 32
            extra = [s_ for s_ in (2, 3, 4, 6, 8, 12, 16, 24, 32) if s_ <= max(1, nk // 2)]
            top = sorted(timed)[:3]
            cands.extend((c, s_) for _, c, _ in top for s_ in extra if (c, s_) not in cands)
    d.gn_stats = stats_ptr
    return best


def gemv(W, bias, x, y, act_in=ACT_NONE, act_out=ACT_NONE):
    M, K = x.shape
    N = W.shape[0]
    check(lib().mvd_gemv(ptr(W), ptr(bias), ptr(x), ptr(y), M, N, K, x.stride(0), y.stride(0), act_in, act_out, stream()))
    return y


def groupnorm(x, y, gamma, beta, B, HW, Cc, eps, silu, ws):
    check(lib().mvd_groupnorm_nhwc(ptr(x), ptr(y), ptr(gamma), ptr(beta), B, HW, Cc, 32, eps, int(silu), ptr(ws), ws.numel(),
                                   stream()))
    return y


def groupnorm_from_stats(x, y, gamma, beta, stats, B, HW, Cc, eps, silu, groups=32):
    check(lib().mvd_groupnorm_from_stats(ptr(x), ptr(y), ptr(gamma), ptr(beta), ptr(stats), B, HW, Cc, groups, eps, int(silu), stream()))
    return y


def layernorm(x, y, w, b, rows, Cc, eps=1e-5, w_plus_one=False, y_f32=None):
    check(lib().mvd_layernorm(ptr(x), ptr(y), ptr(y_f32), ptr(w), ptr(b), rows, Cc, eps, int(w_plus_one), stream()))
    return y


def layernorm_groups(x, y, w, b, rows, Cc, rows_per_group, eps=1e-5, w_plus_one=False, y_f32=None):
    assert w.stride(0) == b.stride(0) and w.stride(-1) == 1 and b.stride(-1) == 1, (w.stride(), b.stride())
    check(lib().mvd_layernorm_groups(ptr(x), ptr(y), ptr(y_f32), ptr(w), ptr(b), w.stride(0), rows, int(rows_per_group), Cc, eps,
                                     int(w_plus_one), stream()))
    return y


def softmax_rows(x, y, scale=1.0, out_scale=1.0):
    rows, cols = x.shape
    check(lib().mvd_softmax_rows(ptr(x), ptr(y), rows, cols, x.stride(0), float(scale), float(out_scale), stream()))
    return y


def attention(planes, out, B, heads, L, dhead, prec=PREC_X4, Lkeys=0):
    qh, ql, kh, kl, vh, vl = planes
    check(lib().mvd_attention(ptr(qh), ptr(ql), ptr(kh), ptr(kl), ptr(vh), ptr(vl), ptr(out), out.shape[-1] // 2, B, heads,
                              L, Lkeys, dhead, prec, stream()))
    return out


def alloc_attn_planes(B, heads, L, dhead, device):
    nqk = lib().mvd_attn_qk_plane_elems(B, heads, L, dhead)
    nvt = lib().mvd_attn_vt_plane_elems(B, heads, L, dhead)
    mk = lambda n: torch.zeros(n, dtype=torch.int16, device=device)
    return (mk(nqk), mk(nqk), mk(nqk), mk(nqk), mk(nvt), mk(nvt))


class Graph:

    def __init__(self):
        self.exec = C.c_void_p()

    def __enter__(self):
        self._side = torch.cuda.Stream()
        self._side.wait_stream(torch.cuda.current_stream())
        self._ctx = torch.cuda.stream(self._side)
        self._ctx.__enter__()
        check(lib().mvd_graph_begin(stream()))
        return self

    def __exit__(self, et, ev, tb):
        rc = lib().mvd_graph_end(stream(), C.byref(self.exec))
        self._ctx.__exit__(et, ev, tb)
        torch.cuda.current_stream().wait_stream(self._side)
        if et is None:
            check(rc)
        return False

    def launch(self):
        check(lib().mvd_graph_launch(self.exec, stream()))

    def __del__(self):
        try:
            if self.exec:
                lib().mvd_graph_destroy(self.exec)
        except Exception:
            pass


class Event:
    def __init__(self):
        self.h = C.c_void_p()
        check(lib().mvd_event_create(C.byref(self.h)))

    def record(self):
        check(lib().mvd_event_record(self.h, stream()))

    def elapsed_ms(self, stop):
        ms = C.c_float()
        check(lib().mvd_event_elapsed_ms(self.h, stop.h, C.byref(ms)))
        return ms.value
```

### mvdfusion_amd/unet.py

```python
import math

import torch
import torch.nn as nn

from . import hip
from .attention import SpatialTransformer, ViewAlignedFeatureTransformer
from .engine import Ctx


class GroupNorm32(nn.GroupNorm):
    pass


def normalization(channels):
    return GroupNorm32(32, channels)


class TimestepBlock(nn.Module):
    pass


class Upsample(nn.Module):
    def __init__(self, channels, use_conv, dims=2, out_channels=None, padding=1):
        super().__init__()
        self.channels, self.out_channels = channels, out_channels or channels
        self.conv = nn.Conv2d(self.channels, self.out_channels, 3, padding=padding)
        self._p = None

    def run(self, ctx, x, H, W, out=None):
        if self._p is None:
            self._p = hip.pack_conv3x3(self.conv.weight, self.conv.bias)
        if out is None:
            out = ctx.act((ctx.B * 4 * H * W, self.out_channels))
        xp = hip.split_planes(x, ctx.ws.planes("updown.x", ctx.B * H * W, self.channels))
        ctx.gemm(xp, self._p, out, conv=dict(B=ctx.B, Hin=H, Win=W, Cin=self.channels, Hout=2 * H, Wout=2 * W,
                                            stride=1, upsample=1), gn=(ctx.B, 4 * H * W), kind="conv")
        return out, 2 * H, 2 * W


class Downsample(nn.Module):
    def __init__(self, channels, use_conv, dims=2, out_channels=None, padding=1):
        super().__init__()
        self.channels, self.out_channels = channels, out_channels or channels
        self.op = nn.Conv2d(self.channels, self.out_channels, 3, stride=2, padding=padding)
        self._p = None

    def run(self, ctx, x, H, W, out=None):
        if self._p is None:
            self._p = hip.pack_conv3x3(self.op.weight, self.op.bias)
        Ho, Wo = H // 2, W // 2
        if out is None:
            out = ctx.act((ctx.B * Ho * Wo, self.out_channels))
        xp = hip.split_planes(x, ctx.ws.planes("updown.x", ctx.B * H * W, self.channels))
        ctx.gemm(xp, self._p, out, conv=dict(B=ctx.B, Hin=H, Win=W, Cin=self.channels, Hout=Ho, Wout=Wo, stride=2,
                                            upsample=0), gn=(ctx.B, Ho * Wo), kind="conv")
        return out, Ho, Wo


class ResBlock(TimestepBlock):

    def __init__(self, channels, emb_channels, dropout, out_channels=None, dims=2, use_checkpoint=False,
                 use_scale_shift_norm=False):
        super().__init__()
        assert not use_scale_shift_norm
        self.channels, self.out_channels = channels, out_channels or channels
        self.in_layers = nn.Sequential(normalization(channels), nn.SiLU(),
                                       nn.Conv2d(channels, self.out_channels, 3, padding=1))
        self.emb_layers = nn.Sequential(nn.SiLU(), nn.Linear(emb_channels, self.out_channels))
        self.out_layers = nn.Sequential(normalization(self.out_channels), nn.SiLU(), nn.Dropout(p=dropout),
                                        nn.Conv2d(self.out_channels, self.out_channels, 3, padding=1))
        self.skip_connection = nn.Identity() if self.out_channels == channels else \
            nn.Conv2d(channels, self.out_channels, 1)
        self._p = None

    def packed(self, fuse_skip=True):
        c1, c2, sk = self.in_layers[2], self.out_layers[3], self.skip_connection
        fuse = bool(fuse_skip) and not isinstance(sk, nn.Identity)
        if self._p is None:
            self._p = (hip.pack_conv3x3(c1.weight, None), None, None)
        if self._p[1] is None or bool(self._p[1].tail_cin) != fuse:
            w2 = hip.pack_conv3x3_tail(c2.weight, c2.bias, sk.weight, sk.bias) if fuse else hip.pack_conv3x3(c2.weight, c2.bias)
            wsk = None if fuse or isinstance(sk, nn.Identity) else hip.pack_linear(sk.weight, sk.bias)
            self._p = (self._p[0], w2, wsk)
        return self._p

    def run(self, ctx, x, H, W, out=None, x_planes=None):
        B, Ci, Co = ctx.B, self.channels, self.out_channels
        M = B * H * W
        w1, w2, wsk = self.packed(fuse_skip=ctx.prec_of("skip") == ctx.prec_of("conv"))
        geo = dict(B=B, Hin=H, Win=W, Hout=H, Wout=W, stride=1, upsample=0)
        a = ctx.ws.planes("res.a", M, Ci)
        ctx.groupnorm(x, a, self.in_layers[0], B, H * W, Ci, silu=True)
        h = ctx.ws.get("res.h", (M, Co))
        a2 = ctx.ws.planes("res.a2", M, Co)
        eb = ctx.emb_bias[self]
        ctx.gemm(a, w1, h, conv=dict(Cin=Ci, **geo), bias=False, bias_b=eb, rows_per_batch=M // eb.shape[0],
                 gn=(B, H * W), kind="conv",
                 gn_apply=(self.out_layers[0], a2, True, True))
        if (wsk is not None or w2.tail_cin) and x_planes is None:
            x_planes = hip.split_planes(x, ctx.ws.planes("res.xp", M, Ci))
        if out is None:
            out = ctx.act((M, Co))
        if w2.tail_cin:
            ctx.gemm(a2, w2, out, conv=dict(Cin=Co, **geo), a2=x_planes, gn=(B, H * W), kind="conv")
            return out
        skip = x
        if wsk is not None:
            skip = ctx.ws.get("res.skip", (M, Co))
            ctx.gemm(x_planes, wsk, skip, kind="skip")
        ctx.gemm(a2, w2, out, conv=dict(Cin=Co, **geo), res=skip, gn=(B, H * W), kind="conv")
        return out


def gn_hint(layer):
    from .attention import SpatialTransformer, ViewAlignedFeatureTransformer
    if isinstance(layer, tuple):
        return layer
    if isinstance(layer, ResBlock):
        return layer.in_layers[0], "res.a", True
    if isinstance(layer, SpatialTransformer):
        return layer.norm, "tf.n", False
    if isinstance(layer, ViewAlignedFeatureTransformer):
        return layer.aligned_attn_norm, "tf.n", False
    return None


class TimestepEmbedSequential(nn.Sequential, TimestepBlock):
    def run(self, ctx, x, H, W, out=None, x_planes=None, next_layer=None, next_cat=None):
        n = len(self)
        for i, layer in enumerate(self):
            dst = out if i == n - 1 else None
            ctx.next_gn = gn_hint(self[i + 1] if i + 1 < n else next_layer)
            ctx.next_cat = next_cat if i == n - 1 else None
            if isinstance(layer, (Upsample, Downsample)):
                x, H, W = layer.run(ctx, x, H, W, out=dst)
            elif isinstance(layer, ResBlock):
                x = layer.run(ctx, x, H, W, out=dst, x_planes=x_planes if i == 0 else None)
            else:
                x = layer.run(ctx, x, H, W, out=dst)
            ctx.next_gn = None
            ctx.next_cat = None
        return x, H, W


class _StemConv(nn.Conv2d):
    _p = None

    def run(self, ctx, x, H, W, out):
        if self._p is None:
            self._p = hip.pack_conv3x3(self.weight, self.bias)
        ctx.gemm(x, self._p, out, conv=dict(B=ctx.B, Hin=H, Win=W, Cin=self._p.conv_cin, Hout=H, Wout=W, stride=1,
                                            upsample=0), gn=(ctx.B, H * W), kind="conv")
        return out


class UNetModel(nn.Module):
    def __init__(self, image_size, in_channels, model_channels, out_channels, num_res_blocks, attention_resolutions,
                 dropout=0, channel_mult=(1, 2, 4, 8), conv_resample=True, dims=2, num_classes=None,
                 use_checkpoint=False, use_fp16=False, num_heads=-1, num_head_channels=-1, num_heads_upsample=-1,
                 use_scale_shift_norm=False, resblock_updown=False, use_new_attention_order=False,
                 use_spatial_transformer=True, use_view_aligned_transformer=True, transformer_depth=1,
                 context_dim=None, n_embed=None, legacy=True):
        super().__init__()
        assert use_view_aligned_transformer and use_spatial_transformer and context_dim is not None
        assert dims == 2 and num_classes is None and not resblock_updown and n_embed is None and conv_resample
        assert num_heads != -1 and num_head_channels == -1, "this build supports the num_heads form (configs/*.yaml)"
        if isinstance(context_dim, (list, tuple)) or type(context_dim).__name__ == "ListConfig":
            context_dim = list(context_dim)[0]
        channel_mult = tuple(channel_mult)
        attention_resolutions = tuple(attention_resolutions)
        self.image_size, self.in_channels, self.model_channels = image_size, in_channels, model_channels
        self.out_channels, self.num_res_blocks, self.channel_mult = out_channels, num_res_blocks, channel_mult
        self.attention_resolutions, self.num_heads, self.context_dim = attention_resolutions, num_heads, context_dim
        ted = model_channels * 4
        self.time_embed = nn.Sequential(nn.Linear(model_channels, ted), nn.SiLU(), nn.Linear(ted, ted))

        def res(cin, cout):
            return ResBlock(cin, ted, dropout, out_channels=cout, use_checkpoint=use_checkpoint)

        def st(c):
            return SpatialTransformer(c, num_heads, c // num_heads, depth=transformer_depth, context_dim=context_dim)

        def vaft(c):
            return ViewAlignedFeatureTransformer(c, num_heads, c // num_heads, depth=transformer_depth,
                                                 context_dim=context_dim, image_size=image_size)

        self.input_blocks = nn.ModuleList([TimestepEmbedSequential(_StemConv(in_channels, model_channels, 3, padding=1))])
        skip_chans = [model_channels]
        ch, ds = model_channels, 1
        for level, mult in enumerate(channel_mult):
            for _ in range(num_res_blocks):
                layers = [res(ch, mult * model_channels)]
                ch = mult * model_channels
                if ds in attention_resolutions:
                    layers.append(st(ch))
                self.input_blocks.append(TimestepEmbedSequential(*layers))
                skip_chans.append(ch)
            if level != len(channel_mult) - 1:
                self.input_blocks.append(TimestepEmbedSequential(Downsample(ch, True, out_channels=ch)))
                skip_chans.append(ch)
                ds *= 2
        self.middle_block = TimestepEmbedSequential(res(ch, ch), st(ch), vaft(ch), res(ch, ch))
        self.output_blocks = nn.ModuleList([])
        for level, mult in list(enumerate(channel_mult))[::-1]:
            for i in range(num_res_blocks + 1):
                layers = [res(ch + skip_chans.pop(), model_channels * mult)]
                ch = model_channels * mult
                if ds in attention_resolutions:
                    layers += [st(ch), vaft(ch)]
                if level and i == num_res_blocks:
                    layers.append(Upsample(ch, True, out_channels=ch))
                    ds //= 2
                self.output_blocks.append(TimestepEmbedSequential(*layers))
        self.out = nn.Sequential(normalization(ch), nn.SiLU(), nn.Conv2d(model_channels, out_channels, 3, padding=1))
        self._head = None
        self._temb = None
        self._xattn = None
        self._head_saved = None
        self._record = None

    def get_cross_attn_parameters(self, finetune_cross_attn, finetune_view_attn):
        out = []
        for name, p in self.named_parameters():
            if finetune_cross_attn and any(k in name for k in (".norm.", ".proj_in.", ".transformer_blocks.", ".proj_out.")):
                out.append(p)
            if finetune_view_attn and ".aligned_attn_" in name:
                out.append(p)
        return out

    def disable_unet_grad(self):
        for name, p in self.named_parameters():
            if ".aligned_attn_" not in name:
                p.requires_grad_(False)

    def _resblocks(self):
        return [m for m in self.modules() if isinstance(m, ResBlock)]

    def time_biases(self, ctx, t_sin):
        if self._temb is None:
            blocks = self._resblocks()
            w = torch.cat([b.emb_layers[1].weight.detach() for b in blocks], 0).contiguous()
            bias = torch.cat([b.emb_layers[1].bias.detach() + b.in_layers[2].bias.detach() for b in blocks], 0).contiguous()
            offs, o = {}, 0
            for b in blocks:
                offs[b] = (o, o + b.out_channels)
                o += b.out_channels
            self._temb = (w, bias, offs)
        w, bias, offs = self._temb
        ted = self.model_channels * 4
        R = t_sin.shape[0]
        e1, emb = ctx.ws.get("temb.e1", (R, ted)), ctx.ws.get("temb.emb", (R, ted))
        out = ctx.ws.get("temb.bias", (R, w.shape[0]))
        ctx.gemv_rows(self.time_embed[0].weight, self.time_embed[0].bias, t_sin, e1, act_out=hip.ACT_SILU)
        ctx.gemv_rows(self.time_embed[2].weight, self.time_embed[2].bias, e1, emb)
        ctx.gemv_rows(w, bias, emb, out, act_in=hip.ACT_SILU)
        ctx.emb_bias = {b: out[:, lo:hi] for b, (lo, hi) in offs.items()}

    def cross_attn_vectors(self, ctx):
        if self._xattn is None:
            sts = [m for m in self.modules() if isinstance(m, SpatialTransformer)]
            ws, bs, offs, o = [], [], {}, 0
            for st in sts:
                a2 = st.transformer_blocks[0].attn2
                wo, wv = a2.to_out[0].weight.detach().double(), a2.to_v.weight.detach().double()
                ws.append((wo @ wv).float())
                bs.append(a2.to_out[0].bias.detach().float())
                offs[st] = (o, o + st.in_channels)
                o += st.in_channels
            self._xattn = (torch.cat(ws, 0).contiguous(), torch.cat(bs, 0).contiguous(), offs, o)
        w, bias, offs, total = self._xattn
        out = ctx.ws.get("xattn.vec", (ctx.context.shape[0], total))
        ctx.gemv_rows(w, bias, ctx.context, out)
        ctx.xattn_vec = {st: out[:, lo:hi] for st, (lo, hi) in offs.items()}

    def run(self, ctx, x_in, t_sin, S):
        B = ctx.B
        self.time_biases(ctx, t_sin)
        self.cross_attn_vectors(ctx)
        hs = []
        H = W = S
        h = x_in
        rec = self._record
        for bi, blk in enumerate(self.input_blocks):
            if rec is not None:
                rec.append((blk, h.clone(), H, W, 0))
            if bi == 0:
                o = ctx.ws.get("hs0", (B * H * W, self.model_channels))
                ctx.next_gn = gn_hint(self.input_blocks[1][0])
                h = blk[0].run(ctx, h, H, W, o)
                ctx.next_gn = None
            else:
                last = blk[-1]
                Ho, Wo = (H // 2, W // 2) if isinstance(last, Downsample) else (H, W)
                co = last.out_channels if isinstance(last, (ResBlock, Downsample)) else last.in_channels
                o = ctx.ws.get(f"hs{bi}", (B * Ho * Wo, co))
                nxt = self.input_blocks[bi + 1][0] if bi + 1 < len(self.input_blocks) else self.middle_block[0]
                h, H, W = blk.run(ctx, h, H, W, out=o, next_layer=nxt)
            hs.append((h, H, W))
        if rec is not None:
            rec.append((self.middle_block, h.clone(), H, W, 0))
        keep = rec is not None or ctx.keep_fp32

        def cat_hint(nblk, co, Hn, Wn):
            first = nblk[0]
            if keep or not isinstance(first, ResBlock) or isinstance(first.skip_connection, nn.Identity):
                return None
            nsk = hs[-1][0]
            Mn = B * Hn * Wn
            return (nsk, ctx.ws.get("cat", (Mn, co + nsk.shape[-1])), ctx.ws.planes("catp", Mn, co + nsk.shape[-1])) + gn_hint(first)

        def out_geometry(blk, H, W):
            last = blk[-1]
            co = last.out_channels if isinstance(last, (ResBlock, Upsample)) else last.in_channels
            return (co, 2 * H, 2 * W) if isinstance(last, Upsample) else (co, H, W)

        h, H, W = self.middle_block.run(ctx, h, H, W, next_cat=cat_hint(self.output_blocks[0], *out_geometry(self.middle_block, H, W)))
        for bi, blk in enumerate(self.output_blocks):
            sk, _, _ = hs.pop()
            M = B * H * W
            ca, cb = h.shape[-1], sk.shape[-1]
            cat = ctx.ws.get("cat", (M, ca + cb))
            catp = ctx.ws.planes("catp", M, ca + cb)
            first = blk[0]
            if cat.data_ptr() in ctx._cat_done:
                ctx._cat_done.discard(cat.data_ptr())
            else:
                need_cat = keep or not isinstance(first, ResBlock) or isinstance(first.skip_connection, nn.Identity)
                ctx.concat(h, ca, sk, cb, cat, catp, B, H * W, gn_apply=gn_hint(first), need_out=need_cat)
            if rec is not None:
                rec.append((blk, cat.clone(), H, W, ca))
            last_blk = bi + 1 == len(self.output_blocks)
            h, H, W = blk.run(ctx, cat, H, W, x_planes=catp, next_layer=(self.out[0], "res.a", True) if last_blk else None,
                              next_cat=None if last_blk else cat_hint(self.output_blocks[bi + 1], *out_geometry(blk, H, W)))
        if self._head is None:
            self._head = hip.pack_conv3x3(self.out[2].weight, self.out[2].bias)
        M = B * H * W
        a = ctx.ws.planes("res.a", M, self.model_channels)
        ctx.groupnorm(h, a, self.out[0], B, H * W, self.model_channels, silu=True)
        y = ctx.ws.get("head", (M, 8))
        ctx.gemm(a, self._head, y, conv=dict(B=B, Hin=H, Win=W, Cin=self.model_channels, Hout=H, Wout=W, stride=1,
                                             upsample=0), ldo=8, kind="conv")
        self._head_saved = (h, a)
        return y


class UNetWrapper(nn.Module):

    def __init__(self, unet_config, unet_path=None, drop_conditions=False, drop_scheme="default", use_zero_123=False,
                 finetune_unet=False, finetune_cross_attn=False, finetune_view_attn=True, remove_keys=()):
        super().__init__()
        params = unet_config.get("params", unet_config) if hasattr(unet_config, "get") else unet_config
        self.unet_model = UNetModel(**dict(params))
        if unet_path:
            from .load_model import load_unet_checkpoint
            load_unet_checkpoint(self.unet_model, unet_path, remove_keys=remove_keys)
        if not finetune_unet:
            self.unet_model.disable_unet_grad()
        self.drop_conditions, self.drop_scheme, self.use_zero_123 = drop_conditions, drop_scheme, use_zero_123
        self.finetune_unet, self.finetune_cross_attn, self.finetune_view_attn = \
            finetune_unet, finetune_cross_attn, finetune_view_attn

    def get_trainable_parameters(self):
        if self.finetune_unet:
            return self.unet_model.parameters()
        return self.unet_model.get_cross_attn_parameters(finetune_cross_attn=self.finetune_cross_attn,
                                                         finetune_view_attn=self.finetune_view_attn)

    def level_channels(self):
        u = self.unet_model
        return [u.model_channels * m for m in u.channel_mult]

    def level0_operand(self, ctx, B, S, D):
        rows = B * S * S * D
        if D == 1:
            c0 = self.level_channels()[0]
            return ctx.ws.get("ovol0", (rows, 2 * (c0 + 768)), torch.int16, zero=True), c0
        return ctx.ws.get("vol0", (rows, 2 * 768), torch.int16, zero=True), 0

    def volume_pyramid(self, ctx, vol, B, S, D):
        levels = [self.level0_operand(ctx, B, S, D)]
        Cc = vol.shape[-1]
        chans = self.level_channels()
        for i in range(1, len(self.unet_model.channel_mult)):
            f = 2 ** i
            rows = B * (S // f) * (S // f) * D
            if D == 1:
                ld, col = chans[i] + Cc, chans[i]
                o = ctx.ws.get(f"ovol{i}", (rows, 2 * ld), torch.int16, zero=True)
            else:
                ld, col = Cc, 0
                o = ctx.ws.planes(f"vol{i}", rows, Cc)
            hip.check(hip.lib().mvd_area_pool(hip.ptr(vol), hip.c_void_p(o.data_ptr() + 4 * col), B, S, D, Cc, f, ld, hip.stream()))
            levels.append((o, col))
        return levels
```

Baseline: 120.0 steps/s.

## Fold nearest-2x upsample into four-tap sub-pixel convolution weights

Adds a four-tap conv mode for upsample+3x3 conv. Each output parity class sees the nearest-upsampled input through a 2x2 effective kernel, so weights are pre-combined per parity and the GEMM runs K=4*Cin over input-resolution rows, with tile rows scattered back to output rows in the epilogue. This cuts the conv FLOPs and A-operand gathers for upsample convs by about 9/4. The cost is four packed weight copies, a row remap in the epilogue, and restricting the mode to the plain store epilogue.

Measured after the change: 122.1 steps/s (median of 6 runs). 1.8% higher.

```diff
diff --git a/include/mvd_hip.h b/include/mvd_hip.h
--- a/include/mvd_hip.h
+++ b/include/mvd_hip.h
@@ -108,6 +108,7 @@
   int lda2, Cin2;
 } mvd_gemm_desc;
 #define MVD_TAPS_FULL 0
+#define MVD_TAPS_UP4 1
 #define MVD_TAPS_CENTRE_TAIL 2
 #define MVD_GNA_SILU 1
 #define MVD_GNA_ROUND_F16 2
diff --git a/mvdfusion_amd/csrc/gemm.hip b/mvdfusion_amd/csrc/gemm.hip
--- a/mvdfusion_amd/csrc/gemm.hip
+++ b/mvdfusion_amd/csrc/gemm.hip
@@ -378,6 +378,7 @@
   const int tile = (cfg - 1) / MVD_GEMM_CFG_STRIDE, loop = ((cfg - 1) % MVD_GEMM_CFG_STRIDE) >> 1;
   if (loop >= MVD_GEMM_LOOPS) return false;
   if (tile >= 2 && d.epi != MVD_EPI_STORE) return false;
+  if (d.a_mode == MVD_A_CONV3X3 && d.tap_mode == MVD_TAPS_UP4 && (d.epi != MVD_EPI_STORE || !d.upsample)) return false;
   const int waves = kTiles[tile].waves;
   if ((loop == 2 || loop == 3) && waves != 8) return false;
   if (loop == 3 || loop >= 8) return false;
@@ -395,6 +396,7 @@
   MVD_CHECK_ARG(dp != nullptr, "mvd_gemm: null descriptor");
   GemmParams p;
   p.d = *dp;
+  p.up4_tpp = p.up4_mq = 0;
   mvd_gemm_desc& d = p.d;
   MVD_CHECK_ARG(d.M > 0 && d.N > 0 && d.K > 0, "mvd_gemm: bad sizes M=%d N=%d K=%d", d.M, d.N, d.K);
   MVD_CHECK_ARG(d.K % 32 == 0, "mvd_gemm: K=%d must be a multiple of 32 (pad the packed weight)", d.K);
@@ -403,8 +405,19 @@
   MVD_CHECK_ARG(d.A && d.Wp, "mvd_gemm: null operand");
   MVD_CHECK_ARG(((uintptr_t)d.A & 127) == 0 && ((uintptr_t)d.Wp & 127) == 0, "mvd_gemm: operands must be 128-byte aligned");
   if (d.a_mode == MVD_A_CONV3X3) {
-    MVD_CHECK_ARG(d.tap_mode == MVD_TAPS_FULL || d.tap_mode == MVD_TAPS_CENTRE_TAIL, "mvd_gemm: tap_mode %d is not served", d.tap_mode);
-    const bool tail = d.tap_mode == MVD_TAPS_CENTRE_TAIL;
+    MVD_CHECK_ARG(d.tap_mode == MVD_TAPS_FULL || d.tap_mode == MVD_TAPS_CENTRE_TAIL || d.tap_mode == MVD_TAPS_UP4,
+                  "mvd_gemm: tap_mode %d is not served", d.tap_mode);
+    const bool tail = d.tap_mode == MVD_TAPS_CENTRE_TAIL, up4 = d.tap_mode == MVD_TAPS_UP4;
+    if (up4) {
+      MVD_CHECK_ARG(d.upsample == 1 && d.stride == 1 && !d.no_pad_tl && d.b_mode == MVD_B_PACKED,
+                    "mvd_gemm: tap_mode MVD_TAPS_UP4 (the four-tap form) serves stride-1 padded convolutions behind a nearest-2x upsample with a packed weight");
+      MVD_CHECK_ARG(d.epi == MVD_EPI_STORE, "mvd_gemm: tap_mode MVD_TAPS_UP4 (the four-tap form) serves MVD_EPI_STORE only (epi=%d)", d.epi);
+      MVD_CHECK_ARG(!d.res && !d.bias_b && !d.colscale && !d.rs_out,
+                    "mvd_gemm: tap_mode MVD_TAPS_UP4 (the four-tap form) takes no res, bias_b, colscale or rs_out (its tile rows are not output rows)");
+      if (d.gn_stats)
+        MVD_CHECK_ARG((d.Hin * d.Win) % 16 == 0, "mvd_gemm: tap_mode MVD_TAPS_UP4 (the four-tap form) with gn_stats needs Hin * Win %% 16 == 0 (Hin=%d Win=%d)", d.Hin,
+                      d.Win);
+    }
     if (tail) {
       MVD_CHECK_ARG(d.A2 != nullptr && ((uintptr_t)d.A2 & 127) == 0 && d.Cin2 > 0 && d.Cin2 % 32 == 0 && d.lda2 >= d.Cin2 && d.lda2 % 32 == 0,
                     "mvd_gemm: the centre-tap tail needs A2 (128-byte aligned), Cin2 %% 32 == 0 and lda2 >= Cin2, a multiple of 32 (Cin2=%d lda2=%d)",
@@ -413,9 +426,9 @@
                     "mvd_gemm: the centre-tap tail serves stride-1 padded convolutions with Hin == Hout, Win == Wout and a packed weight");
       MVD_CHECK_ARG((long long)d.M * 2 * d.lda2 < (1ll << 31), "mvd_gemm: A2 is addressed with 32-bit offsets (M=%d lda2=%d)", d.M, d.lda2);
     }
-    MVD_CHECK_ARG(d.Cin % 32 == 0 && d.K == 9 * d.Cin + (tail ? d.Cin2 : 0),
-                  "mvd_gemm: conv needs Cin %% 32 == 0 and K == 9*Cin (+ Cin2 with a centre-tap tail) (Cin=%d Cin2=%d K=%d)", d.Cin,
-                  tail ? d.Cin2 : 0, d.K);
+    MVD_CHECK_ARG(d.Cin % 32 == 0 && d.K == (up4 ? 4 : 9) * d.Cin + (tail ? d.Cin2 : 0),
+                  "mvd_gemm: conv needs Cin %% 32 == 0 and K == 9*Cin (+ Cin2 with a centre-tap tail; 4*Cin in the four-tap form) (Cin=%d Cin2=%d K=%d)",
+                  d.Cin, tail ? d.Cin2 : 0, d.K);
     MVD_CHECK_ARG(d.M == d.B * d.Hout * d.Wout, "mvd_gemm: conv M mismatch");
     MVD_CHECK_ARG(d.stride == 1 || d.stride == 2, "mvd_gemm: conv stride must be 1 or 2");
     if (d.upsample) MVD_CHECK_ARG(d.stride == 1 && d.Hout == 2 * d.Hin && d.Wout == 2 * d.Win, "mvd_gemm: upsample geometry");
@@ -497,10 +510,17 @@
   const TileInfo& ti = kTiles[tile];
   p.tiles_n = cdiv(d.N, ti.bn);
   p.tiles_m = cdiv(d.M, ti.bm);
+  const bool up4 = d.a_mode == MVD_A_CONV3X3 && d.tap_mode == MVD_TAPS_UP4;
+  if (up4) {
+    p.up4_mq = d.B * d.Hin * d.Win;
+    p.up4_tpp = cdiv(p.up4_mq, ti.bm);
+    p.tiles_m = 4 * p.up4_tpp;
+  }
   if (order < 0) {
+    const int est_tm = up4 ? p.up4_tpp : p.tiles_m;
     const double W = (double)d.N * d.K * 4.0;
-    const double A = (double)d.M * d.K * 4.0 / (d.a_mode == MVD_A_CONV3X3 ? 9.0 : 1.0);
-    const double rep_m = p.tiles_m < 8 ? p.tiles_m : 8, rep_n = p.tiles_n < 8 ? p.tiles_n : 8;
+    const double A = (double)(up4 ? p.up4_mq : d.M) * d.K * 4.0 / (d.a_mode == MVD_A_CONV3X3 ? (up4 ? 4.0 : 9.0) : 1.0);
+    const double rep_m = est_tm < 8 ? est_tm : 8, rep_n = p.tiles_n < 8 ? p.tiles_n : 8;
     order = (W + A * rep_n) < (W * rep_m + A) ? 1 : 0;
   }
   p.m_fastest = order;
diff --git a/mvdfusion_amd/csrc/gemm_common.hpp b/mvdfusion_amd/csrc/gemm_common.hpp
--- a/mvdfusion_amd/csrc/gemm_common.hpp
+++ b/mvdfusion_amd/csrc/gemm_common.hpp
@@ -10,6 +10,7 @@
   int splits;
   int tiles_m, tiles_n;
   int m_fastest;
+  int up4_tpp, up4_mq;
 };
 
 __device__ __forceinline__ float gemm_acc_scale(const mvd_gemm_desc& d) {
diff --git a/mvdfusion_amd/csrc/gemm_device.hpp b/mvdfusion_amd/csrc/gemm_device.hpp
--- a/mvdfusion_amd/csrc/gemm_device.hpp
+++ b/mvdfusion_amd/csrc/gemm_device.hpp
@@ -101,6 +101,62 @@
   return d.tap_mode == MVD_TAPS_CENTRE_TAIL ? 9 * (d.Cin >> 5) : 0x7fffffff;
 }
 
+__device__ __forceinline__ int conv_taps_per_block(const mvd_gemm_desc& d) { return d.tap_mode == MVD_TAPS_UP4 ? 4 : 9; }
+
+struct TileCoord {
+  int m0, n0, par;
+};
+template <int BM, int BN>
+__device__ __forceinline__ TileCoord tile_coord(const GemmParams& p, int tile) {
+  int par = -1, tpm = p.tiles_m;
+  if (p.up4_tpp) {
+    tpm = p.up4_tpp;
+    const int per = tpm * p.tiles_n;
+    par = tile / per;
+    tile -= par * per;
+  }
+  return {(p.m_fastest ? tile % tpm : tile / p.tiles_n) * BM, (p.m_fastest ? tile / tpm : tile % p.tiles_n) * BN, par};
+}
+
+__device__ __forceinline__ int conv_tap_offset(const mvd_gemm_desc& d, int par, int m, int tap) {
+  int b, iy, ix;
+  bool ok;
+  if (par >= 0) {
+    const int hw = d.Hin * d.Win;
+    b = m / hw;
+    const int rem = m - b * hw;
+    const int i = rem / d.Win, j = rem - i * d.Win;
+    iy = i - 1 + (par >> 1) + (tap >> 1);
+    ix = j - 1 + (par & 1) + (tap & 1);
+    ok = tap < 4 && iy >= 0 && iy < d.Hin && ix >= 0 && ix < d.Win;
+  } else {
+    const int hw = d.Hout * d.Wout;
+    b = m / hw;
+    const int rem = m - b * hw;
+    const int oy = rem / d.Wout, ox = rem - oy * d.Wout;
+    const int ky = tap / 3, kx = tap - ky * 3;
+    if (d.upsample) {
+      const int uy = oy + ky - 1, ux = ox + kx - 1;
+      ok = uy >= 0 && uy < d.Hout && ux >= 0 && ux < d.Wout;
+      iy = uy >> 1;
+      ix = ux >> 1;
+    } else {
+      iy = oy * d.stride + ky - (d.no_pad_tl ? 0 : 1);
+      ix = ox * d.stride + kx - (d.no_pad_tl ? 0 : 1);
+      ok = iy >= 0 && iy < d.Hin && ix >= 0 && ix < d.Win;
+    }
+  }
+  return ok ? ((b * d.Hin + iy) * d.Win + ix) * 2 * d.Cin : -1;
+}
+
+__device__ __forceinline__ int epi_out_row(const mvd_gemm_desc& d, int par, int m) {
+  if (par < 0) return m;
+  const int hw = d.Hin * d.Win;
+  const int b = m / hw, rem = m - b * hw;
+  const int i = rem / d.Win, j = rem - i * d.Win;
+  return (b * d.Hout + 2 * i + (par >> 1)) * d.Wout + 2 * j + (par & 1);
+}
+
 #define MVD_PATCH_SLOTS_MAX 288
 __host__ __device__ constexpr int conv_patch_ring(int bn, int waves) {
   const int bstage = ((bn / 8 + waves - 1) / waves) * waves;
@@ -142,13 +198,14 @@
 
 template <int BM, int BN, int WM, int WN>
 __device__ __forceinline__ void tile_epilogue(const GemmParams& p, f32x4 (&acc)[BM / WM / 16][BN / WN / 16], unsigned char* smem, int m0,
-                                              int n0, int lane, int wave, const float* s_rows = nullptr) {
+                                              int n0, int lane, int wave, const float* s_rows = nullptr, int par = -1) {
   constexpr int WTM = BM / WM, WTN = BN / WN;
   constexpr int TM = WTM / 16, TN = WTN / 16;
   constexpr int LDW = WTN + 4;
   constexpr int C4 = WTN / 4;
   const mvd_gemm_desc& d = p.d;
   const int wm = wave / WN, wn = wave % WN;
+  const int Mlim = par >= 0 ? p.up4_mq : d.M;
   float* sC = (float*)smem + wave * (WTM * LDW);
   MVD_STAMP_AT(d, wave, 4);
   {
@@ -175,7 +232,8 @@
       const int idx = ps * 64 + lane;
       const int row = idx / C4, col = (idx - row * C4) * 4;
       const int m = wm0 + row, n = wn0 + col;
-      if (idx < WTM * C4 && m < d.M && n < d.N) *(float4*)(ws + (size_t)m * d.N + n) = *(const float4*)(sC + row * LDW + col);
+      if (idx < WTM * C4 && m < Mlim && n < d.N)
+        *(float4*)(ws + (size_t)epi_out_row(d, par, m) * d.N + n) = *(const float4*)(sC + row * LDW + col);
     }
     return;
   }
@@ -331,7 +389,7 @@
   const int mrow0 = wm0 + lrow;
   const bool lane_ok = lane < RPC * C4 && n + 3 < d.n_store;
   float* const sL = sC + lrow * LDW + lcol;
-  const int rows_ok = min(WTM - lrow, d.M - mrow0);
+  const int rows_ok = min(WTM - lrow, Mlim - mrow0);
   auto pass1 = [&](auto act_c, auto res_c, auto bb_c) {
     constexpr int ACT = decltype(act_c)::value;
     constexpr bool HAS_RES = decltype(res_c)::value, HAS_BB = decltype(bb_c)::value;
@@ -407,11 +465,23 @@
 #pragma unroll 1
       for (int ps = 0; ps * RPC < rows_ok; ++ps)
 #pragma unroll 1
-        for (int e = 0; e < 4; ++e) epi_store_elem(d, mrow0 + ps * RPC, n + e, sL[ps * (RPC * LDW) + e]);
+        for (int e = 0; e < 4; ++e) epi_store_elem(d, epi_out_row(d, par, mrow0 + ps * RPC), n + e, sL[ps * (RPC * LDW) + e]);
     }
   }
   MVD_STAMP_AT(d, wave, 9);
-  if (lane_ok) {
+  if (lane_ok && par >= 0) {
+#pragma unroll 1
+    for (int p0 = 0; p0 * RPC < rows_ok; p0 += 4) {
+      float4 f[4];
+#pragma unroll
+      for (int j = 0; j < 4; ++j) f[j] = *(const float4*)(sL + ((p0 + j) * RPC < rows_ok ? p0 + j : 0) * (RPC * LDW));
+#pragma unroll
+      for (int j = 0; j < 4; ++j) {
+        if ((p0 + j) * RPC >= rows_ok) break;
+        epi_put4(d, epi_out_row(d, par, mrow0 + (p0 + j) * RPC), n, f[j]);
+      }
+    }
+  } else if (lane_ok) {
     float* po = d.out ? d.out + (size_t)mrow0 * d.ldo + n : nullptr;
     u16* psp = d.out_sp ? (u16*)d.out_sp + sp_index((size_t)mrow0, d.ldp, n) : nullptr;
     const size_t ostep = (size_t)RPC * d.ldo, sstep = (size_t)RPC * 2 * d.ldp;
@@ -476,12 +546,13 @@
         if (len > WTN - col) len = WTN - col;
         if (len > d.n_store - n) len = d.n_store - n;
       }
-      const bool whole = d.gn_hw % WTM == 0;
+      const int img_rows = par >= 0 ? d.Hin * d.Win : d.gn_hw;
+      const bool whole = img_rows % WTM == 0;
       float s1 = 0.f, q1 = 0.f;
 #pragma unroll 1
       for (int sl = 0; sl < WTM / 16; ++sl) {
         const int ms = wm0 + sl * 16;
-        if (ms >= d.M) break;
+        if (ms >= Mlim) break;
         if (!whole) s1 = q1 = 0.f;
         if (okc) {
 #pragma unroll
@@ -491,7 +562,7 @@
             q1 += v * v;
           }
         }
-        if (whole && sl + 1 < WTM / 16 && ms + 16 < d.M) continue;
+        if (whole && sl + 1 < WTM / 16 && ms + 16 < Mlim) continue;
         float ss = s1, qq = q1;
         for (int j = 1; j < jmax; ++j) {
           const float ts = __shfl_down(s1, j, 64), tq = __shfl_down(q1, j, 64);
@@ -500,7 +571,7 @@
             qq += tq;
           }
         }
-        if (leader) gn_stats_add(d.gn_stats, ms / d.gn_hw, gidx, d.gn_groups, ss, qq);
+        if (leader) gn_stats_add(d.gn_stats, ms / img_rows, gidx, d.gn_groups, ss, qq);
       }
     }
   }
diff --git a/mvdfusion_amd/csrc/gemm_plain.hpp b/mvdfusion_amd/csrc/gemm_plain.hpp
--- a/mvdfusion_amd/csrc/gemm_plain.hpp
+++ b/mvdfusion_amd/csrc/gemm_plain.hpp
@@ -45,8 +45,11 @@
     const int q = nb >> 3, r = nb & 7, xcd = bid & 7, idx = bid >> 3;
     tile = (xcd < r ? xcd * (q + 1) : r * (q + 1) + (xcd - r) * q) + idx;
   }
-  const int m0 = (p.m_fastest ? tile % p.tiles_m : tile / p.tiles_n) * BM;
-  const int n0 = (p.m_fastest ? tile / p.tiles_m : tile % p.tiles_n) * BN;
+  const TileCoord tc = tile_coord<BM, BN>(p, tile);
+  const int m0 = tc.m0, n0 = tc.n0;
+  const int par = AMODE != MVD_A_DENSE ? tc.par : -1;
+  const int mlim = par >= 0 ? p.up4_mq : d.M;
+  const u16* const wp = (const u16*)d.Wp + (par > 0 ? (size_t)par * p.nk * p.nt16 * 1024 : (size_t)0);
   const int kt0 = blockIdx.z * p.kt_per_split;
   const int kt1 = min(p.nk, kt0 + p.kt_per_split);
   const int nkt = kt1 - kt0;
@@ -72,7 +75,7 @@
     const int R = (gi & 1) * 8 + gr;
     const int gc = (lane & 7) ^ ((R >> 1) & 7);
     const int m = m0 + gi * 8 + gr;
-    a_ok[i] = m < d.M;
+    a_ok[i] = m < mlim;
     a_src[i] = (const u16*)d.A + (size_t)(a_ok[i] ? m : 0) * 2 * d.lda + gc * 8;
     a_tab[i] = (gi * 8 + gr) * 9;
     a_chunk[i] = gc * 8;
@@ -80,31 +83,10 @@
   }
   int* s_tab = (int*)(smem + SMEM);
   if (AMODE != MVD_A_DENSE) {
-    const int hw = d.Hout * d.Wout;
     for (int e = tid; e < BM * 9; e += NW * 64) {
       const int row = e / 9, tap = e - row * 9;
       const int m = m0 + row;
-      int off = -1;
-      if (m < d.M) {
-        const int b = m / hw;
-        const int rem = m - b * hw;
-        const int oy = rem / d.Wout, ox = rem - oy * d.Wout;
-        const int ky = tap / 3, kx = tap - ky * 3;
-        int iy, ix;
-        bool ok;
-        if (d.upsample) {
-          const int uy = oy + ky - 1, ux = ox + kx - 1;
-          ok = uy >= 0 && uy < d.Hout && ux >= 0 && ux < d.Wout;
-          iy = uy >> 1;
-          ix = ux >> 1;
-        } else {
-          iy = oy * d.stride + ky - (d.no_pad_tl ? 0 : 1);
-          ix = ox * d.stride + kx - (d.no_pad_tl ? 0 : 1);
-          ok = iy >= 0 && iy < d.Hin && ix >= 0 && ix < d.Win;
-        }
-        if (ok) off = ((b * d.Hin + iy) * d.Win + ix) * 2 * d.Cin;
-      }
-      s_tab[e] = off;
+      s_tab[e] = m < mlim ? conv_tap_offset(d, par, m, tap) : -1;
     }
     __syncthreads();
   }
@@ -119,7 +101,7 @@
       const int n = n0 + gi * 8 + gr;
       b_src[i] = (gi < B_GRAN && n < d.N) ? (const u16*)d.Wp + (size_t)n * 2 * d.ldb + gc * 8 : nullptr;
     } else {
-      b_src[i] = (gi < B_GRAN && nt < p.nt16) ? (const u16*)d.Wp + (size_t)nt * 1024 + (gi & 1) * 512 + lane * 8 : nullptr;
+      b_src[i] = (gi < B_GRAN && nt < p.nt16) ? wp + (size_t)nt * 1024 + (gi & 1) * 512 + lane * 8 : nullptr;
     }
   }
   const size_t b_kstride = d.b_mode == MVD_B_PLANES ? (size_t)64 : (size_t)p.nt16 * 1024;
@@ -130,6 +112,7 @@
   int c_tap = 0, c_cb = 0;
   int c_kt = kt0;
   const int c_main = conv_tail_start(d);
+  const int c_ntap = conv_taps_per_block(d);
   if (AMODE == MVD_A_DENSE) {
 #pragma unroll
     for (int i = 0; i < AI; ++i) {
@@ -137,8 +120,8 @@
       a_step[i] = a_ok[i] ? 64 : 0;
     }
   } else {
-    c_cb = kt0 / 9;
-    c_tap = kt0 - c_cb * 9;
+    c_cb = kt0 / c_ntap;
+    c_tap = kt0 - c_cb * c_ntap;
 #pragma unroll
     for (int i = 0; i < AI; ++i) a_off[i] = s_tab[a_tab[i] + c_tap];
   }
@@ -178,7 +161,7 @@
   auto advance_tap = [&]() {
     if (AMODE != MVD_A_DENSE) {
       ++c_kt;
-      if (++c_tap == 9) {
+      if (++c_tap == c_ntap) {
         c_tap = 0;
         ++c_cb;
       }
@@ -338,7 +321,7 @@
   }
 
   MVD_STAMP_AT(d, wave, 3);
-  tile_epilogue<BM, BN, WM, WN>(p, acc, smem, m0, n0, lane, wave, AMODE == MVD_A_DENSE && d.ln_stats != nullptr ? s_rows : nullptr);
+  tile_epilogue<BM, BN, WM, WN>(p, acc, smem, m0, n0, lane, wave, AMODE == MVD_A_DENSE && d.ln_stats != nullptr ? s_rows : nullptr, par);
   MVD_STAMP_AT(d, wave, 8);
 }
 
diff --git a/mvdfusion_amd/csrc/gemm_ws.hip b/mvdfusion_amd/csrc/gemm_ws.hip
--- a/mvdfusion_amd/csrc/gemm_ws.hip
+++ b/mvdfusion_amd/csrc/gemm_ws.hip
@@ -35,38 +35,19 @@
     const int q = nb >> 3, r = nb & 7, xcd = bid & 7, idx = bid >> 3;
     tile = (xcd < r ? xcd * (q + 1) : r * (q + 1) + (xcd - r) * q) + idx;
   }
-  const int m0 = (p.m_fastest ? tile % p.tiles_m : tile / p.tiles_n) * BM;
-  const int n0 = (p.m_fastest ? tile / p.tiles_m : tile % p.tiles_n) * BN;
+  const TileCoord tc = tile_coord<BM, BN>(p, tile);
+  const int m0 = tc.m0, n0 = tc.n0;
+  const int par = AMODE != MVD_A_DENSE ? tc.par : -1;
+  const int mlim = par >= 0 ? p.up4_mq : d.M;
   const int kt0 = blockIdx.z * p.kt_per_split;
   const int nkt = min(p.nk, kt0 + p.kt_per_split) - kt0;
   float* s_rows = (float*)(smem + SMEM + TAB_BYTES);
   int* s_tab = (int*)(smem + SMEM);
   if (AMODE != MVD_A_DENSE) {
-    const int hw = d.Hout * d.Wout;
     for (int e = tid; e < BM * 9; e += 512) {
       const int row = e / 9, tap = e - row * 9;
       const int m = m0 + row;
-      int off = -1;
-      if (m < d.M) {
-        const int b = m / hw;
-        const int rem = m - b * hw;
-        const int oy = rem / d.Wout, ox = rem - oy * d.Wout;
-        const int ky = tap / 3, kx = tap - ky * 3;
-        int iy, ix;
-        bool ok;
-        if (d.upsample) {
-          const int uy = oy + ky - 1, ux = ox + kx - 1;
-          ok = uy >= 0 && uy < d.Hout && ux >= 0 && ux < d.Wout;
-          iy = uy >> 1;
-          ix = ux >> 1;
-        } else {
-          iy = oy * d.stride + ky - (d.no_pad_tl ? 0 : 1);
-          ix = ox * d.stride + kx - (d.no_pad_tl ? 0 : 1);
-          ok = iy >= 0 && iy < d.Hin && ix >= 0 && ix < d.Win;
-        }
-        if (ok) off = ((b * d.Hin + iy) * d.Win + ix) * 2 * d.Cin;
-      }
-      s_tab[e] = off;
+      s_tab[e] = m < mlim ? conv_tap_offset(d, par, m, tap) : -1;
     }
     __syncthreads();
   }
@@ -79,13 +60,15 @@
     int a_step[AI], a_tab[AI], a_chunk[AI], a_off[AI], a_tail[AI];
     int c_tap = 0, c_cb = 0, c_kt = kt0;
     const int c_main = conv_tail_start(d);
+    const int c_ntap = conv_taps_per_block(d);
+    const u16* const wp = (const u16*)d.Wp + (par > 0 ? (size_t)par * p.nk * p.nt16 * 1024 : (size_t)0);
 #pragma unroll
     for (int i = 0; i < AI; ++i) {
       const int gi = lw + i * NL;
       const int R = (gi & 1) * 8 + gr;
       const int gc = (lane & 7) ^ ((R >> 1) & 7);
       const int m = m0 + gi * 8 + gr;
-      const bool ok = m < d.M;
+      const bool ok = m < mlim;
       a_cur[i] = ok ? (const u16*)d.A + (size_t)m * 2 * d.lda + gc * 8 + (size_t)kt0 * 64 : zero;
       a_step[i] = ok ? 64 : 0;
       a_tab[i] = (gi * 8 + gr) * 9;
@@ -93,8 +76,8 @@
       a_tail[i] = ok ? m * 2 * d.lda2 : -1;
     }
     if (AMODE != MVD_A_DENSE) {
-      c_cb = kt0 / 9;
-      c_tap = kt0 - c_cb * 9;
+      c_cb = kt0 / c_ntap;
+      c_tap = kt0 - c_cb * c_ntap;
 #pragma unroll
       for (int i = 0; i < AI; ++i) a_off[i] = s_tab[a_tab[i] + c_tap];
     }
@@ -113,7 +96,7 @@
           const int n = n0 + gi * 8 + gr;
           src = (gi < B_GRAN && n < d.N) ? (const u16*)d.Wp + (size_t)n * 2 * d.ldb + gc * 8 : nullptr;
         } else {
-          src = (gi < B_GRAN && nt < p.nt16) ? (const u16*)d.Wp + (size_t)nt * 1024 + (gi & 1) * 512 + lane * 8 : nullptr;
+          src = (gi < B_GRAN && nt < p.nt16) ? wp + (size_t)nt * 1024 + (gi & 1) * 512 + lane * 8 : nullptr;
         }
         b_cur[i] = src ? src + (size_t)kt0 * b_kstride : zero;
         b_step[i] = src ? b_kstride : 0;
@@ -144,7 +127,7 @@
       }
       if (AMODE != MVD_A_DENSE) {
         ++c_kt;
-        if (++c_tap == 9) {
+        if (++c_tap == c_ntap) {
           c_tap = 0;
           ++c_cb;
         }
@@ -273,7 +256,7 @@
   MVD_STAMP_AT(d, wave, 3);
   asm volatile("s_waitcnt vmcnt(0)" ::"v"(pf_sink) : "memory");
   __syncthreads();
-  tile_epilogue<BM, BN, CM, CN>(p, acc, smem, m0, n0, lane, wave, AMODE == MVD_A_DENSE && d.ln_stats != nullptr ? s_rows : nullptr);
+  tile_epilogue<BM, BN, CM, CN>(p, acc, smem, m0, n0, lane, wave, AMODE == MVD_A_DENSE && d.ln_stats != nullptr ? s_rows : nullptr, par);
   MVD_STAMP_AT(d, wave, 8);
 }
 
diff --git a/mvdfusion_amd/hip.py b/mvdfusion_amd/hip.py
--- a/mvdfusion_amd/hip.py
+++ b/mvdfusion_amd/hip.py
@@ -31,6 +31,7 @@
     return fmt, default, policy
 A_DENSE, A_CONV3X3 = 0, 1
 TAPS_FULL, TAPS_CENTRE_TAIL = 0, 2
+TAPS_UP4 = 1
 EPI_STORE, EPI_GEGLU, EPI_QKV = 0, 1, 2
 ACT_NONE, ACT_GELU, ACT_SILU, ACT_QUICKGELU = 0, 1, 2, 3
 STEP_STRIDE = 8
@@ -209,12 +210,13 @@
 
 class PackedWeight:
 
-    __slots__ = ("data", "N", "K", "n_real", "bias", "geglu", "conv_cin", "acc_scale", "tail_cin")
-
-    def __init__(self, data, N, K, n_real, bias, geglu=False, conv_cin=0, acc_scale=1.0, tail_cin=0):
+    __slots__ = ("data", "N", "K", "n_real", "bias", "geglu", "conv_cin", "acc_scale", "tail_cin", "up4")
+
+    def __init__(self, data, N, K, n_real, bias, geglu=False, conv_cin=0, acc_scale=1.0, tail_cin=0, up4=False):
         self.data, self.N, self.K, self.n_real, self.bias, self.geglu, self.conv_cin = data, N, K, n_real, bias, geglu, conv_cin
         self.acc_scale = acc_scale
         self.tail_cin = tail_cin
+        self.up4 = up4
 
 
 class RowStats:
@@ -352,6 +354,42 @@
 def tap_schedule(cin, cin2=0):
     assert cin % 32 == 0 and cin2 % 32 == 0
     return [(0, cb, tap) for cb in range(cin // 32) for tap in range(9)] + [(1, cb, 4) for cb in range(cin2 // 32)]
+
+
+def up4_schedule(weight):
+    w = weight.detach()
+    assert w.dim() == 4 and tuple(w.shape[2:]) == (3, 3)
+    rows = torch.tensor([[[1, 0, 0], [0, 1, 1]], [[1, 1, 0], [0, 0, 1]]], dtype=torch.float64, device=w.device)
+    wq = torch.einsum("ayk,cxl,oikl->acoiyx", rows, rows, w.double()).reshape(4, w.shape[0], w.shape[1], 2, 2).to(w.dtype)
+    nb = (w.shape[1] + 31) // 32
+    return wq, [(par, cb, tap) for par in range(4) for cb in range(nb) for tap in range(4)]
+
+
+def pack_conv3x3_up4(weight, bias=None):
+    wq, _ = up4_schedule(weight.detach().float())
+    Cout, Cin = wq.shape[1], wq.shape[2]
+    cin_pad, Np = (Cin + 31) // 32 * 32, (Cout + 15) // 16 * 16
+    K = 4 * cin_pad
+    m = torch.zeros(4, Cout, cin_pad, 4, dtype=torch.float32, device=wq.device)
+    m[:, :, :Cin] = wq.reshape(4, Cout, Cin, 4)
+    m = m.reshape(4, Cout, cin_pad // 32, 32, 4).permute(0, 1, 2, 4, 3).reshape(4, Cout, K).contiguous()
+    img = Np * K * 4
+    data = torch.empty(4 * img, dtype=torch.uint8, device=wq.device)
+    scale = _pack_scale(m)
+    for par in range(4):
+        check(lib().mvd_pack_linear_weight(ptr(m[par]), Cout, K, K, 0, scale, ptr(data[par * img:]), stream()))
+    b = None
+    if bias is not None:
+        b = torch.zeros(Np, dtype=torch.float32, device=wq.device)
+        b[:Cout] = bias.detach().float()
+    return PackedWeight(data, Np, K, Cout, b, conv_cin=cin_pad, acc_scale=1.0 / scale, up4=True)
+
+
+UP4_MIN_ROWS = int(os.environ.get("MVD_UP4_MIN_ROWS", "128"))
+
+
+def use_up4(B, Hin, Win, training=False):
+    return UP4_MIN_ROWS > 0 and not training and (Hin * Win) % 16 == 0 and B * Hin * Win >= UP4_MIN_ROWS
 
 
 def compose_conv_tail_bias(bias, tail_bias):
@@ -380,7 +418,7 @@
     return PackedWeight(data, Np, 9 * cin_pad + cin2_pad, Cout, b, conv_cin=cin_pad, acc_scale=1.0 / scale, tail_cin=cin2_pad)
 
 
-_CACHE_ATTRS = ("_p", "_pg", "_temb", "_xattn", "_head", "_pq", "_q", "_fused", "_lnf")
+_CACHE_ATTRS = ("_p", "_p4", "_pg", "_temb", "_xattn", "_head", "_pq", "_q", "_fused", "_lnf")
 
 
 def params_signature(module):
@@ -475,7 +513,11 @@
         if a2 is not None:
             assert a2.dtype == torch.int16 and a2.numel() // a2.shape[-1] == d.M and a2.shape[-1] // 2 >= tail_cin
             d.tap_mode, d.A2, d.lda2, d.Cin2 = TAPS_CENTRE_TAIL, a2.data_ptr(), int(a2.shape[-1] // 2), int(tail_cin)
-        assert conv["Cin"] * 9 + tail_cin == W.K, (conv["Cin"], tail_cin, W.K)
+        if getattr(W, "up4", False):
+            assert a2 is None and conv["Cin"] * 4 == W.K, (conv["Cin"], W.K)
+            d.tap_mode = TAPS_UP4
+        else:
+            assert conv["Cin"] * 9 + tail_cin == W.K, (conv["Cin"], tail_cin, W.K)
     else:
         d.a_mode = A_DENSE
         d.M = int(M if M is not None else A.numel() // A.shape[-1])
diff --git a/mvdfusion_amd/unet.py b/mvdfusion_amd/unet.py
--- a/mvdfusion_amd/unet.py
+++ b/mvdfusion_amd/unet.py
@@ -25,15 +25,21 @@
         super().__init__()
         self.channels, self.out_channels = channels, out_channels or channels
         self.conv = nn.Conv2d(self.channels, self.out_channels, 3, padding=padding)
-        self._p = None
+        self._p = self._p4 = None
 
     def run(self, ctx, x, H, W, out=None):
-        if self._p is None:
-            self._p = hip.pack_conv3x3(self.conv.weight, self.conv.bias)
+        if hip.use_up4(ctx.B, H, W, training=ctx.keep_fp32):
+            if self._p4 is None:
+                self._p4 = hip.pack_conv3x3_up4(self.conv.weight, self.conv.bias)
+            wp = self._p4
+        else:
+            if self._p is None:
+                self._p = hip.pack_conv3x3(self.conv.weight, self.conv.bias)
+            wp = self._p
         if out is None:
             out = ctx.act((ctx.B * 4 * H * W, self.out_channels))
         xp = hip.split_planes(x, ctx.ws.planes("updown.x", ctx.B * H * W, self.channels))
-        ctx.gemm(xp, self._p, out, conv=dict(B=ctx.B, Hin=H, Win=W, Cin=self.channels, Hout=2 * H, Wout=2 * W,
+        ctx.gemm(xp, wp, out, conv=dict(B=ctx.B, Hin=H, Win=W, Cin=self.channels, Hout=2 * H, Wout=2 * W,
                                             stride=1, upsample=1), gn=(ctx.B, 4 * H * W), kind="conv")
         return out, 2 * H, 2 * W
 
```
